# Nostrademous/dotaclient

Hardware: AMD Instinct MI355X
Metric: PPO optimizer samples/sec (whole node) + actor steps/sec, 1v1-mid LSTM policy (higher is better)
Workload: dtype fp32

## Files before the change

### dotaclient_amd/learner/engine.py

```python
from __future__ import annotations

import contextlib
import itertools
import os
import threading
from dataclasses import dataclass
from typing import Dict, List, Optional

import torch

from ..models.policy import Policy
from ..parallel.dp import DataParallel, FlatParams
from .losses import ppo_loss, split_heads, vpg_loss
from .optim import FlatAdam


CAPTURE_LOCK = threading.RLock()


_GRAPH_TOKENS = itertools.count(1)


def _capture_stream(device):
    return torch.cuda.Stream(device=device)
# ... 1 lines not shown

@dataclass

class LossConfig:
    algo: str = 'ppo'
    learning_rate: float = 1e-4
    entropy_coef: float = 0.01
    vf_coef: float = 0.5
    clip_eps: float = 0.1
    gamma: float = 0.98
    gae_lambda: float = 0.95
    max_grad_norm: float = 0.5
    compat_value_bug: bool = False
    offpolicy: str = 'clip'
    vtrace: bool = False
    vtrace_rho_bar: float = 1.0
    vtrace_c_bar: float = 1.0


class Learner:
    def __init__(self, policy: Policy, loss_cfg: LossConfig, device='cpu', backend: str = 'auto',
                 bucket_cap_mb: float = 8.0, overlap: bool = True, dp: bool = True, precision: str = 'fp32'):
        if precision not in ('fp32', 'bf16', 'fp32-exact'):
            raise ValueError(f'precision must be fp32, fp32-exact or bf16, got {precision!r}')
        self.device = torch.device(device)
        self.cfg = loss_cfg
        self.precision = precision
        self.policy = policy.to(self.device)
        auto = backend == 'auto'
        if auto:
            backend = 'fused' if self.device.type == 'cuda' else 'torch'
        self.backend = backend
        self.flat = FlatParams(self.policy, device=self.device)
        self.dp = DataParallel(self.policy, flat=self.flat, bucket_cap_mb=bucket_cap_mb, overlap=overlap,
                               broadcast=dp)
        self.opt = FlatAdam(self.flat, lr=loss_cfg.learning_rate, max_grad_norm=loss_cfg.max_grad_norm,
                            use_kernels=self.device.type == 'cuda')
        self.model = self.policy
        if backend == 'fused':
            from ..models.fused import FusedPolicy
            fused = FusedPolicy(self.policy, loss_cfg, precision=precision)
            if fused.use_pipeline():
                self.model = fused
                self.model.attach_flat(self.flat.flat)
            elif auto:
                self.backend = backend = 'torch'
            else:
                raise ValueError(f'backend fused: no kernel path for {self.policy.config} at {precision}')
        self.counts = self.policy.layout.action_counts()
        self.n_steps = 0
        self.graph = None
        self._static_idx: Dict[tuple, torch.Tensor] = {}
        self._graph_warmup = 0

    def enable_graph(self, warmup: int = 2):
        if self.backend != 'fused' or self.device.type != 'cuda':
            return False
        if not self.model.use_pipeline():
            return False
        self._graph_warmup = max(1, int(warmup))
        return True

    def _autocast(self):
        if self.backend == 'torch' and self.device.type == 'cuda' and self.precision == 'bf16':
            return torch.autocast('cuda', dtype=torch.bfloat16)
        return contextlib.nullcontext()

    def hidden_from_batch(self, batch):
        if not self.policy.is_recurrent:
            return None
        return (batch['h0'].unsqueeze(0).contiguous(), batch['c0'].unsqueeze(0).contiguous())

    def loss(self, batch: Dict[str, torch.Tensor]):
        cfg = self.cfg
        stable = not self.policy.config.compat_bugs
        if self.backend == 'fused':
            return self.model.loss(batch, cfg)
        with self._autocast():
            logits, values, _ = self.model.forward_packed(batch['env'], batch['units'], self.hidden_from_batch(batch),
                                                          reset=batch.get('reset'))
        logits = {k: v.float() for k, v in logits.items()}
        values = values.float()
        actions = split_heads(batch['actions'], self.counts)
        masks = split_heads(batch['masks'], self.counts)
        if cfg.algo == 'ppo':
            adv, ret, extra = batch['adv'], batch['ret'], {}
            if cfg.vtrace:
                adv, ret, extra = self._vtrace_torch(batch, logits, values, masks, actions)
            loss, metrics = ppo_loss(logits, values, actions, masks, adv, ret, batch['logp_old'],
                                     cfg.clip_eps, cfg.entropy_coef, cfg.vf_coef, stable=stable,
                                     offpolicy=cfg.offpolicy)
            metrics.update(extra)
            return loss, metrics
        return vpg_loss(logits, values, actions, masks, batch['norm_ret'], batch['ret'], cfg.entropy_coef,
                        cfg.vf_coef, compat_value_bug=cfg.compat_value_bug, stable=stable)

    def _vtrace_torch(self, batch, logits, values, masks, actions):
        from ..constants import EPS
        from ..ops.scan import vtrace_step
        from .losses import sampled_logp
        cfg = self.cfg
        B, S = batch['env'].shape[:2]
        tm = (lambda x: x.detach().float().reshape(B, S, *x.shape[2:]).transpose(0, 1).reshape(B * S, *x.shape[2:]))
        with torch.no_grad():
            lp = sampled_logp(logits, actions, masks, stable=not self.policy.config.compat_bugs)
            adv, ret, st = vtrace_step(tm(values.squeeze(-1)).cpu(), tm(lp).cpu(), tm(batch['logp_old']).cpu(),
                                       tm(batch['vt']).cpu(), B, S, cfg.gamma, cfg.gae_lambda, cfg.vtrace_rho_bar,
                                       cfg.vtrace_c_bar)
            dev = batch['env'].device
            back = (lambda x: x.reshape(S, B).t().contiguous().to(dev))
            adv, ret = back(adv), back(ret)
            v = batch['vt'][..., 2].float()
            n = v.sum().clamp_min(1.0)
            mu = (adv * v).sum() / n
            sd = (((adv - mu) ** 2 * v).sum() / n).sqrt()
            adv = ((adv - mu) / (sd + EPS)) * v
            s = st.sum(0)
            extra = {'offpolicy/rho_mean': (s[0] / s[3].clamp_min(1)).to(dev),
                     'offpolicy/rho_truncated': (s[1] / s[3].clamp_min(1)).to(dev),
                     'offpolicy/behaviour_kl': (s[2] / s[3].clamp_min(1)).to(dev)}
        return adv, ret, extra

    def _fwd_bwd(self, batch):
        self.dp.zero_grad()
        loss, metrics = self.loss(batch)
        loss.backward()
        if self.backend == 'fused' and getattr(self.model, 'direct_used', False):
            self.dp.has_grad.copy_(self.model.grad_mask)
        return {k: v.detach() for k, v in metrics.items()}

    def direct(self) -> bool:
        return self.backend == 'fused' and self.device.type == 'cuda' and self.model.use_pipeline()

    STEP_FIELDS = ('units', 'env', 'actions', 'masks', 'adv', 'ret', 'logp_old', 'norm_ret')

    @staticmethod
    def batch_to_time_major(batch):
        B, S = batch['env'].shape[:2]
        out = {}
        for k in Learner.STEP_FIELDS:
            v = batch.get(k)
            if v is None:
                v = torch.zeros(B, S, device=batch['env'].device)
            out[k] = v.transpose(0, 1).reshape(S * B, *v.shape[2:]).contiguous()
        if 'reset' in batch:
            out['reset'] = batch['reset'].transpose(0, 1).reshape(S * B).contiguous()
        if 'vt' in batch:
            out['vt'] = batch['vt'].transpose(0, 1).reshape(S * B, 4).contiguous()
        for k in ('h0', 'c0'):
            if k in batch:
                out[k] = batch[k].contiguous()
        return out, B, S

    def gather_time_major(self, replay, idx, S: int):
        B = idx.numel()
        fields = self.STEP_FIELDS + tuple(k for k in ('reset', 'vt') if k in replay.data)
        if idx.is_cuda:
            from .. import ops
            seq = [k for k in ('h0', 'c0') if k in replay.data]
            outs = ops.require().replay_gather([replay.data[k] for k in fields] +
                                               [replay.data[k] for k in seq], len(fields),
                                               idx.contiguous())
            return dict(zip(list(fields) + seq, outs))
        ar = getattr(self, '_arange', None)
        if ar is None or ar.numel() < S or ar.device != idx.device:
            ar = self._arange = torch.arange(max(S, 1), device=idx.device, dtype=torch.long)
        rows = (idx.view(1, B) * S + ar[:S].view(S, 1)).reshape(-1)
        out = {}
        for k in fields:
            pool = replay.data[k]
            out[k] = pool.view(-1, *pool.shape[2:]).index_select(0, rows)
        for k in ('h0', 'c0'):
            if k in replay.data:
                out[k] = replay.data[k].index_select(0, idx)
        return out

    def _split_mode(self) -> bool:
        import os
        if getattr(self, '_split', None) is None:
            force = os.environ.get('DCA_DP_SPLIT') == '1'
            ok = (self.direct() and (self.dp.enabled or force) and self.model.chunks == 1
                  and os.environ.get('DCA_DP_SPLIT', '') != '0')
            if ok:
                early = self.model.early_param_names()
                idx = [i for i, n in enumerate(self.model.param_names) if n in early]
                ok = self.dp.split_buckets(idx) if self.dp.enabled else bool(idx)
            self._split = bool(ok)
        return self._split

    def _direct_body(self, batch_tm, B, S, hook=None):
        self.flat.grad.zero_()
        if hook is None and self._split_mode():
            hook = self.dp.launch_early
        self.model.split_hook = hook
        try:
            vec = self.model.train_direct(batch_tm, B, S, self.cfg)
        finally:
            self.model.split_hook = None
        self.dp.has_grad.copy_(self.model.grad_mask)
        return vec

    def _metrics_from_vec(self, vec):
        from ..models.pipelined import METRIC_NAMES
        names = [n for n in METRIC_NAMES if (self.cfg.algo == 'ppo' or n not in ('approx_kl', 'clipfrac'))
                 and (self.cfg.vtrace or not n.startswith('offpolicy/'))]
        return {n: vec[METRIC_NAMES.index(n)] for n in names}

    def _graph_ready(self) -> bool:
        return bool(self._graph_warmup) and self.n_steps >= self._graph_warmup

    @staticmethod
    def _capture_mode() -> str:
        return 'thread_local'

    def _replay_split(self, key, body):
        graphs = self.__dict__.setdefault('_graphs', {})
        if key not in graphs:
            if getattr(self, '_graph_stream', None) is None:
                self._graph_stream = _capture_stream(self.device)
            s = self._graph_stream
            cur = torch.cuda.current_stream(self.device)
            s.wait_stream(cur)
            with torch.cuda.stream(s):
                body(lambda: None)
            cur.wait_stream(s)
            mode = self._capture_mode()
            g1, g2 = torch.cuda.CUDAGraph(), torch.cuda.CUDAGraph()
            switched = []

            def switch():
                g1.capture_end()
                g2.capture_begin(pool=g1.pool(), capture_error_mode=mode)
                switched.append(True)

            torch.cuda.synchronize(self.device)
            with CAPTURE_LOCK, torch.cuda.stream(s):
                g1.capture_begin(capture_error_mode=mode)
                out = body(switch)
                if not switched:
                    raise RuntimeError('direct step never reached its DP split point')
                g2.capture_end()
            cur.wait_stream(s)
            graphs[key] = ((g1, g2), out)
            self.graph = g1
        (g1, g2), out = graphs[key]
        g1.replay()
        self.dp.launch_early()
        g2.replay()
        return out

    def _replay_graph(self, key, body):
        graphs = self.__dict__.setdefault('_graphs', {})
        if key not in graphs:
            if getattr(self, '_graph_stream', None) is None:
                self._graph_stream = _capture_stream(self.device)
            s = self._graph_stream
            cur = torch.cuda.current_stream(self.device)
            s.wait_stream(cur)
            with torch.cuda.stream(s):
                body()
            cur.wait_stream(s)
            g = torch.cuda.CUDAGraph()
            with CAPTURE_LOCK, torch.cuda.graph(g, stream=s, capture_error_mode=self._capture_mode()):
                out = body()
            graphs[key] = (g, out)
            self.graph = g
        g, out = graphs[key]
        g.replay()
        return out

    def _step_direct_batch(self, batch):
        if not self._graph_ready():
            bt, B, S = self.batch_to_time_major(batch)
            return self._direct_body(bt, B, S)
        B, S = batch['env'].shape[:2]
        key = ('batch', B, S, tuple(sorted(batch)))
        if key not in self.__dict__.get('_graphs', {}):
            self._static_in = {k: v.clone() for k, v in batch.items()}
        else:
            for k, v in batch.items():
                self._static_in[k].copy_(v, non_blocking=True)

        if self._split_mode():
            def body_split(hook):
                bt, B_, S_ = self.batch_to_time_major(self._static_in)
                return self._direct_body(bt, B_, S_, hook=hook)
            return self._replay_split(key, body_split)

        def body():
            bt, B_, S_ = self.batch_to_time_major(self._static_in)
            return self._direct_body(bt, B_, S_)
        return self._replay_graph(key, body)

    @staticmethod
    def _replay_key(replay, B: int, S: int):
        tok = replay.__dict__.get('_dca_graph_token')
        if tok is None:
            tok = replay.__dict__['_dca_graph_token'] = next(_GRAPH_TOKENS)
        return ('replay', tok, B, S)

    def release_graphs(self, replay) -> int:
        tok = replay.__dict__.get('_dca_graph_token')
        if tok is None:
            return 0
        graphs = self.__dict__.get('_graphs', {})
        dead = [k for k in graphs if k[0] == 'replay' and k[1] == tok]
        for k in dead:
            g = graphs.pop(k)[0]
            if self.graph is g or (isinstance(g, tuple) and self.graph in g):
                self.graph = None
            self._static_idx.pop(k, None)
        return len(dead)

    def train_step_replay(self, replay, B: int, recent: Optional[int] = None) -> Dict[str, torch.Tensor]:
        if self.direct() and self._graph_ready() and getattr(replay, 'host_sampling', False):
            key = self._replay_key(replay, B, replay.S)
            if key in self.__dict__.get('_graphs', {}):
                replay.sample_into(self._static_idx[key], recent)
                return self._step_replay_key(replay, key, None)
        return self.train_step_indices(replay, replay.sample_indices(B, recent))

    def train_step_indices(self, replay, idx: torch.Tensor) -> Dict[str, torch.Tensor]:
        if not self.direct():
            return self.train_step(replay.gather(idx))
        if self._graph_ready():
            return self._step_replay_key(replay, self._replay_key(replay, idx.numel(), replay.S), idx)
        return self._finish(self._direct_body(self.gather_time_major(replay, idx, replay.S), idx.numel(), replay.S))

    def _step_replay_key(self, replay, key, idx: Optional[torch.Tensor]) -> Dict[str, torch.Tensor]:
        B, S = key[2], key[3]
        if key not in self.__dict__.get('_graphs', {}):
            self._static_idx[key] = idx.clone()
        elif idx is not None:
            self._static_idx[key].copy_(idx)
        sidx = self._static_idx[key]
        if self._split_mode():
            vec = self._replay_split(key, lambda hook: self._direct_body(
                self.gather_time_major(replay, sidx, S), B, S, hook=hook))
        else:
            vec = self._replay_graph(key, lambda: self._direct_body(self.gather_time_major(replay, sidx, S), B, S))
        return self._finish(vec)

    def _sync_and_step(self):
        if self.backend == 'fused':
            self.dp.err_flag.copy_(self.model.err)
        fold = self.dp.enabled and self.opt.use_kernels
        self.dp.sync(scale=not fold)
        if self.backend == 'fused' and self.dp.enabled:
            sticky = getattr(self, '_err_any', None)
            if sticky is None:
                sticky = self._err_any = torch.zeros_like(self.dp.err_flag)
            torch.maximum(sticky, self.dp.err_flag, out=sticky)
        return self.opt.step(self.dp.counts, divide=fold, skip=self.dp.err_flag)

    def check_error(self):
        self.opt.check_nonfinite()
        if self.backend != 'fused':
            return
        sticky = getattr(self, '_err_any', None)
        if sticky is not None and float(sticky.item()) != 0.0:
            own = int(self.model.err.item())
            sticky.zero_()
            raise RuntimeError(f'persistent kernel error on a data-parallel rank (own code {own}): the step was '
                               'skipped by every rank\'s Adam')
        self.model.check_error()

    def error_flags(self) -> List[torch.Tensor]:
        flags = [self.opt.nonfinite]
        if self.backend == 'fused':
            sticky = getattr(self, '_err_any', None)
            if sticky is not None:
                flags.append(sticky)
            flags.append(self.model.err)
        return flags

    def _finish(self, vec):
        metrics = self._metrics_from_vec(vec.clone())
        metrics['grad_norm'] = self._sync_and_step().clone()
        self.n_steps += 1
        return metrics

    def train_step(self, batch: Dict[str, torch.Tensor]) -> Dict[str, torch.Tensor]:
        if self.direct():
            return self._finish(self._step_direct_batch(batch))
        metrics = self._fwd_bwd(batch)
        metrics['grad_norm'] = self._sync_and_step().clone()
        self.n_steps += 1
        return metrics

    @torch.no_grad()
    def evaluate_sequences(self, data: Dict[str, torch.Tensor], n: int, chunk: int = 32):
        S = data['units'].shape[1]
        if self.direct():
            from .. import ops
            C = ops.require()
            fields = ('units', 'env', 'actions', 'masks') + (('reset',) if 'reset' in data else ())
            seq = [k for k in ('h0', 'c0') if k in data]
            lps, vals = [], []
            for i0 in range(0, n, chunk):
                i1 = min(n, i0 + chunk)
                idx = torch.arange(i0, i1, device=self.device, dtype=torch.int64)
                outs = C.replay_gather([data[k] for k in fields] + [data[k] for k in seq], len(fields), idx)
                bt = dict(zip(list(fields) + seq, outs))
                lp, v = self.model.forward_logp_value(bt, i1 - i0, S)
                lps.append(lp.view(S, i1 - i0).t())
                vals.append(v.view(S, i1 - i0).t())
            return torch.cat(lps, 0).contiguous(), torch.cat(vals, 0).contiguous()
        from .losses import sampled_logp
        hidden = None
        if self.policy.is_recurrent and 'h0' in data:
            hidden = (data['h0'][:n].unsqueeze(0).contiguous(), data['c0'][:n].unsqueeze(0).contiguous())
        with self._autocast():
            logits, values, _ = self.model.forward_packed(data['env'][:n], data['units'][:n], hidden,
                                                          reset=data['reset'][:n] if 'reset' in data else None)
        logits = {k: v.float() for k, v in logits.items()}
        lp = sampled_logp(logits, split_heads(data['actions'][:n], self.counts), split_heads(data['masks'][:n],
                                                                                             self.counts),
                          stable=not self.policy.config.compat_bugs)
        return lp.float(), values.float().reshape(n, S)

    def state_dict(self):
        return {'optimizer': self.opt.state_dict(), 'n_steps': self.n_steps}

    def broadcast_state(self, src: int = 0):
        import torch.distributed as dist
        for t in (self.opt.exp_avg, self.opt.exp_avg_sq, self.opt.steps):
            dist.broadcast(t, src)
        n = torch.tensor([self.n_steps], dtype=torch.int64, device=self.opt.steps.device)
        dist.broadcast(n, src)
        self.n_steps = int(n.item())

    def load_state_dict(self, d):
        self.opt.load_state_dict(d['optimizer'])
        self.n_steps = d.get('n_steps', 0)

    def after_load_weights(self):
        self.flat.rebind()
        if self.backend == 'fused':
            self.model.refresh()
```

### dotaclient_amd/models/fused.py

```python
from __future__ import annotations

from typing import Dict, List

import torch

from .policy import Policy

LDZ = 160


class FusedPolicy:
    def __init__(self, policy: Policy, loss_cfg=None, precision: str = 'fp32'):
        from .. import ops
        if precision not in ('fp32', 'bf16', 'fp32-exact'):
            raise ValueError(f'precision must be fp32, fp32-exact or bf16, got {precision!r}')
        self.C = ops.require()
        self.policy = policy
        self.cfg = policy.config
        self.loss_cfg = loss_cfg
        self.precision = precision
        self.fp32 = precision in ('fp32', 'fp32-exact')
        self.exact = precision == 'fp32-exact'
        dev = next(policy.parameters()).device
        self.err = torch.zeros(1, dtype=torch.int32, device=dev)
        self.param_names: List[str] = [n for n, _ in policy.named_parameters()]
        self.params = [p for _, p in policy.named_parameters()]
        self.fully_fused = not self.cfg.entity_attention and self.cfg.unit_dim == 128 and self.cfg.env_dim == 128
        self.attention_fused = (self.cfg.entity_attention and self.cfg.unit_dim == 128 and self.cfg.env_dim == 128
                                and self.cfg.attention_heads == 4 and self.cfg.layout.max_units == 64)

    def wcast(self, t: torch.Tensor) -> torch.Tensor:
        t = t.detach()
        return t if self.fp32 else t.to(torch.bfloat16)

    def apply_direct_grads(self, grads, g, written=(), set_mask: bool = True):
        gl, views, mask = [], [], []
        for name, p, t in zip(self.param_names, self.params, grads):
            mask.append(t is not None or name in written)
            if t is None:
                continue
            if p.grad is None:
                p.grad = torch.zeros_like(p)
            gl.append((t if t.dtype == torch.float32 else t.float()).contiguous())
            views.append(p.grad)
        self.C.multi_axpy(views, gl, None if g is None else g.reshape(1).float().contiguous())
        if set_mask and getattr(self, '_mask_list', None) != mask:
            self._mask_list = mask
            self.grad_mask = torch.tensor(mask, dtype=torch.float32, device=self.err.device)
        self.direct_used = True

    def attach_flat(self, flat: torch.Tensor):
        self.flat_buffer = flat
        self._wimg = None

    def weight_images(self):
        from .pipelined import WeightImages
        with_value = self.loss_cfg is None or self.loss_cfg.vf_coef > 0
        key = (with_value, self.flat_buffer.data_ptr() if getattr(self, 'flat_buffer', None) is not None else None,
               tuple(p.data_ptr() for p in self.params))
        if getattr(self, '_wimg', None) is None or self._wimg_key != key:
            if getattr(self, 'flat_buffer', None) is None:
                raise RuntimeError('FusedPolicy.attach_flat(flat) must be called before the fused LSTM step')
            self._wimg = WeightImages(self, self.flat_buffer, with_value)
            self._wimg_key = key
        return self._wimg

    def scratch(self, name, shape, dtype, device):
        d = self.__dict__.setdefault('_scratch', {})
        t = d.get(name)
        if t is None or tuple(t.shape) != tuple(shape) or t.dtype != dtype or t.device != torch.device(device):
            t = d[name] = torch.zeros(shape, dtype=dtype, device=device)
        return t

    def loss_prep_ws(self, device):
        return self.scratch('loss_prep_ws', (int(self.C.loss_prep_ws_elems()),), torch.int32, device)

    def train_direct(self, batch_tm, B: int, S: int, cfg=None) -> torch.Tensor:
        from .pipelined import train_direct
        if cfg is not None:
            self.loss_cfg = cfg
        self.refresh()
        self.direct_used = False
        return train_direct(self, batch_tm, B, S)

    def forward_logp_value(self, batch_tm, B: int, S: int):
        from .pipelined import forward_logp_value
        self.refresh()
        H = self.cfg.hidden
        dev = batch_tm['units'].device
        h0, c0 = batch_tm.get('h0'), batch_tm.get('c0')
        if h0 is None:
            h0 = c0 = torch.zeros(B, H, device=dev)
        return forward_logp_value(self, batch_tm['units'], batch_tm['env'], batch_tm['actions'], batch_tm['masks'],
                                  h0, c0, B, S, reset_t=batch_tm.get('reset'))

    def side_stream(self):
        if getattr(self, '_side', None) is None:
            self._side = torch.cuda.Stream(device=self.err.device)
        return self._side

    def use_pipeline(self) -> bool:
        if not (self.fully_fused or self.attention_fused) or not self.fp32:
            return False
        if self.cfg.rnn == 'lstm':
            return self.cfg.hidden % 128 == 0
        return self.cfg.hidden % 128 == 0 and self.cfg.pre_rnn_dim == 256

    split_hook = None
    early_applied = frozenset()

    def early_param_names(self) -> frozenset:
        pre = ('affine_pre_rnn.', 'rnn.', 'fake_rnn.', 'affine_head_enum.', 'affine_move_', 'affine_unit_attention.',
               'affine_value.')
        return frozenset(n for n in self.param_names if n.startswith(pre))

    @property
    def chunks(self) -> int:
        import os
        return int(os.environ.get('DCA_PIPELINE_CHUNKS', '1'))

    def gate_perm(self, H, device):
        key = (H, str(device))
        if getattr(self, '_perm_key', None) != key:
            from ..ops.lstm import gate_perm
            self._perm, self._perm_key = gate_perm(H, device), key
            self._inv = torch.empty_like(self._perm)
            self._inv[self._perm] = torch.arange(self._perm.numel(), device=self._perm.device)
        return self._perm

    def gate_perm_i32(self, H, device):
        key = (H, str(device))
        if getattr(self, '_perm32_key', None) != key:
            self._perm32, self._perm32_key = self.gate_perm(H, device).to(torch.int32).contiguous(), key
        return self._perm32

    def gate_inv(self, H, device):
        self.gate_perm(H, device)
        return self._inv

    def type_segments(self, device):
        key = str(device)
        if getattr(self, '_seg_key', None) != key:
            counts = list(self.cfg.layout.counts)
            seg = torch.zeros(sum(counts), 6, device=device)
            off = 0
            for t, cnt in enumerate(counts):
                seg[off:off + cnt, t] = 1.0
                off += cnt
            self._seg, self._seg_key = seg, key
        return self._seg

    def type_offset_list(self):
        import itertools
        return [0] + list(itertools.accumulate(self.cfg.layout.counts))

    def type_offsets(self, device):
        key = str(device)
        if getattr(self, '_toff_key', None) != key:
            import itertools
            offs = [0] + list(itertools.accumulate(self.cfg.layout.counts))
            self._toff, self._toff_key = torch.tensor(offs, dtype=torch.int32, device=device), key
        return self._toff

    def unit_types(self, device):
        key = str(device)
        if getattr(self, '_utype_key', None) != key:
            ty = sum([[t] * c for t, c in enumerate(self.cfg.layout.counts)], [])
            self._utype, self._utype_key = torch.tensor(ty, dtype=torch.uint8, device=device), key
        return self._utype

    def refresh(self):
        self.params = [p for _, p in self.policy.named_parameters()]

    def head_cat(self, P, differentiable: bool = False):
        H = self.cfg.hidden
        dev = P['affine_value.weight'].device
        d = (lambda t: t) if differentiable else (lambda t: t.detach())
        with_value = self.loss_cfg is None or self.loss_cfg.vf_coef > 0
        wv = d(P['affine_value.weight']) if with_value else torch.zeros(1, H, device=dev)
        bv = d(P['affine_value.bias']) if with_value else torch.zeros(1, device=dev)
        pad = LDZ - 150
        w = torch.cat([d(P['affine_unit_attention.weight']), d(P['affine_head_enum.weight']),
                       d(P['affine_move_x.weight']), d(P['affine_move_y.weight']), wv,
                       torch.zeros(pad, H, device=dev)], 0)
        b = torch.cat([d(P['affine_unit_attention.bias']), d(P['affine_head_enum.bias']),
                       d(P['affine_move_x.bias']), d(P['affine_move_y.bias']), bv,
                       torch.zeros(pad, device=dev)], 0)
        return w, b

    def split_head_grads(self, dW, db, grads):
        spans = [('affine_unit_attention', 0, 128), ('affine_head_enum', 128, 131), ('affine_move_x', 131, 140),
                 ('affine_move_y', 140, 149)]
        if self.loss_cfg is None or self.loss_cfg.vf_coef > 0:
            spans.append(('affine_value', 149, 150))
        for name, lo, hi in spans:
            grads[f'{name}.weight'] = dW[lo:hi]
            grads[f'{name}.bias'] = db[lo:hi]

    def loss(self, batch: Dict[str, torch.Tensor], cfg):
        from ..ops.heads import assemble_loss, batch_norms
        from .pipelined import PipelinedPolicyLoss
        if not self.use_pipeline():
            raise ValueError(f'FusedPolicy: no kernel path for {self.cfg} at {self.precision} (use the torch backend)')
        self.loss_cfg = cfg
        self.direct_used = False
        B, S = batch['env'].shape[:2]
        N = B * S
        dev = batch['env'].device
        actions = batch['actions'].reshape(N, -1).contiguous()
        masks = batch['masks'].reshape(N, -1).contiguous()
        ret = batch['ret'].reshape(N).float().contiguous()
        algo = 0 if cfg.algo == 'ppo' else 1
        norms = batch_norms(actions, ret, cfg.compat_value_bug and algo == 1, S)
        zeros = torch.zeros(N, device=dev)
        adv = batch['adv'].reshape(N).contiguous() if 'adv' in batch else zeros
        lpo = batch['logp_old'].reshape(N).contiguous() if 'logp_old' in batch else zeros
        nret = batch['norm_ret'].reshape(N).contiguous() if 'norm_ret' in batch else zeros
        rst = batch.get('reset')
        H = self.cfg.hidden
        h0 = batch.get('h0')
        c0 = batch.get('c0')
        if h0 is None:
            h0 = torch.zeros(B, H, device=dev)
            c0 = torch.zeros(B, H, device=dev)
        self.refresh()
        vt = batch.get('vt') if getattr(cfg, 'vtrace', False) else None
        part, logp = PipelinedPolicyLoss.apply(self, batch['units'].contiguous(), batch['env'].contiguous(), actions,
                                               masks, adv, ret, lpo, nret, norms, h0.contiguous(), c0.contiguous(),
                                               rst, vt, *self.params)
        loss, metrics = assemble_loss(part, norms, cfg, ret, N, S)
        if getattr(self, 'vtrace_stats', None) is not None:
            st = self.vtrace_stats.sum(0)
            for i, k in enumerate(('offpolicy/rho_mean', 'offpolicy/rho_truncated', 'offpolicy/behaviour_kl')):
                metrics[k] = st[i] / st[3].clamp_min(1.0)
        return loss, metrics

# ... 5 lines not shown
```

### dotaclient_amd/models/pipelined.py

```python
from __future__ import annotations

import os
from typing import Dict, List, Optional

import torch

from ..ops.lstm import team_bwd, team_fwd
from .policy import TYPE_SUFFIX

LDZ = 160

DIRECT_GEMM_GRADS = ('rnn.weight_hh_l0', 'rnn.weight_ih_l0', 'affine_pre_rnn.weight', 'affine_pre_rnn.bias')

METRIC_NAMES = ['loss', 'policy_loss', 'entropy_loss', 'advantage_loss', 'entropy', 'advantage', 'approx_kl',
                'clipfrac', 'entropy/enum', 'entropy/x', 'entropy/y', 'entropy/target_unit',
                'offpolicy/rho_mean', 'offpolicy/rho_truncated', 'offpolicy/behaviour_kl']


def _frag_order(w: torch.Tensor) -> torch.Tensor:
    R, K = w.shape
    return w.view(R // 16, 16, K // 32, 4, 8).permute(0, 2, 3, 1, 4).contiguous()


def _k16_order(w: torch.Tensor) -> torch.Tensor:
# ... 375 lines not shown
            if lin:
                pass
            elif rst is not None:
                hprev = torch.cat([h016.unsqueeze(0), hs16[:S - 1]], 0).masked_fill_(rst.bool().unsqueeze(2), 0.0)
                gemm_tn(dG16, hprev.view(n, H), out=dWhh, perm=gperm, accumulate=True)
            elif t0 > 0:
                gemm_tn(dG16, hs16[t0 - 1:t1 - 1].view(n, H), out=dWhh, perm=gperm, accumulate=True)
            else:
                gemm_tn(dG16, hs16[0:t1 - 1].view(n - B, H), out=dWhh, perm=gperm, accumulate=True, b0=h016)
            if lin:
                gemm_tn(dG16, x16[r0:r1], out=dWih, colsum=dbf)
            else:
                gemm_tn(dG16, x16[r0:r1], out=dWih, perm=gperm, accumulate=True)
        dpre16, dx896 = C.dpre_dx(dG16, dx_w[0], dx_w[1], x16[r0:r1], dx_w[2], dx_w[3])
        pre_main = wg_side and split is None and exact
        if pre_main:
            with torch.cuda.stream(sL):
                wg_done = torch.cuda.Event()
                wg_done.record(sL)
            after_enc.append(lambda d=dpre16, xr=x896[r0:r1]: gemm_tn(d, xr, out=dWpre, accumulate=True,
                                                                      colsum=dbpre))
        elif wg_side:
            sL.wait_stream(main)
            with torch.cuda.stream(sL):
                gemm_tn(dpre16, x896[r0:r1], out=dWpre, accumulate=True, colsum=dbpre)
                wg_done = torch.cuda.Event()
                wg_done.record(sL)
        else:
            gemm_tn(dpre16, x896[r0:r1], out=dWpre, accumulate=True, colsum=dbpre)
        if split is not None:
            if wg_done is not None:
                main.wait_event(wg_done)
                wg_done = None
            if not lin:
                grads['rnn.bias_ih_l0'] = db
                grads['rnn.bias_hh_l0'] = db
            early = [grads.pop(nm, None) if nm in early_names else None for nm in fp.param_names]
            fp.apply_direct_grads(early, None, set_mask=False)
            fp.early_applied = early_names
            split()
            split = None
        demb_in = None
        if attn:
            if exact:
                nil = E0p.new_empty(0)
                wot, wq4 = (W['wot_x'], nil), (W['wq4_x'], nil)
            else:
                wot = [_frag_order(t) for t in C.split_bf16x2(P['entity_attn.out.weight'].detach().t().contiguous())]
                wq4 = [_k16_order(t) for t in C.split_bf16x2(P['entity_attn.qkv.weight'].detach())]
            dE1, dQKV, demb_in, lnsum = C.attn_block_bwd(
                dtl, z, dx896, arg, toff, bool(cfg.compat_bugs), Oat, QKV, bqkv, lse, E0p, W['bout'], ln_mu, ln_rs,
                P['entity_attn.ln.weight'].detach(), wot[0], wot[1], wq4[0], wq4[1], None)
            dgam, dbet, dbt_attn = lnsum[:128], lnsum[128:256], lnsum[256:].view(6, 128)
            dbout = torch.empty(128, device=dev)
            dbqkv = torch.empty(384, device=dev)
            if wg_side and _WG_BALANCE == '1':
                sL.wait_stream(main)
                side_after.append(lambda: gemm_tn(dQKV, Xn, out=dWqkv, colsum=dbqkv))
                after_enc.append(lambda: gemm_tn(dE1, Oat, out=dWout, colsum=dbout))
            elif wg_side:
                sL.wait_stream(main)
                side_after.append(lambda: (gemm_tn(dE1, Oat, out=dWout, colsum=dbout),
                                           gemm_tn(dQKV, Xn, out=dWqkv, colsum=dbqkv)))
            else:
                dWout = gemm_tn(dE1, Oat, colsum=dbout)
                dWqkv = gemm_tn(dQKV, Xn, colsum=dbqkv)
        def small_grads():
            return C.enc_small_grads(z[r0:r1], dtl[r0:r1], fp.type_offsets(dev), dx896, env_t[r0:r1], we, be,
                                     bool(cfg.compat_bugs))
        small = None
        if wg_side and not side_after:
            sL.wait_stream(main)
            with torch.cuda.stream(sL):
                small = small_grads()
                wg_done = torch.cuda.Event()
                wg_done.record(sL)
        dwt_c, dw1_c, db1_c = C.encoder_bwd(units_t[r0:r1], w1, b1, wtT16, dtl[r0:r1], z[r0:r1],
                                            dx896, arg[r0:r1], counts, bool(cfg.compat_bugs), demb_in=demb_in,
                                            exact=exact)
        for fn in after_enc:
            fn()
        after_enc.clear()
        if side_after:
            with torch.cuda.stream(sL):
                for fn in side_after:
                    fn()
                small = small_grads()
                wg_done = torch.cuda.Event()
                wg_done.record(sL)
            side_after.clear()
        dw1 = _acc(dw1, dw1_c)
        db1 = _acc(db1, db1_c)
        dWt = _acc(dWt, dwt_c)
        dbt_c, dWe_c, dbe_c = small if small is not None else small_grads()
        dbt = _acc(dbt, dbt_attn if attn else dbt_c)
        dWe = _acc(dWe, dWe_c)
        dbe = _acc(dbe, dbe_c)
    if wg_done is not None:
        main.wait_event(wg_done)
    if not direct:
        if not lin:
            grads['rnn.weight_hh_l0'] = dWhh
            grads['rnn.weight_ih_l0'] = dWih
        grads['affine_pre_rnn.weight'] = dWpre
        grads['affine_pre_rnn.bias'] = dbpre
    if not lin and 'rnn.bias_ih_l0' not in fp.early_applied:
        grads['rnn.bias_ih_l0'] = db
        grads['rnn.bias_hh_l0'] = db
    grads['affine_unit_basic_stats.weight'] = dw1
    grads['affine_unit_basic_stats.bias'] = db1
    for t, s in enumerate(TYPE_SUFFIX):
        grads[f'affine_unit_{s}.weight'] = dWt[t]
        grads[f'affine_unit_{s}.bias'] = dbt[t]
    grads['affine_env.weight'] = dWe
    grads['affine_env.bias'] = dbe
    if attn:
        grads['entity_attn.ln.weight'] = dgam
        grads['entity_attn.ln.bias'] = dbet
        grads['entity_attn.qkv.weight'] = dWqkv
        grads['entity_attn.qkv.bias'] = dbqkv
        grads['entity_attn.out.weight'] = dWout
        grads['entity_attn.out.bias'] = dbout
    part = parts[0] if len(parts) == 1 else torch.cat(parts, 0)
    return part, logp, grads


class PipelinedPolicyLoss(torch.autograd.Function):
    @staticmethod
    def forward(ctx, fp, units, env, actions, masks, adv, ret, logp_old, nret, norms, h0, c0, reset, vt, *params):
        P = dict(zip(fp.param_names, params))
        B, S, U, _ = units.shape
        N = B * S
        tm = (lambda x: x.reshape(B, S, *x.shape[1:]).transpose(0, 1).reshape(N, *x.shape[1:]).contiguous())
        units_t = units.transpose(0, 1).reshape(N, U, 10).contiguous()
        env_t = env.transpose(0, 1).reshape(N, 3).contiguous()
        W = fp.weight_images().refresh(fp.C)
        rst_t = reset.reshape(B, S).transpose(0, 1).reshape(N).contiguous() if reset is not None else None
        part, logp, grads = fused_step_tm(fp, W, P, units_t, env_t, tm(actions), tm(masks), tm(adv), tm(ret),
                                          tm(logp_old), tm(nret), norms, h0, c0, B, S, reset_t=rst_t,
                                          vt_t=tm(vt.reshape(N, 4)) if vt is not None else None)
        ctx.grads = [grads.get(nm) for nm in fp.param_names]
        ctx.fp = fp
        logp_b = logp.view(S, B).t().reshape(N)
        ctx.mark_non_differentiable(logp_b)
        return part.sum(0), logp_b

    @staticmethod
    def backward(ctx, gpart, _glogp):
        ctx.fp.apply_direct_grads(ctx.grads, gpart[15])
        ctx.grads = None
        return (None,) * (14 + len(ctx.fp.param_names))


def train_direct(fp, batch_tm: Dict[str, torch.Tensor], B: int, S: int) -> torch.Tensor:
    C = fp.C
    lc = fp.loss_cfg
    N = B * S
    dev = batch_tm['units'].device
    norms = fp.scratch('norms', (8,), torch.float32, dev)
    main = torch.cuda.current_stream(dev)
    sL = fp.side_stream()
    sL.wait_stream(main)
    with torch.cuda.stream(sL):
        C.loss_prep(batch_tm['actions'], fp.loss_prep_ws(dev), norms)
        if lc.compat_value_bug and lc.vf_coef > 0:
            g_last = batch_tm['ret'].view(S, B)[:, B - 1]
            norms[6:8] = torch.stack([g_last.sum(), (g_last * g_last).sum()])
    W = fp.weight_images().refresh(C)
    P = dict(zip(fp.param_names, fp.params))
    H = fp.cfg.hidden
    h0 = batch_tm.get('h0')
    c0 = batch_tm.get('c0')
    if h0 is None:
        h0 = torch.zeros(B, H, device=dev)
        c0 = torch.zeros(B, H, device=dev)
    gout = {nm: P[nm].grad for nm in DIRECT_GEMM_GRADS if nm in P}
    vt = batch_tm.get('vt') if getattr(lc, 'vtrace', False) else None
    if getattr(lc, 'vtrace', False) and vt is None:
        raise ValueError('LossConfig.vtrace needs the per-row vt field (learner/optimizer.py advantages="vtrace-step")')
    part, _, grads = fused_step_tm(fp, W, P, batch_tm['units'], batch_tm['env'], batch_tm['actions'],
                                   batch_tm['masks'], batch_tm['adv'], batch_tm['ret'], batch_tm['logp_old'],
                                   batch_tm['norm_ret'], norms, h0, c0, B, S, gout=gout,
                                   reset_t=batch_tm.get('reset'), vt_t=vt)
    fp.apply_direct_grads([grads.get(nm) for nm in fp.param_names], None,
                          written=set(gout) | set(fp.early_applied))
    out = torch.empty(16, device=dev)
    C.loss_assemble(part, norms, N, 0 if lc.algo == 'ppo' else 1, float(lc.entropy_coef), float(lc.vf_coef), out,
                    S=S, compat_value_bug=bool(lc.compat_value_bug))
    if fp.vtrace_stats is not None:
        st = fp.vtrace_stats.sum(0)
        out[12:15] = st[:3] / st[3].clamp_min(1.0)
    return out


def forward_logp_value(fp, units_t, env_t, act_t, msk_t, h0, c0, B: int, S: int,
                       reset_t: Optional[torch.Tensor] = None):
    C = fp.C
    cfg = fp.cfg
    exact = bool(getattr(fp, 'exact', False))
    lin = cfg.rnn != 'lstm'
    N = B * S
    U = units_t.shape[1]
    H = cfg.hidden
    dev = units_t.device
    W = fp.weight_images().refresh(C)
    P = dict(zip(fp.param_names, fp.params))
    w1, b1 = P['affine_unit_basic_stats.weight'].detach(), P['affine_unit_basic_stats.bias'].detach()
    we, be = P['affine_env.weight'].detach(), P['affine_env.bias'].detach()
    x896, emb, arg = C.encoder_fwd(units_t, env_t, w1, b1, W['wt16'], W['bt'], we, be, list(cfg.layout.counts),
                                   bool(cfg.compat_bugs), exact=exact)
    if cfg.entity_attention:
        E0p = emb.view(N * U, 128)
        if exact:
            nil = E0p.new_empty(0)
            wq, wo = (W['wq_x'], nil), (W['wo_x'], nil)
        else:
            wq, wo = W['wq_f'], W['wo_f']
        arg = torch.empty(N, 6, 128, dtype=torch.uint8, device=dev)
        out = C.attn_block_fwd(E0p, W['bout'], P['entity_attn.ln.weight'].detach(), P['entity_attn.ln.bias'].detach(),
                               wq[0], wq[1], P['entity_attn.qkv.bias'].detach(), wo[0], wo[1],
                               fp.type_offset_list(), x896, arg, bool(cfg.compat_bugs), 1e-5)
        emb = out[6].view(N, U, 128)
    elif cfg.compat_bugs:
        x896[:, 768:896] = x896[:, 512:640]
    if exact:
        nil = W['wpre16'].new_empty(0)
        x16, xp = C.pre_rnn_chain(x896, W['wpre16'], nil, W['bpre16'], W['wih16'], nil)
        hw = ((W['wcat256'], nil), W['bcat256'])
    else:
        x16, xp = C.pre_rnn_chain(x896, W['pre_s'][0], W['pre_s'][1], W['bpre16'], W['ih_s'][0], W['ih_s'][1])
        hw = (W['wcat_s'], W['bcat256'])
    if lin:
        hs = xp.add_(W['bias4']).view(S, B, H)
    else:
        rst = reset_t.reshape(S, B) if reset_t is not None else None
        hs = torch.empty(S, B, H, device=dev)
        o = team_fwd(C, xp.view(S, B, H, 4), W['whh16'], h0.contiguous(), c0.contiguous(), fp.err, False,
                     time_major=True, hs_out=hs, cs_out=torch.empty(S, B, H, device=dev),
                     gates_out=torch.empty(S, B, H, 4, device=dev), bias4=W['bias4'], reset=rst)
        hs = o[0]
    z = C.rowmm_out256(hs.reshape(N, H), hw[0][0], hw[0][1], hw[1])
    zero = fp.scratch('fwd_zero', (N,), torch.float32, dev)
    norms = fp.scratch('fwd_norms', (8,), torch.float32, dev)
    _, _, _, lp = C.heads_loss(z, emb, act_t, msk_t, zero, zero, zero, zero, norms, 0, False, S, B, 0.1, 0.0, 0.0,
                               dz_bf16=False, precise=exact)
    return lp, z[:, 149].contiguous()
```

### dotaclient_amd/ops/csrc/bindings.cpp

```cpp
#include <torch/extension.h>
#include <ATen/hip/HIPContext.h>
#include <hip/hip_runtime.h>

#include <algorithm>
#include <cstring>

#include "launchers.h"

namespace {

inline hipStream_t cur_stream() { return at::hip::getCurrentHIPStream().stream(); }

inline void hip_check(hipError_t e, const char* what) {
  TORCH_CHECK(e == hipSuccess, what, " failed: ", hipGetErrorString(e));
}

#define CHECK_DEV(t) TORCH_CHECK((t).is_cuda(), #t " must be a GPU tensor")
#define CHECK_CONTIG(t) TORCH_CHECK((t).is_contiguous(), #t " must be contiguous")
#define CHECK_DT(t, dt) TORCH_CHECK((t).scalar_type() == (dt), #t " must be " #dt)
#define CHECK_F32(t) CHECK_DEV(t); CHECK_CONTIG(t); CHECK_DT(t, at::kFloat)
#define CHECK_BF16(t) CHECK_DEV(t); CHECK_CONTIG(t); CHECK_DT(t, at::kBFloat16)
#define CHECK_I32(t) CHECK_DEV(t); CHECK_CONTIG(t); CHECK_DT(t, at::kInt)
#define CHECK_U8(t) CHECK_DEV(t); CHECK_CONTIG(t); CHECK_DT(t, at::kByte)

// ... 75 lines not shown
    CHECK_DEV(dst[i]); CHECK_DEV(src[i]); CHECK_CONTIG(dst[i]); CHECK_CONTIG(src[i]);
    TORCH_CHECK(dst[i].nbytes() == src[i].nbytes(), "multi_copy: byte size mismatch at ", i);
    d.push_back(dst[i].data_ptr());
    s.push_back(src[i].data_ptr());
    n.push_back((long long)dst[i].nbytes());
  }
  hip_check(dca_multi_copy(d.data(), s.data(), n.data(), (int)d.size(), cur_stream()), "dca_multi_copy");
}

void multi_axpy(std::vector<torch::Tensor> dst, std::vector<torch::Tensor> src, c10::optional<torch::Tensor> scale) {
  TORCH_CHECK(dst.size() == src.size(), "multi_axpy: list length mismatch");
  TORCH_CHECK(dst.size() <= 64, "multi_axpy: at most 64 tensors");
  std::vector<float*> d;
  std::vector<const float*> s;
  std::vector<long long> n;
  for (size_t i = 0; i < dst.size(); ++i) {
    CHECK_F32(dst[i]); CHECK_F32(src[i]);
    TORCH_CHECK(dst[i].numel() == src[i].numel(), "multi_axpy: numel mismatch at ", i);
    d.push_back(ptr<float>(dst[i]));
    s.push_back(ptr<float>(src[i]));
    n.push_back(dst[i].numel());
  }
  const float* sp = nullptr;
  if (scale.has_value() && scale->defined()) { CHECK_F32((*scale)); sp = ptr<float>(*scale); }
  hip_check(dca_multi_axpy(d.data(), s.data(), n.data(), (int)d.size(), sp, cur_stream()), "dca_multi_axpy");
}

constexpr int64_t kTeamTraceElems = 32LL * 4 * 64 * 8;
inline unsigned long long* trace_ptr(const c10::optional<torch::Tensor>& t, int64_t need, const char* name) {
  if (!t.has_value() || !t->defined()) return nullptr;
  CHECK_DEV(*t); CHECK_CONTIG(*t);
  TORCH_CHECK(t->scalar_type() == at::kLong && t->numel() >= need, name,
              ": trace must be a contiguous int64 GPU tensor with >= ", need, " elements");
  return ptr<unsigned long long>(*t);
}


namespace {
inline torch::Tensor out_or_new(const c10::optional<torch::Tensor>& o, at::IntArrayRef shape,
                                const at::TensorOptions& opt, const char* name) {
  if (o.has_value() && o->defined()) {
    TORCH_CHECK(o->is_cuda() && o->is_contiguous() && o->sizes() == shape && o->scalar_type() == opt.dtype(),
                name, ": preallocated output has the wrong shape/dtype/layout");
    return *o;
  }
  return torch::empty(shape, opt);
}
}

inline const unsigned char* reset_ptr(const c10::optional<torch::Tensor>& r, int B, int S) {
  if (!r.has_value() || !r->defined()) return nullptr;
  CHECK_DEV(*r); CHECK_CONTIG(*r);
  TORCH_CHECK(r->scalar_type() == at::kByte && r->numel() == (int64_t)B * S, "reset must be B*S uint8 flags");
  return r->data_ptr<unsigned char>();
}

inline void check_ctl(const torch::Tensor& ctl) {
  CHECK_DEV(ctl); CHECK_CONTIG(ctl);
  TORCH_CHECK(ctl.numel() * ctl.element_size() >= (int64_t)dca_lstm_team_ctl_bytes(),
              "team control block too small (use ops.lstm.team_ctl())");
}

std::vector<torch::Tensor> lstm_team_fwd(torch::Tensor xp4, torch::Tensor whh, torch::Tensor h0, torch::Tensor c0,
                                         torch::Tensor err, torch::Tensor ctl, bool want_f32_h,
                                         c10::optional<torch::Tensor> trace,
                                         bool time_major, c10::optional<torch::Tensor> hs_out,
                                         c10::optional<torch::Tensor> cs_out, c10::optional<torch::Tensor> gates_out,
                                         c10::optional<torch::Tensor> bias4, bool precise,
                                         c10::optional<torch::Tensor> reset) {
  CHECK_F32(xp4); CHECK_DEV(whh); CHECK_CONTIG(whh); CHECK_F32(h0); CHECK_F32(c0); CHECK_I32(err); check_ctl(ctl);
  const bool f32w = whh.scalar_type() == at::kFloat;
  TORCH_CHECK(f32w || whh.scalar_type() == at::kBFloat16, "whh must be bf16 or f32");
  TORCH_CHECK(xp4.dim() == 4 && xp4.size(3) == 4, "xp4 must be (B,S,H,4) or (S,B,H,4)");
  const int B = time_major ? xp4.size(1) : xp4.size(0), S = time_major ? xp4.size(0) : xp4.size(1);
  const int H = xp4.size(2);
  TORCH_CHECK(whh.size(0) == 4 * H && whh.size(1) == H, "whh must be (4H,H)");
  TORCH_CHECK(h0.size(0) == B && h0.size(1) == H && c0.size(0) == B && c0.size(1) == H, "h0/c0 must be (B,H)");
  TORCH_CHECK(H == 128 || H == 256 || H == 512, "lstm_team_fwd: H in {128,256,512}");
  auto f32 = xp4.options();
  const int64_t d0 = time_major ? S : B, d1 = time_major ? B : S;
  auto hs = out_or_new(hs_out, {d0, d1, H}, f32w ? f32 : f32.dtype(at::kBFloat16), "hs_out");
  torch::Tensor hsf = (want_f32_h && !f32w) ? torch::empty({d0, d1, H}, f32) : torch::Tensor();
  auto cs = out_or_new(cs_out, {d0, d1, H}, f32, "cs_out");
  auto gates4 = out_or_new(gates_out, {d0, d1, H, 4}, f32, "gates_out");
  auto hn = torch::empty({B, H}, f32);
  auto cn = torch::empty({B, H}, f32);
  const float* bias_p = nullptr;
  if (bias4.has_value() && bias4->defined()) {
    CHECK_F32((*bias4));
    TORCH_CHECK(bias4->numel() == 4 * H, "bias4 must hold 4H floats (unit-major)");
    bias_p = ptr<float>(*bias4);
  }
  const size_t wsb = dca_lstm_team_workspace(B, H, 0, f32w ? 1 : 0);
  auto ws = torch::empty({(int64_t)wsb}, f32.dtype(at::kByte));
  hip_check(dca_lstm_team_fwd(ptr<float>(xp4), whh.data_ptr(), ptr<float>(h0), ptr<float>(c0),
                              f32w ? nullptr : ptr<short>(hs),
                              f32w ? ptr<float>(hs) : (want_f32_h ? ptr<float>(hsf) : nullptr), ptr<float>(cs),
                              ptr<float>(gates4), ptr<float>(hn), ptr<float>(cn), ctl.data_ptr(), ws.data_ptr(), wsb,
                              ptr<unsigned>(err), B, S, H, time_major ? 1 : 0, cur_stream(),
                              trace_ptr(trace, kTeamTraceElems, "lstm_team_fwd"),
                              bias_p, f32w ? 1 : 0, precise ? 1 : 0, reset_ptr(reset, B, S)),
            "dca_lstm_team_fwd");
  if (f32w) return {hs, hs, cs, gates4, hn, cn};
  return {hs, want_f32_h ? hsf : hs, cs, gates4, hn, cn};
}

std::vector<torch::Tensor> lstm_team_bwd(torch::Tensor dhs, torch::Tensor gates4, torch::Tensor cs,
                                         torch::Tensor c0, c10::optional<torch::Tensor> dhn,
                                         c10::optional<torch::Tensor> dcn, torch::Tensor whh, torch::Tensor err,
                                         torch::Tensor ctl, c10::optional<torch::Tensor> trace, bool time_major,
                                         c10::optional<torch::Tensor> dg_out, bool dg_bf16, bool want_dbias,
                                         bool precise, c10::optional<torch::Tensor> reset) {
  CHECK_F32(dhs); CHECK_F32(gates4); CHECK_F32(cs); CHECK_F32(c0); CHECK_DEV(whh); CHECK_CONTIG(whh); CHECK_I32(err);
  check_ctl(ctl);
  const bool f32w = whh.scalar_type() == at::kFloat;
  TORCH_CHECK(f32w || whh.scalar_type() == at::kBFloat16, "whh must be bf16 or f32");
  TORCH_CHECK(!(f32w && dg_bf16), "lstm_team_bwd: the fp32 variant writes fp32 gate gradients");
  const int B = time_major ? dhs.size(1) : dhs.size(0), S = time_major ? dhs.size(0) : dhs.size(1);
  const int H = dhs.size(2);
  TORCH_CHECK(gates4.dim() == 4 && gates4.size(0) == dhs.size(0) && gates4.size(1) == dhs.size(1) &&
                  gates4.size(2) == H && gates4.size(3) == 4, "gates4 must match dhs with a trailing 4");
  TORCH_CHECK(cs.sizes() == dhs.sizes(), "cs must match dhs");
  TORCH_CHECK(c0.size(0) == B && c0.size(1) == H, "c0 must be (B,H)");
  TORCH_CHECK(whh.size(0) == 4 * H && whh.size(1) == H, "whh must be (4H,H)");
  TORCH_CHECK(H == 128 || H == 256 || H == 512, "lstm_team_bwd: H in {128,256,512}");
  const float* dhn_p = nullptr;
  const float* dcn_p = nullptr;
  if (dhn.has_value() && dhn->defined()) { CHECK_F32((*dhn)); dhn_p = ptr<float>(*dhn); }
  if (dcn.has_value() && dcn->defined()) { CHECK_F32((*dcn)); dcn_p = ptr<float>(*dcn); }
  auto f32 = dhs.options();
  auto dgates4 = out_or_new(dg_out, {dhs.size(0), dhs.size(1), H, 4}, dg_bf16 ? f32.dtype(at::kBFloat16) : f32,
                            "dg_out");
  auto dh0 = torch::empty({B, H}, f32);
  auto dc0 = torch::empty({B, H}, f32);
  torch::Tensor dbp = want_dbias ? torch::empty({dca_lstm_team_chains(B, f32w ? 1 : 0), 4 * H}, f32) : torch::Tensor();
  const size_t wsb = dca_lstm_team_workspace(B, H, 1, f32w ? 1 : 0);
  auto ws = torch::empty({(int64_t)wsb}, f32.dtype(at::kByte));
  hip_check(dca_lstm_team_bwd(ptr<float>(dhs), ptr<float>(gates4), ptr<float>(cs), ptr<float>(c0), dhn_p, dcn_p,
                              whh.data_ptr(), dg_bf16 ? nullptr : ptr<float>(dgates4), ptr<float>(dh0),
                              ptr<float>(dc0), ctl.data_ptr(), ws.data_ptr(), wsb, ptr<unsigned>(err), B, S, H,
                              time_major ? 1 : 0, cur_stream(),
                              trace_ptr(trace, kTeamTraceElems, "lstm_team_bwd"),
                              dg_bf16 ? ptr<short>(dgates4) : nullptr, want_dbias ? ptr<float>(dbp) : nullptr,
                              f32w ? 1 : 0, precise ? 1 : 0, reset_ptr(reset, B, S)),
            "dca_lstm_team_bwd");
  if (want_dbias) return {dgates4, dh0, dc0, dbp.sum(0)};
  return {dgates4, dh0, dc0};
}

std::vector<torch::Tensor> heads_loss(torch::Tensor z, torch::Tensor emb, torch::Tensor act, torch::Tensor msk,
                                      torch::Tensor adv, torch::Tensor ret, torch::Tensor logp_old,
                                      torch::Tensor nret, torch::Tensor norms, int64_t algo, bool compat_value_bug,
                                      int64_t S_bug, int64_t B_bug, double clip_eps, double ent_coef,
                                      double vf_coef, bool dz_bf16, bool precise) {
  CHECK_F32(z); CHECK_DEV(emb); CHECK_CONTIG(emb); CHECK_U8(act); CHECK_U8(msk); CHECK_F32(adv); CHECK_F32(ret);
  CHECK_F32(logp_old); CHECK_F32(nret); CHECK_F32(norms);
  const bool ef32 = emb.scalar_type() == at::kFloat;
  TORCH_CHECK(ef32 || emb.scalar_type() == at::kBFloat16, "emb must be bf16 or f32");
  TORCH_CHECK(z.dim() == 2 && emb.dim() == 3 && emb.size(2) == 128, "z (N,ldz), emb (N,U,128)");
  const int N = z.size(0), ldz = z.size(1), U = emb.size(1);
  TORCH_CHECK(emb.size(0) == N && act.size(0) == N && msk.size(0) == N, "row count mismatch");
  TORCH_CHECK(act.size(1) == 21 + U && msk.size(1) == 21 + U, "actions/masks must be (N, 21+U)");
  TORCH_CHECK(adv.numel() == N && ret.numel() == N && logp_old.numel() == N && nret.numel() == N, "per-row inputs");
  TORCH_CHECK(norms.numel() >= 8, "norms must hold 8 floats");
  TORCH_CHECK(ldz % 4 == 0 && ldz >= 150 && U <= 64, "ldz must be a multiple of 4 and >= 150; U <= 64");
  auto dz = dz_bf16 ? torch::empty_like(z, z.options().dtype(at::kBFloat16)) : torch::empty_like(z);
  auto dtl = torch::empty({N, U}, z.options());
  const int nb = dca_heads_loss_nblocks(N);
  auto part = torch::empty({nb, 16}, z.options());
  auto logp = torch::empty({N}, z.options());
  hip_check(dca_heads_loss(ptr<float>(z), ldz, emb.data_ptr(), ptr<unsigned char>(act), ptr<unsigned char>(msk),
                           21 + U, ptr<float>(adv), ptr<float>(ret), ptr<float>(logp_old), ptr<float>(nret),
                           ptr<float>(norms), dz_bf16 ? nullptr : ptr<float>(dz), ptr<float>(dtl), ptr<float>(part),
                           ptr<float>(logp), N, U, (int)algo, compat_value_bug ? 1 : 0, (int)S_bug, (int)B_bug,
                           (float)clip_eps, (float)ent_coef, (float)vf_coef, cur_stream(),
                           dz_bf16 ? ptr<short>(dz) : nullptr, ef32 ? 1 : 0, precise && ef32 ? 1 : 0),
            "dca_heads_loss");
  return {dz, dtl, part, logp};
}

std::vector<torch::Tensor> encoder_fwd(torch::Tensor units, torch::Tensor env, torch::Tensor w1, torch::Tensor b1,
                                       torch::Tensor wt, torch::Tensor bt, torch::Tensor we, torch::Tensor be,
                                       std::vector<int64_t> counts, bool compat, bool exact,
                                       c10::optional<torch::Tensor> x896_out, c10::optional<torch::Tensor> emb_out,
                                       c10::optional<torch::Tensor> arg_out) {
  CHECK_F32(units); CHECK_F32(env); CHECK_F32(w1); CHECK_F32(b1); CHECK_DEV(wt); CHECK_CONTIG(wt); CHECK_F32(bt);
  CHECK_F32(we); CHECK_F32(be);
  const bool f32w = wt.scalar_type() == at::kFloat;
  TORCH_CHECK(f32w || wt.scalar_type() == at::kBFloat16, "wt must be bf16 or f32");
  TORCH_CHECK(!exact || f32w, "encoder_fwd: exact mode needs fp32 weights");
  TORCH_CHECK(units.dim() == 3 && units.size(2) == 10, "units must be (N,U,10)");
  const int N = units.size(0), U = units.size(1);
  TORCH_CHECK(env.size(0) == N && env.size(1) == 3, "env must be (N,3)");
  TORCH_CHECK(w1.size(0) == 128 && w1.size(1) == 10 && wt.size(0) == 6 && wt.size(1) == 128 && wt.size(2) == 128,
              "weight shapes");
  TORCH_CHECK(counts.size() == 6, "counts must have 6 entries");
  int c[6];
  int64_t tot = 0;
  for (int i = 0; i < 6; ++i) { c[i] = (int)counts[i]; tot += counts[i]; }
  TORCH_CHECK(tot == U && U <= 64, "counts must sum to U <= 64");
  auto o = units.options();
  const auto adt = f32w ? at::kFloat : at::kBFloat16;
  auto x896 = out_or_new(x896_out, {N, 896}, o.dtype(adt), "x896_out");
  auto emb = out_or_new(emb_out, {N, U, 128}, o.dtype(adt), "emb_out");
  auto arg = out_or_new(arg_out, {N, 6, 128}, o.dtype(at::kByte), "arg_out");
  hip_check(dca_encoder_fwd(ptr<float>(units), ptr<float>(env), ptr<float>(w1), ptr<float>(b1), wt.data_ptr(),
                            ptr<float>(bt), ptr<float>(we), ptr<float>(be), x896.data_ptr(), emb.data_ptr(),
                            ptr<unsigned char>(arg), N, U, c, compat ? 1 : 0, cur_stream(), exact ? 2 : (f32w ? 1 : 0)),
            "dca_encoder_fwd");
  return {x896, emb, arg};
}

std::vector<torch::Tensor> encoder_bwd(torch::Tensor units, torch::Tensor w1, torch::Tensor b1, torch::Tensor wtT,
                                       torch::Tensor dtl, torch::Tensor q, torch::Tensor dx, torch::Tensor arg,
                                       std::vector<int64_t> counts, bool compat,
                                       c10::optional<torch::Tensor> demb_in, bool exact) {
  CHECK_F32(units); CHECK_F32(w1); CHECK_F32(b1); CHECK_DEV(wtT); CHECK_CONTIG(wtT); CHECK_F32(dtl); CHECK_F32(dx);
  CHECK_U8(arg); CHECK_DEV(q); CHECK_DT(q, at::kFloat);
  const bool f32w = wtT.scalar_type() == at::kFloat;
  TORCH_CHECK(f32w || wtT.scalar_type() == at::kBFloat16, "wtT must be bf16 or f32");
  TORCH_CHECK(!exact || f32w, "encoder_bwd: exact mode needs fp32 weights");
  const int N = units.size(0), U = units.size(1);
  TORCH_CHECK(q.dim() == 2 && q.size(0) == N && q.size(1) >= 128 && q.stride(1) == 1 && q.stride(0) % 4 == 0,
              "q must be (N, >=128) with unit column stride and 16-B aligned rows");
  TORCH_CHECK(dtl.size(0) == N && dtl.size(1) == U && dx.size(0) == N && dx.size(1) == 896, "dtl/dx shapes");
  TORCH_CHECK(arg.size(0) == N && arg.size(1) == 6 && arg.size(2) == 128, "arg shape");
  int c[6];
  int64_t tot = 0;
  for (int i = 0; i < 6; ++i) { c[i] = (int)counts[i]; tot += counts[i]; }
  TORCH_CHECK(tot == U && U <= 64, "counts must sum to U <= 64");
  auto o = units.options();
  auto dwt = torch::empty({6, 128, 128}, o);
  auto dw1 = torch::empty({128, 10}, o);
  auto db1 = torch::empty({128}, o);
  const size_t wsb = dca_encoder_bwd_workspace(N, U, c, f32w ? 1 : 0);
  auto ws = torch::empty({(int64_t)((wsb + 3) / 4)}, o);
  const void* dein = nullptr;
  if (demb_in && demb_in->defined()) {
    CHECK_DEV(*demb_in); CHECK_CONTIG(*demb_in);
    TORCH_CHECK(demb_in->scalar_type() == (f32w ? at::kFloat : at::kBFloat16), "encoder_bwd: demb_in dtype");
    TORCH_CHECK(demb_in->numel() == (int64_t)N * U * 128, "demb_in must be (N, U, 128)");
    dein = demb_in->data_ptr();
  }
  hip_check(dca_encoder_bwd(ptr<float>(units), ptr<float>(w1), ptr<float>(b1), wtT.data_ptr(), ptr<float>(dtl),
                            ptr<float>(q), (int)q.stride(0), ptr<float>(dx), ptr<unsigned char>(arg), ptr<float>(dwt),
                            ptr<float>(dw1), ptr<float>(db1), ws.data_ptr(), wsb, N, U, c, compat ? 1 : 0,
                            cur_stream(), dein, exact ? 2 : (f32w ? 1 : 0)),
            "dca_encoder_bwd");
  return {dwt, dw1, db1};
}

void sample_actions(torch::Tensor z, torch::Tensor emb, torch::Tensor handles, int64_t seed, torch::Tensor ctr,
                    torch::Tensor idx, torch::Tensor act, torch::Tensor msk, torch::Tensor logp, torch::Tensor value) {
  CHECK_F32(z); CHECK_DEV(emb); CHECK_CONTIG(emb); CHECK_DEV(handles); CHECK_CONTIG(handles);
  const bool e32 = emb.scalar_type() == at::kFloat;
  TORCH_CHECK(e32 || emb.scalar_type() == at::kBFloat16, "sample_actions: emb bf16 or fp32");
  const bool h32 = handles.scalar_type() == at::kInt;
  TORCH_CHECK(h32 || handles.scalar_type() == at::kLong, "sample_actions: handles int64 or int32");
  CHECK_DEV(ctr); CHECK_DT(ctr, at::kLong); CHECK_I32(idx); CHECK_U8(act); CHECK_U8(msk); CHECK_F32(logp);
  CHECK_F32(value);
  TORCH_CHECK(z.dim() == 2 && emb.dim() == 3 && emb.size(2) == 128, "z (N,ldz), emb (N,U,128)");
  const int N = z.size(0), ldz = z.size(1), U = emb.size(1);
  TORCH_CHECK(emb.size(0) == N && handles.size(0) == N && handles.size(1) == U, "row/unit count mismatch");
  TORCH_CHECK(idx.size(0) == N && idx.size(1) == 4 && logp.numel() == N && value.numel() == N, "output shapes");
  TORCH_CHECK(act.size(0) == N && act.size(1) == 21 + U && msk.sizes() == act.sizes(), "act/msk (N,21+U)");
  TORCH_CHECK(U <= 64 && ldz >= 150, "U <= 64, ldz >= 150");
  hip_check(dca_sample_actions(ptr<float>(z), ldz, emb.data_ptr(), e32 ? 1 : 0, handles.data_ptr(), h32 ? 1 : 0, N,
                               U, (unsigned long long)seed, ptr<long long>(ctr), ptr<int>(idx),
                               ptr<unsigned char>(act), ptr<unsigned char>(msk), ptr<float>(logp), ptr<float>(value),
                               cur_stream()),
            "dca_sample_actions");
}

static long long* bump_ptr(const c10::optional<torch::Tensor>& bump) {
  if (!bump || !bump->defined()) return nullptr;
  CHECK_DEV(*bump); CHECK_DT(*bump, at::kLong);
  TORCH_CHECK(bump->numel() >= 1, "bump: (1) int64 counter");
  return ptr<long long>(*bump);
}

void actor_state_prep(torch::Tensor pre, torch::Tensor h, torch::Tensor c, torch::Tensor keep, torch::Tensor xh,
                      c10::optional<torch::Tensor> bump) {
  CHECK_BF16(pre); CHECK_F32(h); CHECK_F32(c); CHECK_F32(keep); CHECK_BF16(xh);
  const int N = h.size(0), H = h.size(1), P = pre.size(1);
  TORCH_CHECK(pre.dim() == 2 && pre.size(0) == N && c.sizes() == h.sizes() && keep.numel() == N && xh.dim() == 2 &&
              xh.size(0) == N && xh.size(1) == P + H && H % 4 == 0 && P % 4 == 0, "actor_state_prep shapes");
  hip_check(dca_actor_state_prep(ptr<short>(pre), ptr<float>(h), ptr<float>(c), ptr<float>(keep), ptr<short>(xh), N, P,
                                 H, bump_ptr(bump), cur_stream()), "dca_actor_state_prep");
}

void lstm_cell(torch::Tensor gates, torch::Tensor h, torch::Tensor c, torch::Tensor h16,
               c10::optional<torch::Tensor> active) {
  CHECK_F32(gates); CHECK_F32(h); CHECK_F32(c); CHECK_BF16(h16);
  const int N = h.size(0), H = h.size(1);
  TORCH_CHECK(gates.size(0) == N && gates.size(1) == 4 * H && c.sizes() == h.sizes() && h16.sizes() == h.sizes(),
              "lstm_cell shapes");
  const float* act = nullptr;
  if (active && active->defined()) {
    CHECK_F32(*active);
    TORCH_CHECK(active->numel() == N, "lstm_cell: active must have one entry per row");
    act = ptr<float>(*active);
  }
  hip_check(dca_lstm_cell(ptr<float>(gates), ptr<float>(h), ptr<float>(c), ptr<short>(h16), act, N, H, cur_stream()),
            "dca_lstm_cell");
}

void actor_fp8(torch::Tensor x896, torch::Tensor wpre, torch::Tensor spre, torch::Tensor bpre, torch::Tensor wg,
               torch::Tensor sg, torch::Tensor bg, torch::Tensor wh, torch::Tensor sh, torch::Tensor bh,
               torch::Tensor h, torch::Tensor c, torch::Tensor keep, torch::Tensor z,
               c10::optional<torch::Tensor> active, c10::optional<torch::Tensor> bump) {
  CHECK_BF16(x896); CHECK_U8(wpre); CHECK_U8(wg); CHECK_U8(wh);
  CHECK_F32(spre); CHECK_F32(bpre); CHECK_F32(sg); CHECK_F32(bg); CHECK_F32(sh); CHECK_F32(bh);
  CHECK_F32(h); CHECK_F32(c); CHECK_F32(keep); CHECK_F32(z);
  const int n = x896.size(0);
  TORCH_CHECK(x896.dim() == 2 && x896.size(1) == 896, "actor_fp8: x896 (n, 896)");
  TORCH_CHECK(wpre.numel() == 256 * 896 && spre.numel() == 256 && bpre.numel() == 256, "actor_fp8: pre-RNN 256x896");
  TORCH_CHECK(wg.numel() == 2048 * 768 && sg.numel() == 2048 && bg.numel() == 2048, "actor_fp8: gates 2048x768");
  TORCH_CHECK(wh.numel() == 160 * 512 && sh.numel() == 160 && bh.numel() == 160, "actor_fp8: heads 160x512");
  TORCH_CHECK(h.dim() == 2 && h.size(0) == n && h.size(1) == 512 && c.sizes() == h.sizes() && keep.numel() == n,
              "actor_fp8: h, c (n, 512), keep (n)");
  TORCH_CHECK(z.dim() == 2 && z.size(0) == n && z.size(1) == 160, "actor_fp8: z (n, 160)");
  const float* act = nullptr;
  if (active && active->defined()) {
    CHECK_F32(*active);
    TORCH_CHECK(active->numel() == n, "actor_fp8: active (n)");
    act = ptr<float>(*active);
  }
  hip_check(dca_actor_fp8(ptr<short>(x896), wpre.data_ptr(), ptr<float>(spre), ptr<float>(bpre), wg.data_ptr(),
                          ptr<float>(sg), ptr<float>(bg), wh.data_ptr(), ptr<float>(sh), ptr<float>(bh), ptr<float>(h),
// ... 78 lines not shown
  } else {
    CHECK_BF16(wqh); CHECK_BF16(wql); CHECK_BF16(woh); CHECK_BF16(wol);
  }
  TORCH_CHECK(e0.numel() % (64 * 128) == 0 && e0.size(-1) == 128, "attn_block_fwd: e0 (N·64, 128)");
  const int64_t N = e0.numel() / (64 * 128);
  TORCH_CHECK(wqh.numel() == 384 * 128 && (exact || wql.numel() == 384 * 128) && woh.numel() == 128 * 128 &&
              (exact || wol.numel() == 128 * 128) && bq.numel() == 384 && bout.numel() == 128 && gamma.numel() == 128 &&
              beta.numel() == 128, "attn_block_fwd: weight shapes");
  TORCH_CHECK(x896.dim() == 2 && x896.size(0) == N && x896.size(1) == 896, "attn_block_fwd: x896 (N, 896)");
  TORCH_CHECK(arg.numel() == N * 6 * 128, "attn_block_fwd: arg (N, 6, 128)");
  TORCH_CHECK(type_off.size() == 7 && type_off[0] == 0 && type_off[6] == 64, "attn_block_fwd: 7 type offsets 0 … 64");
  int off[7];
  for (int i = 0; i < 7; ++i) off[i] = (int)type_off[i];
  auto o32 = e0.options();
  auto xn = torch::empty({N * 64, 128}, o32);
  auto mu = torch::empty({N * 64}, o32);
  auto rs = torch::empty({N * 64}, o32);
  auto qkv = torch::empty({N * 64, 384}, o32);
  auto o = torch::empty({N * 64, 128}, o32);
  auto lse = torch::empty({N, 4, 64}, o32);
  auto e1 = torch::empty({N * 64, 128}, o32);
  hip_check(dca_attn_block_fwd_f32(ptr<float>(e0), ptr<float>(bout), ptr<float>(gamma), ptr<float>(beta),
                                   wqh.data_ptr(), exact ? nullptr : wql.data_ptr(), ptr<float>(bq), woh.data_ptr(),
                                   exact ? nullptr : wol.data_ptr(), ptr<float>(xn), ptr<float>(mu), ptr<float>(rs),
                                   ptr<float>(qkv), ptr<float>(o), ptr<float>(lse), ptr<float>(e1), ptr<float>(x896),
                                   ptr<unsigned char>(arg), off, compat ? 1 : 0, (int)N, (float)eps, cur_stream(),
                                   exact ? 1 : 0),
            "dca_attn_block_fwd_f32");
  return {xn, mu, rs, qkv, o, lse, e1};
}

static void check_type_off(const std::vector<int64_t>& t) {
  TORCH_CHECK(t.size() == 7 && t[0] == 0 && t[6] == 64, "type offsets must be 7 values from 0 to 64");
  for (int i = 0; i < 6; ++i) TORCH_CHECK(t[i + 1] >= t[i], "type offsets must be non-decreasing");
}

std::vector<torch::Tensor> attn_block_bwd(torch::Tensor dtl, torch::Tensor q, torch::Tensor dx, torch::Tensor arg,
                                          std::vector<int64_t> type_off, bool compat, torch::Tensor o,
                                          torch::Tensor qkv, torch::Tensor bq, torch::Tensor lse, torch::Tensor e0,
                                          torch::Tensor bout, torch::Tensor mu, torch::Tensor rs, torch::Tensor gamma,
                                          torch::Tensor woth, torch::Tensor wotl, torch::Tensor wq4h,
                                          torch::Tensor wq4l, c10::optional<torch::Tensor> trace) {
  CHECK_F32(dtl); CHECK_DEV(q); CHECK_DT(q, at::kFloat); CHECK_F32(dx); CHECK_U8(arg); CHECK_F32(o); CHECK_F32(qkv);
  CHECK_F32(bq); CHECK_F32(lse); CHECK_F32(e0); CHECK_F32(bout); CHECK_F32(mu); CHECK_F32(rs); CHECK_F32(gamma);
  const bool exact = woth.scalar_type() == at::kFloat;
  CHECK_DEV(woth); CHECK_CONTIG(woth); CHECK_DEV(wq4h); CHECK_CONTIG(wq4h);
  if (exact) {
    CHECK_F32(wq4h);
  } else {
    CHECK_BF16(woth); CHECK_BF16(wotl); CHECK_BF16(wq4h); CHECK_BF16(wq4l);
  }
  check_type_off(type_off);
  const int64_t N = dtl.size(0);
  TORCH_CHECK(dtl.dim() == 2 && dtl.size(1) == 64, "attn_block_bwd: dtl (N, 64)");
  TORCH_CHECK(q.dim() == 2 && q.size(0) == N && q.size(1) >= 128 && q.stride(1) == 1, "attn_block_bwd: q (N, >=128)");
  TORCH_CHECK(dx.dim() == 2 && dx.size(0) == N && dx.size(1) == 896, "attn_block_bwd: dx (N, 896)");
  TORCH_CHECK(arg.numel() == N * 6 * 128, "attn_block_bwd: arg (N, 6, 128)");
  TORCH_CHECK(o.numel() == N * 64 * 128 && e0.numel() == N * 64 * 128 && qkv.numel() == N * 64 * 384 &&
              lse.numel() == N * 4 * 64 && mu.numel() == N * 64 && rs.numel() == N * 64, "attn_block_bwd: saved shapes");
  TORCH_CHECK(bq.numel() == 384 && bout.numel() == 128 && gamma.numel() == 128 && woth.numel() == 128 * 128 &&
              (exact || wotl.numel() == 128 * 128) && wq4h.numel() == 384 * 128 &&
              (exact || wq4l.numel() == 384 * 128), "attn_block_bwd: weight shapes");
  int off[7];
  for (int i = 0; i < 7; ++i) off[i] = (int)type_off[i];
  auto o32 = e0.options();
  auto de1 = torch::empty({N * 64, 128}, o32);
  auto dqkv = torch::empty({N * 64, 384}, o32);
  auto de0 = torch::empty({N * 64, 128}, o32);
  auto part = torch::empty({N, 1024}, o32);
  auto tmp = torch::empty({(int64_t)dca_attn_block_bwd_groups((int)N), 1024}, o32);
  auto sums = torch::empty({1024}, o32);
  if (trace.has_value() && trace->defined()) {
    CHECK_DEV(*trace); CHECK_CONTIG(*trace);
    TORCH_CHECK(trace->scalar_type() == at::kLong && trace->numel() >= 64 * 4 * 8,
                "attn_block_bwd: trace must be a contiguous int64 GPU tensor with >= 2048 elements");
  }
  hip_check(dca_attn_block_bwd_f32(ptr<float>(dtl), ptr<float>(q), (int)q.stride(0), ptr<float>(dx),
                                   ptr<unsigned char>(arg), off, compat ? 1 : 0, ptr<float>(o), ptr<float>(qkv),
                                   ptr<float>(bq), ptr<float>(lse), ptr<float>(e0), ptr<float>(bout), ptr<float>(mu),
                                   ptr<float>(rs), ptr<float>(gamma), woth.data_ptr(),
                                   exact ? nullptr : wotl.data_ptr(), wq4h.data_ptr(),
                                   exact ? nullptr : wq4l.data_ptr(), ptr<float>(de1), ptr<float>(dqkv),
                                   ptr<float>(de0), ptr<float>(part), ptr<float>(tmp), ptr<float>(sums), (int)N,
                                   cur_stream(),
                                   (trace.has_value() && trace->defined()) ? ptr<unsigned long long>(*trace) : nullptr,
                                   exact ? 1 : 0),
            "dca_attn_block_bwd_f32");
  return {de1, dqkv, de0, sums};
}


void returns_scan(torch::Tensor rew, torch::Tensor val, torch::Tensor off, torch::Tensor seglen, torch::Tensor boot,
                  torch::Tensor done, torch::Tensor keys, torch::Tensor ema, torch::Tensor ret, torch::Tensor adv,
                  torch::Tensor norm, torch::Tensor stats, int64_t mode, bool normalize, double gamma, double lam,
                  double factor, double eps, c10::optional<torch::Tensor> lr, double rho_bar, double c_bar) {
  CHECK_F32(rew); CHECK_F32(ema); CHECK_F32(ret); CHECK_F32(adv); CHECK_F32(norm); CHECK_F32(stats);
  TORCH_CHECK(rew.dim() == 2, "rew must be (L, K)");
  const int64_t L = rew.size(0);
  const int nseg = seglen.numel();
  for (auto* t : {&off, &seglen, &keys, &boot, &done})
    TORCH_CHECK(!t->is_cuda() && t->is_contiguous(), "returns_scan: segment metadata must be contiguous host tensors");
  TORCH_CHECK(off.scalar_type() == at::kInt && seglen.scalar_type() == at::kInt && keys.scalar_type() == at::kInt &&
              boot.scalar_type() == at::kFloat && done.scalar_type() == at::kByte, "returns_scan: metadata dtypes");
  TORCH_CHECK(off.numel() == nseg + 1 && boot.numel() == nseg && done.numel() == nseg && keys.numel() == nseg,
              "returns_scan: per-segment tensor lengths");
  TORCH_CHECK(ret.numel() == L && adv.numel() == L && norm.numel() == L && stats.numel() == 2 * nseg,
              "returns_scan: output lengths");
  TORCH_CHECK(ema.dim() == 2 && ema.size(1) == 3, "ema must be (n_keys, 3)");
  TORCH_CHECK(mode == 0 || mode == 1 || mode == 2, "mode must be 0 (discount), 1 (gae) or 2 (v-trace gae)");
  TORCH_CHECK(rew.size(1) <= 64, "returns_scan: at most 64 sub-rewards");
  const float* vp = nullptr;
  const float* lp = nullptr;
  if (mode >= 1) {
    CHECK_F32(val);
    TORCH_CHECK(val.numel() == L, "returns_scan: values must have one entry per row");
    vp = ptr<float>(val);
  }
  if (mode == 2) {
    TORCH_CHECK(lr.has_value() && lr->defined(), "returns_scan: v-trace needs the per-row log ratios");
    CHECK_F32((*lr));
    TORCH_CHECK(lr->numel() == L, "returns_scan: log ratios must have one entry per row");
    lp = ptr<float>(*lr);
  }
  if (nseg == 0) return;
  const int* o = off.data_ptr<int>();
  const int* k = keys.data_ptr<int>();
  TORCH_CHECK(o[0] == 0 && o[nseg] == L, "returns_scan: offsets must span [0, L]");
  int max_len = 0;
  for (int i = 0; i < nseg; ++i) {
    TORCH_CHECK(o[i + 1] >= o[i], "returns_scan: decreasing offsets at segment ", i);
    TORCH_CHECK(k[i] >= 0 && k[i] < ema.size(0), "returns_scan: key out of range at segment ", i);
    max_len = std::max(max_len, o[i + 1] - o[i]);
  }
  auto meta = torch::empty({(int64_t)(4 * nseg + 1 + (nseg + 3) / 4)}, torch::dtype(at::kInt).pinned_memory(true));
  int* mp = meta.data_ptr<int>();
  std::memcpy(mp, o, sizeof(int) * (nseg + 1));
  std::memcpy(mp + nseg + 1, seglen.data_ptr<int>(), sizeof(int) * nseg);
  std::memcpy(mp + 2 * nseg + 1, k, sizeof(int) * nseg);
  std::memcpy(mp + 3 * nseg + 1, boot.data_ptr<float>(), sizeof(float) * nseg);
  std::memcpy(mp + 4 * nseg + 1, done.data_ptr<uint8_t>(), nseg);
  auto md = meta.to(rew.device(), true);
  int* d = md.data_ptr<int>();
  auto ema_out = ema.clone();
  hip_check(dca_returns(ptr<float>(rew), (int)rew.size(1), vp, lp, d, d + nseg + 1,
                        reinterpret_cast<float*>(d + 3 * nseg + 1), reinterpret_cast<unsigned char*>(d + 4 * nseg + 1),
                        d + 2 * nseg + 1, nseg, max_len, ptr<float>(ret), ptr<float>(adv), ptr<float>(norm),
                        ptr<float>(stats), ptr<float>(ema), ptr<float>(ema_out), (int)mode, normalize ? 1 : 0,
                        (float)gamma, (float)lam, (float)rho_bar, (float)c_bar, (float)factor, (float)eps,
                        cur_stream()),
            "dca_returns");
  ema.copy_(ema_out);
}

void loss_prep(torch::Tensor act, torch::Tensor ws, torch::Tensor norms) {
  CHECK_U8(act); CHECK_I32(ws); CHECK_F32(norms);
  TORCH_CHECK(act.dim() == 2 && act.size(1) >= 22 && act.size(1) <= 128, "act must be (N, 21+U), U <= 107");
  const int nb = dca_loss_prep_blocks();
  TORCH_CHECK(ws.numel() >= 5 * nb + 1 && norms.numel() >= 8, "loss_prep: workspace / norms too small");
  int* w = ptr<int>(ws);
  hip_check(dca_loss_prep(ptr<unsigned char>(act), (int)act.size(0), (int)act.size(1), w,
                          reinterpret_cast<unsigned*>(w + 5 * nb), ptr<float>(norms), cur_stream()),
            "dca_loss_prep");
}

int64_t loss_prep_ws_elems() { return 5 * dca_loss_prep_blocks() + 1; }

std::vector<torch::Tensor> vtrace_step(torch::Tensor z, int64_t vcol, torch::Tensor lp, torch::Tensor mu,
                                       torch::Tensor vt, int64_t B, int64_t S, double gamma, double lam,
                                       double rho_bar, double c_bar) {
  CHECK_DEV(z); CHECK_DT(z, at::kFloat); CHECK_F32(lp); CHECK_F32(mu); CHECK_F32(vt);
  const int64_t N = B * S;
  TORCH_CHECK(z.dim() == 2 && z.size(0) == N && z.stride(1) == 1 && vcol >= 0 && vcol < z.size(1),
              "vtrace_step: z (B·S, ldz) with the value column inside");
  TORCH_CHECK(lp.numel() == N && mu.numel() == N && vt.numel() == 4 * N, "vtrace_step: per-row inputs");
  auto adv = torch::empty({N}, z.options());
  auto ret = torch::empty({N}, z.options());
  auto stats = torch::empty({B, 4}, z.options());
  hip_check(dca_vtrace_step(ptr<float>(z), (int)z.stride(0), (int)vcol, ptr<float>(lp), ptr<float>(mu),
                            ptr<float>(vt), ptr<float>(adv), ptr<float>(ret), ptr<float>(stats), (int)B, (int)S,
                            (float)gamma, (float)lam, (float)rho_bar, (float)c_bar, cur_stream()),
            "dca_vtrace_step");
  return {adv, ret, stats};
}

void featurize_raw(torch::Tensor raw, torch::Tensor hero, torch::Tensor units, c10::optional<torch::Tensor> handles) {
  CHECK_DEV(raw); CHECK_CONTIG(raw); CHECK_DT(raw, at::kInt);
  CHECK_F32(hero);
  CHECK_DEV(units); CHECK_CONTIG(units);
  TORCH_CHECK(raw.dim() == 3 && (raw.size(2) == 8 || raw.size(2) == 4),
              "featurize_raw: raw must be (rows, U, 8) int32, or (rows, U, 4) — the 16-byte records (fp16 out)");
  const int64_t rows = raw.size(0), U = raw.size(1);
  TORCH_CHECK(hero.numel() == rows * 4, "featurize_raw: hero must be (rows, 4)");
  TORCH_CHECK(units.numel() == rows * U * 10, "featurize_raw: units must be (rows, U, 10)");
  const bool half = units.scalar_type() == at::kHalf;
  TORCH_CHECK(half || units.scalar_type() == at::kFloat, "featurize_raw: units fp32 or fp16");
  void* hp = nullptr;
  if (handles.has_value() && handles->defined()) {
    CHECK_DEV(*handles); CHECK_CONTIG(*handles);
    TORCH_CHECK(handles->numel() == rows * U, "featurize_raw: handles must be (rows, U)");
    TORCH_CHECK(handles->scalar_type() == (half ? at::kInt : at::kLong),
                "featurize_raw: handles int64 with fp32 features, int32 with fp16");
    hp = handles->data_ptr();
  }
  TORCH_CHECK(rows * U < (int64_t)1 << 31, "featurize_raw: too many unit slots");
  if (raw.size(2) == 4) {
    TORCH_CHECK(half, "featurize_raw: 16-byte records featurize to fp16 (+ int32 handles)");
    hip_check(dca_featurize_raw16(raw.data_ptr(), ptr<float>(hero), units.data_ptr(), hp, (int)rows, (int)U,
                                  cur_stream()),
              "dca_featurize_raw16");
    return;
  }
  hip_check(dca_featurize_raw(raw.data_ptr(), ptr<float>(hero), units.data_ptr(), hp, (int)rows, (int)U, half ? 1 : 0,
                              cur_stream()),
            "dca_featurize_raw");
}

torch::Tensor occupy_xcd(int64_t xcd, int64_t blocks, double seconds, torch::Tensor like) {
  TORCH_CHECK(xcd >= 0 && xcd < 8 && blocks >= 1 && blocks <= 4096 && seconds > 0.0 && seconds <= 10.0,
              "occupy_xcd: xcd in [0, 8), 1..4096 blocks, 0 < seconds <= 10");
  auto seen = torch::zeros({blocks}, like.options().dtype(at::kInt));
  hip_check(dca_occupy_xcd((int)xcd, (int)blocks, seconds, ptr<int>(seen), cur_stream()), "dca_occupy_xcd");
  return seen;
}

void loss_assemble(torch::Tensor part, torch::Tensor norms, int64_t N, int64_t algo, double ent_coef, double vf_coef,
                   torch::Tensor out, int64_t S, bool compat_value_bug) {
  CHECK_F32(part); CHECK_F32(norms); CHECK_F32(out);
  TORCH_CHECK(part.dim() == 2 && part.size(1) == 16 && out.numel() >= 16 && norms.numel() >= 8,
              "loss_assemble shapes");
  hip_check(dca_loss_assemble(ptr<float>(part), (int)part.size(0), ptr<float>(norms), (int)N, (int)algo,
                              (float)ent_coef, (float)vf_coef, ptr<float>(out), (int)S, compat_value_bug ? 1 : 0,
                              cur_stream()),
            "dca_loss_assemble");
}

void weight_prep(torch::Tensor src, torch::Tensor map16, torch::Tensor dst16, torch::Tensor map32,
                 torch::Tensor dst32, c10::optional<torch::Tensor> maps, c10::optional<torch::Tensor> dsth,
                 c10::optional<torch::Tensor> dstl) {
  CHECK_F32(src); CHECK_I32(map16); CHECK_BF16(dst16); CHECK_I32(map32); CHECK_F32(dst32);
  TORCH_CHECK(map16.numel() == dst16.numel() && map32.numel() == 2 * dst32.numel(), "weight_prep: map sizes");
  const int* ms = nullptr;
  short *dh = nullptr, *dl = nullptr;
  int ns = 0;
  if (maps && maps->defined()) {
    TORCH_CHECK(dsth && dsth->defined() && dstl && dstl->defined(), "weight_prep: split map needs both hi / lo outputs");
    CHECK_I32(*maps); CHECK_BF16(*dsth); CHECK_BF16(*dstl);
    TORCH_CHECK(maps->numel() == dsth->numel() && dstl->numel() == dsth->numel(), "weight_prep: split map sizes");
    ms = ptr<int>(*maps); dh = ptr<short>(*dsth); dl = ptr<short>(*dstl); ns = (int)maps->numel();
  }
  hip_check(dca_weight_prep(ptr<float>(src), ptr<int>(map16), ptr<short>(dst16), (int)dst16.numel(), ptr<int>(map32),
                            ptr<float>(dst32), (int)dst32.numel(), ms, dh, dl, ns, cur_stream()),
            "dca_weight_prep");
}

void gemm_tn(torch::Tensor A, torch::Tensor B, torch::Tensor C, c10::optional<torch::Tensor> perm, bool accumulate,
             c10::optional<torch::Tensor> B0, c10::optional<torch::Tensor> colsum, bool exact) {
  CHECK_DEV(A); CHECK_DEV(B); CHECK_DEV(C);
  const bool f32 = A.scalar_type() == at::kFloat;
  TORCH_CHECK((A.scalar_type() == at::kBFloat16 || f32) && B.scalar_type() == A.scalar_type() &&
                  C.scalar_type() == at::kFloat, "gemm_tn: A, B both bf16 or both f32; C f32");
  TORCH_CHECK(A.dim() == 2 && B.dim() == 2 && C.dim() == 2 && A.stride(1) == 1 && B.stride(1) == 1 &&
              C.stride(1) == 1, "gemm_tn: 2-D operands with unit column stride");
  const int K = A.size(0), M = A.size(1), N = B.size(1);
  int split_rows = 0;
  const void* b0 = nullptr;
  if (B0 && B0->defined()) {
    CHECK_DEV(*B0);
    TORCH_CHECK(B0->scalar_type() == A.scalar_type() && B0->dim() == 2 && B0->size(1) == N && B0->stride(1) == 1 &&
                B0->stride(0) == B.stride(0), "gemm_tn: B0 must match B's dtype, columns and row stride");
    split_rows = B0->size(0);
    b0 = B0->data_ptr();
  }
  TORCH_CHECK(B.size(0) + split_rows == K, "gemm_tn: K mismatch between A and [B0; B]");
  const int al = f32 ? 4 : 8;
  TORCH_CHECK(M % 8 == 0 && N % 8 == 0 && A.stride(0) % al == 0 && B.stride(0) % al == 0,
              "gemm_tn: M, N multiples of 8 and row strides 16-B aligned");
  TORCH_CHECK((reinterpret_cast<uintptr_t>(A.data_ptr()) & 15) == 0 && (reinterpret_cast<uintptr_t>(B.data_ptr()) & 15) == 0 &&
              (b0 == nullptr || (reinterpret_cast<uintptr_t>(b0) & 15) == 0), "gemm_tn: operands must be 16-B aligned");
  const int* pp = nullptr;
  int64_t crow = M;
  if (perm && perm->defined()) {
    CHECK_I32(*perm);
    TORCH_CHECK(perm->numel() == M, "gemm_tn: perm must have M entries");
    pp = ptr<int>(*perm);
    crow = C.size(0);
  }
  TORCH_CHECK(C.size(0) >= crow && C.size(1) == N, "gemm_tn: C shape");
  float* csp = nullptr;
  if (colsum && colsum->defined()) {
    CHECK_F32(*colsum);
    TORCH_CHECK(colsum->numel() >= crow, "gemm_tn: colsum must have one entry per C row");
    csp = ptr<float>(*colsum);
  }
  if (K == 0) {
    if (!accumulate) {
      C.zero_();
      if (csp) colsum->zero_();
    }
    return;
  }
  int splits, kc, tiles;
  TORCH_CHECK(!exact || f32, "gemm_tn: exact mode needs fp32 operands");
  const int mode = exact ? 2 : (f32 ? 1 : 0);
  dca_gemm_tn_plan(M, N, K, &splits, &kc, &tiles, mode);
  torch::Tensor slab;
  if (splits > 1) slab = torch::empty({(int64_t)splits * M * N + (csp ? (int64_t)splits * M : 0)}, C.options());
  hip_check(dca_gemm_tn(A.data_ptr(), (int)A.stride(0), B.data_ptr(), (int)B.stride(0), b0, split_rows,
                        ptr<float>(C), (int)C.stride(0), pp, accumulate ? 1 : 0, M, N, K,
                        splits > 1 ? ptr<float>(slab) : nullptr, csp, cur_stream(), mode),
            "dca_gemm_tn");
}

std::vector<torch::Tensor> enc_small_grads(torch::Tensor z, torch::Tensor dtl, torch::Tensor type_off, torch::Tensor dx,
                                           torch::Tensor env, torch::Tensor we, torch::Tensor be, bool compat) {
// ... 2 lines not shown
  const int N = z.size(0), U = dtl.size(1);
  TORCH_CHECK(dtl.size(0) == N && dx.size(0) == N && dx.size(1) == 896 && env.size(0) == N && env.size(1) == 3 &&
              we.size(0) == 128 && we.size(1) == 3 && be.numel() == 128 && type_off.numel() == 7,
              "enc_small_grads shapes");
  auto o = z.options();
  auto part = torch::empty({(int64_t)dca_enc_small_blocks() * dca_enc_small_out()}, o);
  auto out = torch::empty({(int64_t)dca_enc_small_out()}, o);
  hip_check(dca_enc_small_grads(ptr<float>(z), (int)z.stride(0), ptr<float>(dtl), U, ptr<int>(type_off),
                                ptr<float>(dx), ptr<float>(env), ptr<float>(we), ptr<float>(be), N, compat ? 1 : 0,
                                ptr<float>(part), ptr<float>(out), cur_stream()),
            "dca_enc_small_grads");
  return {out.narrow(0, 0, 768).view({6, 128}), out.narrow(0, 768, 384).view({128, 3}), out.narrow(0, 1152, 128)};
}

std::vector<torch::Tensor> split_bf16x2(torch::Tensor src, bool slab_major) {
  CHECK_F32(src);
  TORCH_CHECK(src.numel() % 4 == 0, "split_bf16x2: numel % 4 == 0");
  if (slab_major) {
    TORCH_CHECK(src.dim() == 2 && src.size(1) % 32 == 0, "split_bf16x2: slab-major images need (R, K), K % 32 == 0");
    const int R = src.size(0), K = src.size(1);
    auto hi = torch::empty({K / 32, R, 32}, src.options().dtype(at::kBFloat16));
    auto lo = torch::empty({K / 32, R, 32}, src.options().dtype(at::kBFloat16));
    hip_check(dca_split_bf16x2_blk(ptr<float>(src), ptr<short>(hi), ptr<short>(lo), R, K, cur_stream()),
              "dca_split_bf16x2_blk");
    return {hi, lo};
  }
  auto hi = torch::empty(src.sizes(), src.options().dtype(at::kBFloat16));
  auto lo = torch::empty(src.sizes(), src.options().dtype(at::kBFloat16));
  hip_check(dca_split_bf16x2(ptr<float>(src), ptr<short>(hi), ptr<short>(lo), src.numel(), cur_stream()),
            "dca_split_bf16x2");
  return {hi, lo};
}

std::vector<torch::Tensor> dpre_dx(torch::Tensor dG, torch::Tensor w1h, torch::Tensor w1l, torch::Tensor x,
                                   torch::Tensor w2h, torch::Tensor w2l) {
  CHECK_F32(dG); CHECK_F32(x); CHECK_DEV(w1h); CHECK_CONTIG(w1h); CHECK_DEV(w2h); CHECK_CONTIG(w2h);
  const bool exact = w1h.scalar_type() == at::kFloat;
  if (exact) {
    TORCH_CHECK(w2h.scalar_type() == at::kFloat, "dpre_dx: both weights fp32 (exact) or bf16 hi/lo pairs");
  } else {
    CHECK_DT(w1h, at::kBFloat16); CHECK_DT(w2h, at::kBFloat16); CHECK_DEV(w1l); CHECK_CONTIG(w1l);
    CHECK_DEV(w2l); CHECK_CONTIG(w2l); CHECK_DT(w1l, at::kBFloat16); CHECK_DT(w2l, at::kBFloat16);
    TORCH_CHECK(w1l.sizes() == w1h.sizes() && w2l.sizes() == w2h.sizes(), "dpre_dx: hi / lo image shapes");
  }
  const int N = dG.size(0), K1 = dG.size(1);
  TORCH_CHECK(dG.dim() == 2 && x.dim() == 2, "dpre_dx: 2-D dG and x");
  int X;
  if (exact) {
    TORCH_CHECK(w1h.dim() == 2 && w2h.dim() == 2, "dpre_dx: exact weights (256,K1) (X,256)");
    X = w2h.size(0);
    TORCH_CHECK(w1h.size(0) == 256 && w1h.size(1) == K1 && w2h.size(1) == 256, "dpre_dx: shapes (256,K1) (X,256)");
  } else {
    TORCH_CHECK(w1h.dim() == 3 && w2h.dim() == 3 && w1h.size(0) * 32 == K1 && w1h.size(1) == 256 &&
                w1h.size(2) == 32 && w2h.size(0) == 8 && w2h.size(2) == 32,
                "dpre_dx: bf16x3 weights are slab-major images (K1/32,256,32) and (8,X,32)");
    X = w2h.size(1);
  }
  TORCH_CHECK(x.size(0) == N && x.size(1) == 256, "dpre_dx: x (N,256)");
  TORCH_CHECK(K1 % 128 == 0 && X % 128 == 0, "dpre_dx: K1 % 128 == 0 and X % 128 == 0");
  TORCH_CHECK((long long)N * K1 * 4 <= 0x7fff0000LL, "dpre_dx: dG too large for one launch");
  auto o = dG.options();
  auto dpre = torch::empty({N, 256}, o);
  auto dx = torch::empty({N, X}, o);
  hip_check(dca_dpre_dx(ptr<float>(dG), w1h.data_ptr(), exact ? nullptr : w1l.data_ptr(), ptr<float>(x),
                        w2h.data_ptr(), exact ? nullptr : w2l.data_ptr(), ptr<float>(dpre), ptr<float>(dx), N, K1, X,
                        exact ? 1 : 0, 0, cur_stream()),
            "dca_dpre_dx");
  return {dpre, dx};
}

static bool chain_exact(const torch::Tensor& wh, const torch::Tensor& wl, const char* what) {
  CHECK_DEV(wh); CHECK_CONTIG(wh);
  if (wh.scalar_type() == at::kFloat) {
    TORCH_CHECK(wh.dim() == 2 && wl.numel() == 0, what, ": exact weights are 2-D fp32 with an empty lo image");
    return true;
  }
  CHECK_BF16(wh); CHECK_BF16(wl);
  TORCH_CHECK(wl.sizes() == wh.sizes(), what, ": hi / lo image shapes");
  return false;
}

torch::Tensor rowmm_out256(torch::Tensor A, torch::Tensor wh, torch::Tensor wl, torch::Tensor bias) {
  CHECK_F32(A); CHECK_F32(bias);
  const bool exact = chain_exact(wh, wl, "rowmm_out256");
  const int N = A.size(0), K = A.size(1);
  TORCH_CHECK(A.dim() == 2 && K % 128 == 0 && bias.numel() == 256, "rowmm_out256: A (N, K % 128 == 0), bias (256)");
  if (exact) {
    TORCH_CHECK(wh.size(0) == 256 && wh.size(1) == K, "rowmm_out256: exact W (256, K)");
  } else {
    TORCH_CHECK(wh.dim() == 3 && wh.size(0) * 32 == K && wh.size(1) == 256 && wh.size(2) == 32,
                "rowmm_out256: slab-major images (K/32, 256, 32)");
  }
  TORCH_CHECK((long long)N * K * 4 <= 0x7fff0000LL, "rowmm_out256: A too large for one launch");
  auto out = torch::empty({N, 256}, A.options());
  hip_check(dca_dpre_dx(ptr<float>(A), wh.data_ptr(), exact ? nullptr : wl.data_ptr(), ptr<float>(bias), nullptr,
                        nullptr, ptr<float>(out), nullptr, N, K, 0, exact ? 1 : 0, 2, cur_stream()),
            "dca_dpre_dx(stage 1)");
  return out;
}

torch::Tensor rowmm_in256(torch::Tensor A, torch::Tensor wh, torch::Tensor wl) {
  CHECK_F32(A);
  const bool exact = chain_exact(wh, wl, "rowmm_in256");
  const int N = A.size(0);
  TORCH_CHECK(A.dim() == 2 && A.size(1) == 256, "rowmm_in256: A (N, 256)");
  int X;
  if (exact) {
    TORCH_CHECK(wh.size(1) == 256 && wh.size(0) % 128 == 0, "rowmm_in256: exact W (X, 256), X % 128 == 0");
    X = wh.size(0);
  } else {
    TORCH_CHECK(wh.dim() == 3 && wh.size(0) == 8 && wh.size(2) == 32 && wh.size(1) % 128 == 0,
                "rowmm_in256: slab-major images (8, X, 32), X % 128 == 0");
    X = wh.size(1);
  }
  auto out = torch::empty({N, X}, A.options());
  hip_check(dca_dpre_dx(ptr<float>(A), nullptr, nullptr, nullptr, wh.data_ptr(), exact ? nullptr : wl.data_ptr(),
                        nullptr, ptr<float>(out), N, 0, X, exact ? 1 : 0, 0, cur_stream()),
            "dca_dpre_dx(stage 2)");
  return out;
}

std::vector<torch::Tensor> pre_rnn_chain(torch::Tensor x896, torch::Tensor w1h, torch::Tensor w1l, torch::Tensor bias,
                                         torch::Tensor w2h, torch::Tensor w2l, c10::optional<torch::Tensor> x_out,
                                         c10::optional<torch::Tensor> xp_out) {
  CHECK_F32(x896); CHECK_F32(bias);
  const bool exact = chain_exact(w1h, w1l, "pre_rnn_chain");
  TORCH_CHECK(chain_exact(w2h, w2l, "pre_rnn_chain") == exact, "pre_rnn_chain: both weights exact or both bf16x3");
  const int N = x896.size(0), K1 = x896.size(1);
  TORCH_CHECK(x896.dim() == 2 && bias.numel() == 256, "pre_rnn_chain: x896 (N, K1), bias (256)");
  int X;
  if (exact) {
    TORCH_CHECK(w1h.size(0) == 256 && w1h.size(1) == K1 && w2h.size(1) == 256, "pre_rnn_chain: exact W_pre (256, K1), "
                "W_ih (X, 256)");
    X = w2h.size(0);
  } else {
    TORCH_CHECK(w1h.dim() == 3 && w1h.size(0) * 32 == K1 && w1h.size(1) == 256 && w1h.size(2) == 32 &&
                w2h.dim() == 3 && w2h.size(0) == 8 && w2h.size(2) == 32,
                "pre_rnn_chain: slab-major images (K1/32,256,32) and (8,X,32)");
    X = w2h.size(1);
  }
  TORCH_CHECK(K1 % 128 == 0 && X % 128 == 0, "pre_rnn_chain: K1 % 128 == 0 and X % 128 == 0");
  TORCH_CHECK((long long)N * K1 * 4 <= 0x7fff0000LL, "pre_rnn_chain: x896 too large for one launch");
  auto o = x896.options();
  auto x = out_or_new(x_out, {N, 256}, o, "x_out");
  auto xp = out_or_new(xp_out, {N, X}, o, "xp_out");
  hip_check(dca_dpre_dx(ptr<float>(x896), w1h.data_ptr(), exact ? nullptr : w1l.data_ptr(), ptr<float>(bias),
                        w2h.data_ptr(), exact ? nullptr : w2l.data_ptr(), ptr<float>(x), ptr<float>(xp), N, K1, X,
                        exact ? 1 : 0, 1, cur_stream()),
            "dca_dpre_dx(forward)");
  return {x, xp};
}


std::vector<torch::Tensor> replay_gather(std::vector<torch::Tensor> pools, int64_t n_step, torch::Tensor idx) {
  CHECK_DEV(idx); CHECK_CONTIG(idx); CHECK_DT(idx, at::kLong);
  TORCH_CHECK(!pools.empty() && pools.size() <= 12, "replay_gather: 1..12 fields");
  const int B = idx.numel();
  const int S = n_step > 0 ? pools[0].size(1) : 1;
  std::vector<torch::Tensor> out;
  std::vector<const void*> src;
  std::vector<void*> dst;
  std::vector<long long> rb;
  std::vector<int> ps;
  for (size_t i = 0; i < pools.size(); ++i) {
    const torch::Tensor& p = pools[i];
    CHECK_DEV(p); CHECK_CONTIG(p);
    const bool step = (int64_t)i < n_step;
    TORCH_CHECK(!step || (p.dim() >= 2 && p.size(1) == S), "replay_gather: per-step pools must be (capacity, S, ...)");
    std::vector<int64_t> shape;
    if (step) {
      shape.push_back((int64_t)S * B);
      for (int d = 2; d < p.dim(); ++d) shape.push_back(p.size(d));
    } else {
      shape.push_back(B);
      for (int d = 1; d < p.dim(); ++d) shape.push_back(p.size(d));
    }
    auto o = torch::empty(shape, p.options());
    const int64_t per = step ? p.numel() / (p.size(0) * S) : p.numel() / p.size(0);
    src.push_back(p.data_ptr());
    dst.push_back(o.data_ptr());
    rb.push_back((long long)(per * p.element_size()));
    ps.push_back(step ? 1 : 0);
    out.push_back(o);
  }
  hip_check(dca_replay_gather(src.data(), dst.data(), rb.data(), ps.data(), (int)pools.size(), ptr<long long>(idx), S,
                              B, cur_stream()),
            "dca_replay_gather");
  return out;
}

}

PYBIND11_MODULE(TORCH_EXTENSION_NAME, m) {
  m.doc() = "dotaclient_amd gfx950 HIP kernels";
  m.def("adam_step", &adam_step, "fused global-norm clip + Adam over a flat fp32 buffer (divide: grad holds DP sums, "
        "averaged by the has-grad counts in-kernel)", py::arg("param"), py::arg("grad"), py::arg("m"), py::arg("v"),
        py::arg("seg"), py::arg("counts"), py::arg("steps"), py::arg("norm_out"), py::arg("lr"), py::arg("b1"),
        py::arg("b2"), py::arg("eps"), py::arg("max_norm"), py::arg("divide") = false, py::arg("header") = 0,
        py::arg("skip") = py::none(), py::arg("nonfinite") = py::none());
  m.def("ingest_scatter", &ingest_scatter, "packed valid rows -> zero-padded rows of every field + validity mask");
  m.def("adv_normalize", &adv_normalize, "PPO advantage normalisation over the valid rows (one workgroup)");
  m.def("multi_copy", &multi_copy, "dst_i <- src_i (same byte sizes, contiguous, 16-B aligned) in one launch");
  m.def("multi_axpy", &multi_axpy, "dst_i += scale * src_i for a list of fp32 tensors (one graph-safe launch)",
        py::arg("dst"), py::arg("src"), py::arg("scale") = py::none());
  m.def("lstm_team_ctl_bytes", &dca_lstm_team_ctl_bytes, "bytes of a persistent team-LSTM control block");
  m.def("heads_loss", &heads_loss, "fused heads + pointer + masked log-softmax + PPO/VPG loss + gradients",
        py::arg("z"), py::arg("emb"), py::arg("act"), py::arg("msk"), py::arg("adv"), py::arg("ret"),
        py::arg("logp_old"), py::arg("nret"), py::arg("norms"), py::arg("algo"), py::arg("compat_value_bug"),
        py::arg("S_bug"), py::arg("B_bug"), py::arg("clip_eps"), py::arg("ent_coef"), py::arg("vf_coef"),
        py::arg("dz_bf16") = false, py::arg("precise") = false);
  m.def("encoder_fwd", &encoder_fwd, "fused entity encoder forward (unit MLP, per-type GEMM, max-pool+argmax)",
        py::arg("units"), py::arg("env"), py::arg("w1"), py::arg("b1"), py::arg("wt"), py::arg("bt"), py::arg("we"),
        py::arg("be"), py::arg("counts"), py::arg("compat"), py::arg("exact") = false,
        py::arg("x896_out") = py::none(), py::arg("emb_out") = py::none(), py::arg("arg_out") = py::none());
  m.def("encoder_bwd", &encoder_bwd, "fused entity encoder backward: dW_type (K-blocked split-K MFMA GEMM), dW1, db1",
        py::arg("units"), py::arg("w1"), py::arg("b1"), py::arg("wtT"), py::arg("dtl"), py::arg("q"), py::arg("dx"),
        py::arg("arg"), py::arg("counts"), py::arg("compat"), py::arg("demb_in") = py::none(),
        py::arg("exact") = false);
  m.def("lstm_team_fwd", &lstm_team_fwd, "XCD-team persistent LSTM forward (L2-local hand-off), unit-major gates",
        py::arg("xp4"), py::arg("whh"), py::arg("h0"), py::arg("c0"), py::arg("err"), py::arg("ctl"),
        py::arg("want_f32_h"), py::arg("trace") = py::none(), py::arg("time_major") = false, py::arg("hs_out") = py::none(),
        py::arg("cs_out") = py::none(), py::arg("gates_out") = py::none(), py::arg("bias4") = py::none(),
        py::arg("precise") = false, py::arg("reset") = py::none());
  m.def("lstm_team_bwd", &lstm_team_bwd, "XCD-team persistent LSTM backward (L2-local reduce-scatter)",
        py::arg("dhs"), py::arg("gates4"), py::arg("cs"), py::arg("c0"), py::arg("dhn"), py::arg("dcn"),
        py::arg("whh"), py::arg("err"), py::arg("ctl"), py::arg("trace") = py::none(),
        py::arg("time_major") = false, py::arg("dg_out") = py::none(), py::arg("dg_bf16") = false,
        py::arg("want_dbias") = false, py::arg("precise") = false, py::arg("reset") = py::none());
  m.def("lstm_team_chains", [](int64_t B, bool f32) { return dca_lstm_team_chains((int)B, f32 ? 1 : 0); },
        "sequence chains of a team-recurrence launch of B sequences", py::arg("B"), py::arg("f32"));
  m.def("sample_actions", &sample_actions, "fused masked hierarchical Gumbel-max action sampling (actor)");
  m.def("actor_state_prep", &actor_state_prep, "actor step: state resets + [x | bf16(h)] gate-GEMM operand",
        py::arg("pre"), py::arg("h"), py::arg("c"), py::arg("keep"), py::arg("xh"), py::arg("bump") = py::none());
  m.def("lstm_cell", &lstm_cell, "LSTM cell nonlinearity from fp32 gates (actor single step)", py::arg("gates"),
        py::arg("h"), py::arg("c"), py::arg("h16"), py::arg("active") = py::none());
  m.def("encoder_fp8", &encoder_fp8, "fp8 (e4m3) entity encoder of the actor step: unit MLP, per-type GEMMs, pools "
        "(per_unit: the one-unit-at-a-time workgroup form instead of the wave-parallel one)", py::arg("units"),
        py::arg("env"), py::arg("w1"), py::arg("b1"), py::arg("wt"), py::arg("st"), py::arg("bt"), py::arg("we"),
        py::arg("be"), py::arg("counts"), py::arg("per_unit") = false);
  m.def("actor_core", &actor_core, "fp32 / bf16 actor policy core: pre-RNN + LSTM step (or linear layer) + heads",
        py::arg("x896"), py::arg("wpre"), py::arg("bpre"), py::arg("wg"), py::arg("bg"), py::arg("wh"), py::arg("bh"),
        py::arg("h"), py::arg("c"), py::arg("keep"), py::arg("z"), py::arg("mode"), py::arg("linear") = false,
        py::arg("active") = py::none(), py::arg("bump") = py::none());
  m.def("actor_fp8", &actor_fp8, "fp8 (e4m3) actor policy core: pre-RNN + LSTM step + heads from x896",
        py::arg("x896"), py::arg("wpre"), py::arg("spre"), py::arg("bpre"), py::arg("wg"), py::arg("sg"), py::arg("bg"),
        py::arg("wh"), py::arg("sh"), py::arg("bh"), py::arg("h"), py::arg("c"), py::arg("keep"), py::arg("z"),
        py::arg("active") = py::none(), py::arg("bump") = py::none());
  m.def("attn_block_fwd", &attn_block_fwd, "fused fp32 entity-attention block forward: LN + QKV + attention + "
        "out-projection + residual + pools (-> xn, mean, rstd, qkv, o, lse, e1)");
  m.def("attn_block_bwd", &attn_block_bwd, "fused fp32 entity-attention block backward: demb + dO + attention "
        "backward + dXn + LayerNorm backward (-> de1, dqkv, de0, [dgamma | dbeta | dbt])");
    m.def("loss_prep", &loss_prep, "loss normalisers from one-hot action rows (graph-replayable)");
  m.def("loss_prep_ws_elems", &loss_prep_ws_elems, "int32 workspace elements of loss_prep");
  m.def("loss_assemble", &loss_assemble, "loss scalar + metrics from heads/loss partials", py::arg("part"),
        py::arg("norms"), py::arg("N"), py::arg("algo"), py::arg("ent_coef"), py::arg("vf_coef"), py::arg("out"),
        py::arg("S") = 0, py::arg("compat_value_bug") = false);
  m.def("weight_prep", &weight_prep, "gather the flat fp32 params into bf16 / fp32 working weight images (+ bf16 "
        "hi / lo split images)", py::arg("src"), py::arg("map16"), py::arg("dst16"), py::arg("map32"), py::arg("dst32"),
        py::arg("maps") = py::none(), py::arg("dsth") = py::none(), py::arg("dstl") = py::none());
  m.def("gemm_tn", &gemm_tn, "C (+)= A^T B for K-outer bf16 or fp32 (bf16x3) operands (split-K MFMA, LDS transposed reads)",
        py::arg("A"), py::arg("B"), py::arg("C"), py::arg("perm") = py::none(), py::arg("accumulate") = false,
        py::arg("B0") = py::none(), py::arg("colsum") = py::none(), py::arg("exact") = false);
  m.def("dpre_dx", &dpre_dx, "fused pre-RNN dX chain: (dG·W_ih)*[x>0] -> dpre, dpre·W_pre -> dx (bf16x3 with pre-split "
        "bf16 hi/lo weights, or exact-f32 MFMA with fp32 weights)", py::arg("dG"), py::arg("w1h"), py::arg("w1l"),
        py::arg("x"), py::arg("w2h"), py::arg("w2l"));
  m.def("pre_rnn_chain", &pre_rnn_chain, "fused forward chain x = relu(x896·W_pre^T + b), xp = x·W_ih^T (bf16x3)",
        py::arg("x896"), py::arg("w1h"), py::arg("w1l"), py::arg("bias"), py::arg("w2h"), py::arg("w2l"),
        py::arg("x_out") = py::none(), py::arg("xp_out") = py::none());
  m.def("rowmm_out256", &rowmm_out256, "C (N,256) = A (N,K)·W^T + b on the chain kernel's stage 1 (bf16x3)",
        py::arg("A"), py::arg("wh"), py::arg("wl"), py::arg("bias"));
  m.def("rowmm_in256", &rowmm_in256, "C (N,X) = A (N,256)·W^T on the chain kernel's stage 2 (bf16x3)", py::arg("A"),
        py::arg("wh"), py::arg("wl"));
  m.def("split_bf16x2", &split_bf16x2, "fp32 -> (hi, lo) bf16 images with x = hi + lo (slab_major: (R,K) -> "
        "[K/32][R][32] images, the dpre_dx operand layout)", py::arg("src"), py::arg("slab_major") = false);
  m.def("enc_small_grads", &enc_small_grads, "entity-encoder type-bias and env-layer gradients in one pass");
  m.def("replay_gather", &replay_gather, "minibatch gather from an HBM replay pool into time-major rows (one launch)");
  m.def("vtrace_step", &vtrace_step, "V-trace advantages / value targets of a minibatch from the step's own values",
        py::arg("z"), py::arg("vcol"), py::arg("lp"), py::arg("mu"), py::arg("vt"), py::arg("B"), py::arg("S"),
        py::arg("gamma"), py::arg("lam"), py::arg("rho_bar") = 1.0, py::arg("c_bar") = 1.0);
  m.def("featurize_raw", &featurize_raw, "GPU unit featurization from raw unit records (featurize.hip)",
        py::arg("raw"), py::arg("hero"), py::arg("units"), py::arg("handles") = py::none());
  m.def("occupy_xcd", &occupy_xcd, "test utility: hold CUs of one XCD for a while (160 KB LDS per workgroup)",
        py::arg("xcd"), py::arg("blocks"), py::arg("seconds"), py::arg("like"));
  m.def("returns_scan", &returns_scan, "segmented reverse scan: discounted returns / GAE / V-trace GAE + per-team EMA "
        "normalisation (positional: ..., factor, eps, lr or None, rho_bar, c_bar)");
}
```

### dotaclient_amd/ops/csrc/glue.hip

```cpp
#include "common.h"

namespace {

constexpr int kPrepThreads = 256;
constexpr int kPrepBlocks = 256;

__global__ __launch_bounds__(kPrepThreads) void loss_prep_kernel(const unsigned char* __restrict__ act, int N, int A,
                                                                 int* __restrict__ partial,
                                                                 unsigned* __restrict__ counter,
                                                                 float* __restrict__ norms) {
  const int lane = threadIdx.x & 63, w = threadIdx.x >> 6;
  const int nw = gridDim.x * (kPrepThreads / dca::kWave);
  const unsigned long long m_enum = 0x7ull, m_x = 0x1ffull << 3, m_y = 0x1ffull << 12;
  const unsigned long long m_t = ~(m_enum | m_x | m_y);
  int c[5] = {0, 0, 0, 0, 0};
  for (int r = blockIdx.x * (kPrepThreads / dca::kWave) + w; r < N; r += nw) {
    const unsigned char* row = act + (size_t)r * A;
    const bool v0 = lane < A && row[lane] != 0;
    const bool v1 = lane + 64 < A && row[lane + 64] != 0;
    const unsigned long long b0 = __ballot(v0), b1 = __ballot(v1);
    c[0] += (b0 | b1) != 0ull;
    c[1] += __popcll(b0 & m_enum);
    c[2] += __popcll(b0 & m_x);
    c[3] += __popcll(b0 & m_y);
    c[4] += __popcll(b0 & m_t) + __popcll(b1);
  }
  __shared__ int red[kPrepThreads / dca::kWave][5];
  __shared__ bool last;
  if (lane == 0)
    for (int i = 0; i < 5; ++i) red[w][i] = c[i];
  __syncthreads();
  if (threadIdx.x < 5) {
    int v = 0;
#pragma unroll
    for (int k = 0; k < kPrepThreads / dca::kWave; ++k) v += red[k][threadIdx.x];
    partial[blockIdx.x * 5 + threadIdx.x] = v;
  }
  __syncthreads();
  if (threadIdx.x == 0) {
    __threadfence();
    const unsigned t = __hip_atomic_fetch_add(counter, 1u, __ATOMIC_ACQ_REL, __HIP_MEMORY_SCOPE_AGENT);
    last = (t == gridDim.x - 1);
  }
  __syncthreads();
  if (!last) return;
  __threadfence();
  __shared__ int fold[kPrepBlocks][5];
  for (int b = threadIdx.x; b < kPrepBlocks; b += kPrepThreads)
    for (int i = 0; i < 5; ++i)
      fold[b][i] = b < (int)gridDim.x
                       ? __hip_atomic_load(partial + b * 5 + i, __ATOMIC_RELAXED, __HIP_MEMORY_SCOPE_AGENT) : 0;
  __syncthreads();
  for (int o = kPrepBlocks / 2; o > 0; o >>= 1) {
    for (int b = threadIdx.x; b < o; b += kPrepThreads)
      for (int i = 0; i < 5; ++i) fold[b][i] += fold[b + o][i];
    __syncthreads();
  }
  if (threadIdx.x < 5) red[0][threadIdx.x] = fold[0][threadIdx.x];
  __syncthreads();
  if (threadIdx.x == 0) {
    auto inv = [](long long x) { return x > 0 ? 1.f / (float)x : 0.f; };
    const long long n_valid = red[0][0];
    long long tot = 0;
    for (int h = 0; h < 4; ++h) tot += red[0][1 + h];
    norms[0] = inv(n_valid);
    norms[1] = inv(tot);
    for (int h = 0; h < 4; ++h) norms[2 + h] = inv(red[0][1 + h]);
    norms[6] = 0.f;
    norms[7] = 0.f;
    __hip_atomic_store(counter, 0u, __ATOMIC_RELAXED, __HIP_MEMORY_SCOPE_AGENT);
  }
}

constexpr int kAsmThreads = 1024;

__global__ __launch_bounds__(kAsmThreads) void loss_assemble_kernel(const float* __restrict__ part, int nrows,
                                                                    const float* __restrict__ norms, int N, int algo,
                                                                    float ent_coef, float vf_coef,
                                                                    float* __restrict__ out, int S, int vbug) {
  const int t = threadIdx.x, col = t & 15, rg = t >> 4;
  float s = 0.f;
  int r = rg;
  for (; r + 7 * 64 < nrows; r += 8 * 64) {
    float v[8];
#pragma unroll
    for (int k = 0; k < 8; ++k) v[k] = part[(size_t)(r + k * 64) * 16 + col];
#pragma unroll
    for (int k = 0; k < 8; ++k) s += v[k];
  }
  for (; r < nrows; r += 64) s += part[(size_t)r * 16 + col];
  __shared__ float red[64][17];
  red[rg][col] = s;
  __syncthreads();
  for (int o = 32; o > 0; o >>= 1) {
    if (rg < o) red[rg][col] += red[rg + o][col];
    __syncthreads();
  }
  if (t != 0) return;
  float p[16];
  for (int i = 0; i < 16; ++i) p[i] = red[0][i];
  float eh[4], ent = 0.f;
  for (int h = 0; h < 4; ++h) {
    eh[h] = p[2 + h] * norms[2 + h];
    ent += eh[h];
  }
  float pol, val, entl, adv, kl = 0.f, cf = 0.f;
  const float invN = 1.f / (float)(N > 0 ? N : 1);
  if (algo != 1) {
    pol = -p[0] * norms[0];
    val = vf_coef * p[1] * norms[0];
    entl = -ent_coef * ent;
    adv = p[8] * norms[0];
    kl = p[6] * norms[0];
    cf = p[7] * norms[0];
  } else {
    pol = p[0] * norms[1];
    entl = ent_coef > 0.f ? -ent_coef * ent : 0.f;
    val = vf_coef > 0.f ? vf_coef * p[1] * invN : 0.f;
    adv = p[8] * invN;
    if (vbug && vf_coef > 0.f && S > 0) {
      const float Sf = (float)S, Bf = (float)(N / S);
      val = vf_coef * (Sf * p[10] - 2.f * p[9] * norms[6] + (float)N * norms[7]) / (Bf * Sf * Sf);
      adv = p[9] * invN - norms[6] / Sf;
    }
  }
  out[0] = pol + val + entl;
  out[1] = pol;
  out[2] = entl;
  out[3] = val;
  out[4] = ent;
  out[5] = adv;
  out[6] = kl;
  out[7] = cf;
  for (int h = 0; h < 4; ++h) out[8 + h] = eh[h];
  for (int i = 12; i < 16; ++i) out[i] = 0.f;
}

__global__ __launch_bounds__(256) void weight_prep_kernel(const float* __restrict__ src, const int* __restrict__ map16,
                                                          short* __restrict__ dst16, int n16,
                                                          const int2* __restrict__ map32, float* __restrict__ dst32,
                                                          int n32, const int* __restrict__ maps,
                                                          short* __restrict__ dsth, short* __restrict__ dstl, int ns) {
  const int stride = gridDim.x * blockDim.x;
  for (int i = blockIdx.x * blockDim.x + threadIdx.x; i < ns; i += stride) {
    const int m = maps[i];
    const float v = m >= 0 ? src[m] : 0.f;
    const short h = dca::f2bf(v);
    dsth[i] = h;
    dstl[i] = dca::f2bf(v - dca::bf2f(h));
  }
  for (int i = blockIdx.x * blockDim.x + threadIdx.x; i < n16; i += stride) {
    const int m = map16[i];
    dst16[i] = dca::f2bf(m >= 0 ? src[m] : 0.f);
  }
  for (int i = blockIdx.x * blockDim.x + threadIdx.x; i < n32; i += stride) {
    const int2 m = map32[i];
    dst32[i] = (m.x >= 0 ? src[m.x] : 0.f) + (m.y >= 0 ? src[m.y] : 0.f);
  }
}

constexpr int kSgBlocks = 256;
constexpr int kSgPhases = 4;
constexpr int kSgRows = 32;
constexpr int kSgOut = 6 * 128 + 128 * 3 + 128;

__global__ __launch_bounds__(128 * kSgPhases) void enc_small_grads_kernel(const float* __restrict__ z, int ldz,
                                                              const float* __restrict__ dtl, int U,
                                                              const int* __restrict__ type_off,
                                                              const float* __restrict__ dx, const float* __restrict__ env,
                                                              const float* __restrict__ we, const float* __restrict__ be,
                                                              int N, int compat, float* __restrict__ part) {
  const int d = threadIdx.x & 127, ph = threadIdx.x >> 7;
  __shared__ float s_seg[kSgRows][6];
  __shared__ float s_env[kSgRows][3];
  __shared__ float red[kSgPhases - 1][kSgOut];
  float adbt[6] = {0.f, 0.f, 0.f, 0.f, 0.f, 0.f}, adwe[3] = {0.f, 0.f, 0.f}, adbe = 0.f;
  const float w0 = we[d * 3 + 0], w1 = we[d * 3 + 1], w2 = we[d * 3 + 2], bd = be[d];
  const int rows_per = (N + gridDim.x - 1) / gridDim.x;
  const int r_lo = blockIdx.x * rows_per, r_hi = min(N, r_lo + rows_per);
  for (int t0 = r_lo; t0 < r_hi; t0 += kSgRows) {
    const int nt = min(kSgRows, r_hi - t0);
    __syncthreads();
    for (int i = threadIdx.x; i < nt * 6; i += 128 * kSgPhases) {
      const int r = i / 6, ty = i % 6;
      const float* dr = dtl + (size_t)(t0 + r) * U;
      float sacc = 0.f;
      for (int u = type_off[ty]; u < type_off[ty + 1]; ++u) sacc += dr[u];
      s_seg[r][ty] = sacc;
    }
    for (int i = threadIdx.x; i < nt * 3; i += 128 * kSgPhases)
      s_env[i / 3][i % 3] = env[(size_t)(t0 + i / 3) * 3 + i % 3];
    __syncthreads();
    for (int r = ph; r < nt; r += kSgPhases) {
      const size_t n = t0 + r;
      const float q = z[n * ldz + d];
      const float* dxr = dx + n * 896;
      float pool[6];
#pragma unroll
      for (int ty = 0; ty < 6; ++ty) pool[ty] = dxr[128 + 128 * ty + d];
      if (compat) {
        pool[3] += pool[5];
        pool[5] = 0.f;
      }
#pragma unroll
      for (int ty = 0; ty < 6; ++ty) adbt[ty] += q * s_seg[r][ty] + pool[ty];
      const float e0 = s_env[r][0], e1 = s_env[r][1], e2 = s_env[r][2];
      const float pre = e0 * w0 + e1 * w1 + e2 * w2 + bd;
      const float de = pre > 0.f ? dxr[d] : 0.f;
      adwe[0] += de * e0;
      adwe[1] += de * e1;
      adwe[2] += de * e2;
      adbe += de;
    }
  }
  __syncthreads();
  if (ph > 0) {
    float* rr = red[ph - 1];
    for (int ty = 0; ty < 6; ++ty) rr[ty * 128 + d] = adbt[ty];
    for (int c = 0; c < 3; ++c) rr[768 + d * 3 + c] = adwe[c];
    rr[1152 + d] = adbe;
  }
  __syncthreads();
  if (ph == 0) {
    float* o = part + (size_t)blockIdx.x * kSgOut;
    for (int ty = 0; ty < 6; ++ty) {
      float v = adbt[ty];
      for (int k = 0; k < kSgPhases - 1; ++k) v += red[k][ty * 128 + d];
      o[ty * 128 + d] = v;
    }
    for (int c = 0; c < 3; ++c) {
      float v = adwe[c];
      for (int k = 0; k < kSgPhases - 1; ++k) v += red[k][768 + d * 3 + c];
      o[768 + d * 3 + c] = v;
    }
    float v = adbe;
    for (int k = 0; k < kSgPhases - 1; ++k) v += red[k][1152 + d];
    o[1152 + d] = v;
  }
}

__global__ __launch_bounds__(256) void enc_small_reduce(const float* __restrict__ part, int nblk,
                                                        float* __restrict__ out) {
  const int c = blockIdx.x * 64 + (threadIdx.x & 63), ph = threadIdx.x >> 6;
  float s = 0.f;
  if (c < kSgOut) {
    int b = ph;
    for (; b + 12 < nblk; b += 16) {
      const float v0 = part[(size_t)b * kSgOut + c], v1 = part[(size_t)(b + 4) * kSgOut + c];
      const float v2 = part[(size_t)(b + 8) * kSgOut + c], v3 = part[(size_t)(b + 12) * kSgOut + c];
      s += v0;
      s += v1;
      s += v2;
      s += v3;
    }
    for (; b < nblk; b += 4) s += part[(size_t)b * kSgOut + c];
  }
  __shared__ float red[4][64];
  red[ph][threadIdx.x & 63] = s;
  __syncthreads();
  if (ph == 0 && c < kSgOut) out[c] = ((red[0][threadIdx.x] + red[1][threadIdx.x]) + red[2][threadIdx.x]) +
                                       red[3][threadIdx.x];
}

constexpr int kMaxGather = 12;
struct GatherField {
  const char* src;
  char* dst;
  long long row_bytes;
  int per_step;
  int unit;
};
struct GatherArgs {
  GatherField f[kMaxGather];
  const long long* idx;
  int S, B;
};

template <typename T>
__device__ __forceinline__ void gather_rows(const GatherField& F, const long long* __restrict__ idx, int S, int B) {
  const long long wpr = F.row_bytes / (long long)sizeof(T);
  const long long rows = F.per_step ? (long long)S * B : B;
  const long long total = rows * wpr;
  const T* src = reinterpret_cast<const T*>(F.src);
  T* dst = reinterpret_cast<T*>(F.dst);
  for (long long i = (long long)blockIdx.x * blockDim.x + threadIdx.x; i < total; i += (long long)gridDim.x * blockDim.x) {
    const long long r = i / wpr, w = i - r * wpr;
    long long srow;
    if (F.per_step) {
      const long long t = r / B, b = r - t * B;
      srow = idx[b] * S + t;
    } else {
      srow = idx[r];
    }
    dst[r * wpr + w] = src[srow * wpr + w];
  }
}

__global__ __launch_bounds__(256) void replay_gather_kernel(GatherArgs a) {
  const GatherField& F = a.f[blockIdx.y];
  if (F.unit == 16) gather_rows<uint4>(F, a.idx, a.S, a.B);
  else if (F.unit == 4) gather_rows<unsigned>(F, a.idx, a.S, a.B);
  else gather_rows<unsigned char>(F, a.idx, a.S, a.B);
}

}

extern "C" hipError_t dca_replay_gather(const void* const* src, void* const* dst, const long long* row_bytes,
                                        const int* per_step, int nf, const long long* idx, int S, int B,
                                        hipStream_t st) {
  if (nf < 1 || nf > kMaxGather) return hipErrorInvalidValue;
  GatherArgs a{};
  for (int i = 0; i < nf; ++i) {
    const unsigned long long align = (unsigned long long)src[i] | (unsigned long long)dst[i];
    int unit = 1;
    if (row_bytes[i] % 16 == 0 && align % 16 == 0) unit = 16;
    else if (row_bytes[i] % 4 == 0 && align % 4 == 0) unit = 4;
    a.f[i] = GatherField{static_cast<const char*>(src[i]), static_cast<char*>(dst[i]), row_bytes[i], per_step[i], unit};
  }
  a.idx = idx;
  a.S = S;
  a.B = B;
  hipLaunchKernelGGL(replay_gather_kernel, dim3(256, nf), dim3(256), 0, st, a);
  DCA_CHECK_LAUNCH();
  return hipSuccess;
}

extern "C" int dca_enc_small_out() { return kSgOut; }
extern "C" int dca_enc_small_blocks() { return kSgBlocks; }

extern "C" hipError_t dca_enc_small_grads(const float* z, int ldz, const float* dtl, int U, const int* type_off,
                                          const float* dx, const float* env, const float* we, const float* be, int N,
                                          int compat, float* part, float* out, hipStream_t st) {
  hipLaunchKernelGGL(enc_small_grads_kernel, dim3(kSgBlocks), dim3(128 * kSgPhases), 0, st, z, ldz, dtl, U, type_off, dx, env, we,
                     be, N, compat, part);
  DCA_CHECK_LAUNCH();
  hipLaunchKernelGGL(enc_small_reduce, dim3((kSgOut + 63) / 64), dim3(256), 0, st, part, kSgBlocks, out);
  DCA_CHECK_LAUNCH();
  return hipSuccess;
}

extern "C" int dca_loss_prep_blocks() { return kPrepBlocks; }

extern "C" hipError_t dca_loss_prep(const unsigned char* act, int N, int A, int* partial, unsigned* counter,
                                    float* norms, hipStream_t st) {
  hipLaunchKernelGGL(loss_prep_kernel, dim3(kPrepBlocks), dim3(kPrepThreads), 0, st, act, N, A, partial, counter,
                     norms);
  DCA_CHECK_LAUNCH();
  return hipSuccess;
}

extern "C" hipError_t dca_loss_assemble(const float* part, int nrows, const float* norms, int N, int algo,
                                        float ent_coef, float vf_coef, float* out, int S, int vbug, hipStream_t st) {
  hipLaunchKernelGGL(loss_assemble_kernel, dim3(1), dim3(kAsmThreads), 0, st, part, nrows, norms, N, algo, ent_coef, vf_coef,
                     out, S, vbug);
  DCA_CHECK_LAUNCH();
  return hipSuccess;
}

extern "C" hipError_t dca_weight_prep(const float* src, const int* map16, short* dst16, int n16, const int* map32,
                                      float* dst32, int n32, const int* maps, short* dsth, short* dstl, int ns,
                                      hipStream_t st) {
  int n = n16 > n32 ? n16 : n32;
  if (ns > n) n = ns;
  int blocks = (n + 255) / 256;
  if (blocks > 2048) blocks = 2048;
  if (blocks < 1) blocks = 1;
  hipLaunchKernelGGL(weight_prep_kernel, dim3(blocks), dim3(256), 0, st, src, map16, dst16, n16,
                     reinterpret_cast<const int2*>(map32), dst32, n32, maps, dsth, dstl, ns);
  DCA_CHECK_LAUNCH();
  return hipSuccess;
}

namespace {
constexpr int kOccupyLds = 160 * 1024;
__global__ __launch_bounds__(64) void occupy_xcd_kernel(int xcd, unsigned long long ticks, int* seen) {
  extern __shared__ __attribute__((aligned(16))) float occ_lds[];
  const unsigned x = __builtin_amdgcn_s_getreg((3 << 11) | 20) & 0xf;
  if ((int)x != xcd) {
    if (threadIdx.x == 0) seen[blockIdx.x] = 0;
    return;
  }
  const unsigned long long t0 = __builtin_amdgcn_s_memrealtime();
  occ_lds[threadIdx.x] = 0.f;
  while (__builtin_amdgcn_s_memrealtime() - t0 < ticks) __builtin_amdgcn_s_sleep(127);
  if (threadIdx.x == 0) seen[blockIdx.x] = (int)x + 1 + (int)occ_lds[threadIdx.x];
}
}

extern "C" hipError_t dca_occupy_xcd(int xcd, int blocks, double seconds, int* seen, hipStream_t st) {
  if (blocks < 1 || blocks > 4096 || seconds <= 0.0 || seconds > 10.0) return hipErrorInvalidValue;
  static bool attr = false;
  if (!attr) {
    hipError_t e = hipFuncSetAttribute(reinterpret_cast<const void*>(occupy_xcd_kernel),
                                       hipFuncAttributeMaxDynamicSharedMemorySize, kOccupyLds);
    if (e != hipSuccess) return e;
    attr = true;
  }
  const unsigned long long ticks = (unsigned long long)(seconds * 1e8);
  hipLaunchKernelGGL(occupy_xcd_kernel, dim3(blocks), dim3(64), kOccupyLds, st, xcd, ticks, seen);
  DCA_CHECK_LAUNCH();
  return hipSuccess;
}
```

### dotaclient_amd/ops/csrc/heads_loss.hip

```cpp
#include "common.h"

namespace {

constexpr int kRowsPerBlock = 4;
constexpr int kQ = 128;
constexpr int kNPart = 16;

struct Params {
  const float* z; int ldz;
  const void* emb;
  const unsigned char* act; const unsigned char* msk; int A;
  const float* adv; const float* ret; const float* logp_old; const float* nret;
  const float* norms;
  float* dz; float* dtl; float* part; float* logp_out;
  short* dz16;
  int N, U, algo, compat_value_bug, S_bug, B_bug;
  float clip_eps, ent_coef, vf_coef;
};

__device__ __forceinline__ void put_dz(const Params& P, size_t i, float v) {
  if (P.dz16) P.dz16[i] = dca::f2bf(v);
  else P.dz[i] = v;
}

template <bool PRECISE>
__device__ __forceinline__ float xexp(float x) { return PRECISE ? expf(x) : __expf(x); }
template <bool PRECISE>
__device__ __forceinline__ float xlog(float x) { return PRECISE ? logf(x) : __logf(x); }

template <bool PRECISE>
__device__ __forceinline__ void head_lsm(float logit, bool m, int lane, int W, float& logp, float& p) {
  const bool in = lane < W;
  const float v = (in && m) ? logit : -INFINITY;
  float mx = dca::wave_max(v);
  const bool any = mx > -INFINITY;
  if (!any) mx = 0.f;
  const float e = (in && m) ? xexp<PRECISE>(logit - mx) : 0.f;
  float s = dca::wave_sum(e);
  if (!(s > 0.f)) s = 1.f;
  logp = logit - mx - xlog<PRECISE>(s);
  p = (in && m) ? (PRECISE ? e / s : xexp<PRECISE>(logp)) : 0.f;
}

template <bool F32, bool PRECISE>
__global__ __launch_bounds__(256) void heads_loss_kernel(Params P) {
  const int tid = threadIdx.x, wv = tid >> 6, lane = tid & 63;
  const int n = blockIdx.x * kRowsPerBlock + wv;
  __shared__ float s_tl[kRowsPerBlock][64];
  __shared__ float s_dtl[kRowsPerBlock][64];
  __shared__ float s_part[kRowsPerBlock][kNPart];
  __shared__ float s_zl[kRowsPerBlock][32];
  __shared__ unsigned char s_act[kRowsPerBlock][128];
  __shared__ unsigned char s_msk[kRowsPerBlock][128];
  float acc[kNPart];
#pragma unroll
  for (int i = 0; i < kNPart; ++i) acc[i] = 0.f;

  if (n < P.N) {
    const int U = P.U;
    const float* zr = P.z + (size_t)n * P.ldz;
    const int ks = lane & 15, ug = lane >> 4;
    float q8[8];
    {
      const float4 a = *reinterpret_cast<const float4*>(zr + 8 * ks);
      const float4 b = *reinterpret_cast<const float4*>(zr + 8 * ks + 4);
      q8[0] = a.x; q8[1] = a.y; q8[2] = a.z; q8[3] = a.w; q8[4] = b.x; q8[5] = b.y; q8[6] = b.z; q8[7] = b.w;
    }
    const float zl = zr[kQ + min(lane, 21)];
    const float A_n = P.adv[n], R_n = P.ret[n], lpo_n = P.logp_old[n], nret_n = P.nret[n];
    float nm[8];
#pragma unroll
    for (int i = 0; i < 8; ++i) nm[i] = P.norms[i];
    const unsigned char* ar = P.act + (size_t)n * P.A;
    const unsigned char* mr = P.msk + (size_t)n * P.A;
    const unsigned char a0 = ar[min(lane, P.A - 1)], a1 = ar[min(lane + 64, P.A - 1)];
    const unsigned char m0 = mr[min(lane, P.A - 1)], m1 = mr[min(lane + 64, P.A - 1)];
    constexpr int kMaxIt = 16;
    float e8[kMaxIt][8];
    const int nit = (U + 3) >> 2;
#pragma unroll
    for (int it = 0; it < kMaxIt; ++it)
      if (it < nit) {
        const size_t o = ((size_t)n * U + min(it * 4 + ug, U - 1)) * kQ + 8 * ks;
        if constexpr (F32) {
          const float4 a = *reinterpret_cast<const float4*>(static_cast<const float*>(P.emb) + o);
          const float4 b = *reinterpret_cast<const float4*>(static_cast<const float*>(P.emb) + o + 4);
          e8[it][0] = a.x; e8[it][1] = a.y; e8[it][2] = a.z; e8[it][3] = a.w;
          e8[it][4] = b.x; e8[it][5] = b.y; e8[it][6] = b.z; e8[it][7] = b.w;
        } else {
          const dca::bf16x8 h = *reinterpret_cast<const dca::bf16x8*>(static_cast<const short*>(P.emb) + o);
#pragma unroll
          for (int j = 0; j < 8; ++j) e8[it][j] = dca::bf2f(h[j]);
        }
      }
    if (lane < 32) s_zl[wv][lane] = zl;
    s_act[wv][lane] = a0; s_act[wv][lane + 64] = a1;
    s_msk[wv][lane] = m0; s_msk[wv][lane + 64] = m1;
#pragma unroll
    for (int it = 0; it < kMaxIt; ++it) {
      if (it < nit) {
        const int u = it * 4 + ug;
        float d = 0.f;
#pragma unroll
        for (int j = 0; j < 8; ++j) d += q8[j] * e8[it][j];
        d = dca::group_sum<16>(d);
        if (ks == 0 && u < U) s_tl[wv][u] = d;
      }
    }
    __builtin_amdgcn_wave_barrier();
    __builtin_amdgcn_fence(__ATOMIC_RELEASE, "wavefront");
    const int hoff[4] = {0, 3, 12, 21};
    const int hw[4] = {3, 9, 9, U};
    float logp[4], pr[4], a[4];
    bool mk[4];
    float sel = 0.f;
    int nsel = 0;
#pragma unroll
    for (int h = 0; h < 4; ++h) {
      const bool in = lane < hw[h];
      float lg = 0.f;
      if (in) lg = (h == 3) ? s_tl[wv][lane] : s_zl[wv][hoff[h] + lane];
      mk[h] = in && s_msk[wv][hoff[h] + lane];
      a[h] = (in && s_act[wv][hoff[h] + lane]) ? 1.f : 0.f;
      head_lsm<PRECISE>(lg, mk[h], lane, hw[h], logp[h], pr[h]);
      if (!in) logp[h] = 0.f;
      const float sh = dca::wave_sum(a[h] * logp[h]);
      sel += sh;
      const int ns = __popcll(__ballot(a[h] > 0.f));
      nsel += ns;
      acc[2 + h] += -dca::wave_sum(mk[h] ? pr[h] * logp[h] : 0.f);
    }
    const float valid = nsel > 0 ? 1.f : 0.f;
    const float V = s_zl[wv][21];
    const float R = R_n;
    float g_sel = 0.f, dV = 0.f;
    if (P.algo == 0) {
      const float A = A_n;
      const float lr = sel - lpo_n;
      const float r = xexp<PRECISE>(lr);
      const float s1 = r * A;
      const float rc = fminf(fmaxf(r, 1.f - P.clip_eps), 1.f + P.clip_eps);
      const float s2 = rc * A;
      acc[0] += valid * fminf(s1, s2);
      const bool clipped = (A > 0.f && r > 1.f + P.clip_eps) || (A < 0.f && r < 1.f - P.clip_eps);
      g_sel = clipped ? 0.f : -valid * A * r * nm[0];
      acc[1] += valid * (V - R) * (V - R);
      dV = P.vf_coef * 2.f * (V - R) * valid * nm[0];
      acc[6] += valid * (-lr);
      acc[7] += valid * (fabsf(r - 1.f) > P.clip_eps ? 1.f : 0.f);
      acc[8] += valid * A;
    } else if (P.algo == 2) {
      const float A = A_n;
      const float lr = sel - lpo_n;
      const float r = xexp<PRECISE>(lr);
      const float w = fminf(r, 1.f);
      acc[0] += valid * w * A;
      g_sel = -valid * A * w * nm[0];
      acc[1] += valid * (V - R) * (V - R);
      dV = P.vf_coef * 2.f * (V - R) * valid * nm[0];
      acc[6] += valid * (-lr);
      acc[7] += valid * (r > 1.f ? 1.f : 0.f);
      acc[8] += valid * A;
    } else {
      const float nr = nret_n;
      acc[0] += -sel * nr;
      g_sel = -nr * nm[1];
      acc[1] += (V - R) * (V - R);
      acc[9] += V;
      acc[10] += V * V;
      acc[8] += V - R;
      if (P.vf_coef > 0.f) {
        if (P.compat_value_bug) {
          const float S = (float)P.S_bug, Bq = (float)P.B_bug;
          dV = P.vf_coef * 2.f * (S * V - nm[6]) / (Bq * S * S);
        } else {
          dV = P.vf_coef * 2.f * (V - R) / ((float)P.S_bug * (float)P.B_bug);
        }
      }
    }
    acc[11] += valid;
    if (P.logp_out) if (lane == 0) P.logp_out[n] = sel;
#pragma unroll
    for (int h = 0; h < 4; ++h) {
      const bool in = lane < hw[h];
      float dlp = g_sel * a[h];
      if (P.ent_coef > 0.f) dlp += P.ent_coef * nm[2 + h] * (mk[h] ? pr[h] * (1.f + logp[h]) : 0.f);
      if (!in) dlp = 0.f;
      const float sd = dca::wave_sum(dlp);
      const float dl = dlp - (mk[h] ? pr[h] : 0.f) * sd;
      if (in) {
        if (h == 3) {
          s_dtl[wv][lane] = dl;
          P.dtl[(size_t)n * U + lane] = dl;
        } else {
          put_dz(P, (size_t)n * P.ldz + kQ + hoff[h] + lane, dl);
        }
      }
    }
    if (lane == 0) put_dz(P, (size_t)n * P.ldz + kQ + 21, dV);
    for (int c = kQ + 22 + lane; c < P.ldz; c += 64) put_dz(P, (size_t)n * P.ldz + c, 0.f);
    __builtin_amdgcn_wave_barrier();
    __builtin_amdgcn_fence(__ATOMIC_RELEASE, "wavefront");
    float dq[8] = {0.f, 0.f, 0.f, 0.f, 0.f, 0.f, 0.f, 0.f};
#pragma unroll
    for (int it = 0; it < kMaxIt; ++it) {
      if (it < nit) {
        const int u = it * 4 + ug;
        const float g = (u < U) ? s_dtl[wv][u] : 0.f;
#pragma unroll
        for (int j = 0; j < 8; ++j) dq[j] += g * e8[it][j];
      }
    }
#pragma unroll
    for (int j = 0; j < 8; ++j) {
      dq[j] += __shfl_xor(dq[j], 16, 64);
      dq[j] += __shfl_xor(dq[j], 32, 64);
    }
    if (ug == 0) {
      if (P.dz16) {
        dca::bf16x8 h;
#pragma unroll
        for (int j = 0; j < 8; ++j) h[j] = dca::f2bf(dq[j]);
        *reinterpret_cast<dca::bf16x8*>(P.dz16 + (size_t)n * P.ldz + 8 * ks) = h;
      } else {
        float4* o = reinterpret_cast<float4*>(P.dz + (size_t)n * P.ldz + 8 * ks);
        o[0] = make_float4(dq[0], dq[1], dq[2], dq[3]);
        o[1] = make_float4(dq[4], dq[5], dq[6], dq[7]);
      }
    }
  }
  if (lane == 0) {
#pragma unroll
    for (int i = 0; i < kNPart; ++i) s_part[wv][i] = acc[i];
  }
  __syncthreads();
  if (tid < kNPart) {
    float s = 0.f;
#pragma unroll
    for (int w = 0; w < kRowsPerBlock; ++w) s += s_part[w][tid];
    P.part[(size_t)blockIdx.x * kNPart + tid] = s;
  }
}

}

extern "C" int dca_heads_loss_nblocks(int N) { return (N + kRowsPerBlock - 1) / kRowsPerBlock; }

extern "C" hipError_t dca_heads_loss(const float* z, int ldz, const void* emb, const unsigned char* act,
                                     const unsigned char* msk, int A, const float* adv, const float* ret,
                                     const float* logp_old, const float* nret, const float* norms, float* dz,
                                     float* dtl, float* part, float* logp_out, int N, int U, int algo,
                                     int compat_value_bug, int S_bug, int B_bug, float clip_eps, float ent_coef,
                                     float vf_coef, hipStream_t st, short* dz16, int emb_f32, int precise) {
  if (U > 64 || U < 1 || ldz < kQ + 22 || A != 21 + U) return hipErrorInvalidValue;
  Params P{z, ldz, emb, act, msk, A, adv, ret, logp_old, nret, norms, dz, dtl, part, logp_out, dz16, N, U, algo,
           compat_value_bug, S_bug, B_bug, clip_eps, ent_coef, vf_coef};
  if (emb_f32 && precise) heads_loss_kernel<true, true><<<dca_heads_loss_nblocks(N), 256, 0, st>>>(P);
  else if (emb_f32) heads_loss_kernel<true, false><<<dca_heads_loss_nblocks(N), 256, 0, st>>>(P);
  else heads_loss_kernel<false, false><<<dca_heads_loss_nblocks(N), 256, 0, st>>>(P);
  return hipGetLastError();
}
```

### dotaclient_amd/ops/csrc/launchers.h

```cpp
#pragma once
#include <hip/hip_runtime.h>
#include <stdint.h>

extern "C" {

hipError_t dca_split_bf16x2(const float* src, short* hi, short* lo, long long n, hipStream_t stream);
hipError_t dca_split_bf16x2_blk(const float* src, short* hi, short* lo, int R, int K, hipStream_t stream);
hipError_t dca_attn_block_fwd_f32(const float* e0, const float* bout, const float* gamma, const float* beta,
                                  const void* wqh, const void* wql, const float* bq, const void* woh,
                                  const void* wol, float* xn, float* mu, float* rs, float* qkv, float* o, float* lse,
                                  float* e1, float* x896, unsigned char* arg, const int* off, int compat, int N,
                                  float eps, hipStream_t stream, int exact);
int dca_attn_block_bwd_groups(int N);
hipError_t dca_attn_block_bwd_f32(const float* dtl, const float* q, int ldq, const float* dx, const unsigned char* arg,
                                  const int* off, int compat, const float* o, const float* qkv, const float* bq,
                                  const float* lse, const float* e0, const float* bout, const float* mu,
                                  const float* rs, const float* gamma, const void* woth, const void* wotl,
                                  const void* wq4h, const void* wq4l, float* de1, float* dqkv, float* de0,
                                  float* part, float* tmp, float* sums, int N, hipStream_t stream,
                                  unsigned long long* trace, int exact);
hipError_t dca_actor_fp8(const short* x896, const void* wpre, const float* spre, const float* bpre, const void* wg,
                         const float* sg, const float* bg, const void* wh, const float* sh, const float* bh, float* h,
                         float* c, const float* keep, const float* active, float* z, int n, long long* bump,
                         hipStream_t stream);
hipError_t dca_encoder_fp8(const void* units, int f16, const float* env, const float* w1, const float* b1,
                           const void* wt, const float* st, const float* bt, const float* we, const float* be,
                           short* x896, short* emb, int N, int U, const int* counts, int per_unit,
                           hipStream_t stream);

hipError_t dca_dpre_dx(const float* dG, const void* w1h, const void* w1l, const float* x, const void* w2h,
                       const void* w2l, float* dpre, float* dx, int N, int K1, int X, int exact, int epi, hipStream_t stream);

hipError_t dca_adam_step(float* param, const float* grad, float* m, float* v, const int* seg, int64_t n,
                         const float* counts, float* steps, int n_params, float* partials, float* norm_out, float lr,
                         float b1, float b2, float eps, float max_norm, hipStream_t st, int divide, int64_t header,
                         const float* skip, float* nonfinite);
int dca_adam_partials_len(int n_params);

hipError_t dca_ingest_scatter(void* const* dst, const void* const* src, const int* row_bytes, int n, const int* inv,
                              int L, int nsrc, float* valid, hipStream_t st);
hipError_t dca_adv_normalize(const float* adv, const float* valid, float* out, int L, float eps, hipStream_t st);
hipError_t dca_multi_copy(void* const* dst, const void* const* src, const long long* bytes, int n, hipStream_t st);
hipError_t dca_multi_axpy(float* const* dst, const float* const* src, const long long* numel, int n,
                          const float* scale, hipStream_t st);

int dca_heads_loss_nblocks(int N);
hipError_t dca_heads_loss(const float* z, int ldz, const void* emb, const unsigned char* act, const unsigned char* msk,
                          int A, const float* adv, const float* ret, const float* logp_old, const float* nret,
                          const float* norms, float* dz, float* dtl, float* part, float* logp_out, int N, int U,
                          int algo, int compat_value_bug, int S_bug, int B_bug, float clip_eps, float ent_coef,
                          float vf_coef, hipStream_t st, short* dz16, int emb_f32, int precise = 0);

hipError_t dca_encoder_fwd(const float* units, const float* env, const float* w1, const float* b1, const void* wt,
                           const float* bt, const float* we, const float* be, void* x896, void* emb,
                           unsigned char* arg, int N, int U, const int* counts, int compat, hipStream_t st, int f32);
size_t dca_encoder_bwd_workspace(int N, int U, const int* counts, int f32);
hipError_t dca_encoder_bwd(const float* units, const float* w1, const float* b1, const void* wtT, const float* dtl,
                           const float* q, int ldq, const float* dx, const unsigned char* arg, float* dwt, float* dw1,
                           float* db1, void* ws, size_t ws_bytes, int N, int U, const int* counts, int compat,
                           hipStream_t st, const void* demb_in, int f32);

size_t dca_lstm_team_ctl_bytes();
size_t dca_lstm_team_workspace(int B, int H, int backward, int f32);
hipError_t dca_lstm_team_fwd(const float* xp4, const void* whh, const float* h0, const float* c0, short* hs,
                             float* hsf, float* cs, float* gates4, float* hn, float* cn, void* ctl, void* ws,
                             size_t ws_bytes, unsigned* err, int B, int S, int H, int time_major, hipStream_t st,
                             unsigned long long* trace, const float* bias4, int f32, int precise = 0,
                             const unsigned char* rst = nullptr);
int dca_lstm_team_chains(int B, int f32);
hipError_t dca_lstm_team_bwd(const float* dhs, const float* gates4, const float* cs, const float* c0,
                             const float* dhn, const float* dcn, const void* whh, float* dgates4, float* dh0,
                             float* dc0, void* ctl, void* ws, size_t ws_bytes, unsigned* err, int B, int S, int H,
                             int time_major, hipStream_t st, unsigned long long* trace, short* dg16, float* dbpart,
                             int f32, int precise = 0, const unsigned char* rst = nullptr);

hipError_t dca_sample_actions(const float* z, int ldz, const void* emb, int emb_f32, const void* handles, int h32,
                              int N, int U, unsigned long long seed, const long long* ctr, int* idx,
                              unsigned char* act, unsigned char* msk, float* logp, float* value, hipStream_t st);
hipError_t dca_actor_core(const void* x896, int x_f32, const void* wpre, const float* bpre, const void* wg,
                          const float* bg, const void* wh, const float* bh, float* h, float* c, const float* keep,
                          const float* active, float* z, int n, int hidden, int linear, int mode, long long* bump,
                          hipStream_t st);
hipError_t dca_actor_state_prep(const short* pre, float* h, float* c, const float* keep, short* xh, int N, int P,
                                int H, long long* bump, hipStream_t st);
hipError_t dca_lstm_cell(const float* gates, float* h, float* c, short* h16, const float* active, int N, int H,
                         hipStream_t st);

hipError_t dca_vtrace_step(const float* z, int ldz, int vcol, const float* lp, const float* mu, const float* vt,
                           float* adv, float* ret, float* stats, int B, int S, float gamma, float lam, float rho_bar,
                           float c_bar, hipStream_t st);
hipError_t dca_returns(const float* rew, int K, const float* val, const float* lr, const int* off, const int* seglen,
                       const float* boot, const unsigned char* done, const int* keys, int nseg, int max_len,
                       float* ret, float* adv, float* norm, float* stats, const float* ema_in, float* ema_out,
                       int mode, int normalize, float gamma, float lam, float rho_bar, float c_bar, float factor,
                       float eps, hipStream_t st);

int dca_loss_prep_blocks();
hipError_t dca_loss_prep(const unsigned char* act, int N, int A, int* partial, unsigned* counter, float* norms,
                         hipStream_t st);
hipError_t dca_occupy_xcd(int xcd, int blocks, double seconds, int* seen, hipStream_t st);
hipError_t dca_featurize_raw(const void* raw, const float* hero, void* units, void* handles, int rows, int U,
                             int half_out, hipStream_t st);
hipError_t dca_featurize_raw16(const void* raw16, const float* hero, void* units, void* handles, int rows, int U,
                               hipStream_t st);
hipError_t dca_loss_assemble(const float* part, int nrows, const float* norms, int N, int algo, float ent_coef,
                             float vf_coef, float* out, int S, int vbug, hipStream_t st);
hipError_t dca_weight_prep(const float* src, const int* map16, short* dst16, int n16, const int* map32, float* dst32,
                           int n32, const int* maps, short* dsth, short* dstl, int ns, hipStream_t st);

void dca_gemm_tn_plan(int M, int N, int K, int* splits, int* kc, int* tiles, int f32);
hipError_t dca_gemm_tn(const void* A, int lda, const void* B, int ldb, const void* B0, int split_rows, float* C,
                       int ldc, const int* perm, int accumulate, int M, int N, int K, float* slab, float* colsum,
                       hipStream_t st, int f32);

int dca_enc_small_out();
int dca_enc_small_blocks();
hipError_t dca_enc_small_grads(const float* z, int ldz, const float* dtl, int U, const int* type_off, const float* dx,
                               const float* env, const float* we, const float* be, int N, int compat, float* part,
                               float* out, hipStream_t st);

hipError_t dca_replay_gather(const void* const* src, void* const* dst, const long long* row_bytes, const int* per_step,
                             int nf, const long long* idx, int S, int B, hipStream_t st);

}
```

Measured before the change: 2.006 million.

## Fuse replay gather, grad zeroing and weight prep into one step prologue kernel

Adds a step_prologue launch that performs the replay minibatch gather, zero-fills the flat gradient buffer and builds the bf16/fp32 weight images in a single kernel. It also lets loss_prep read action rows directly from the replay pool through the index vector on a side stream, so train_direct skips its own loss_prep and weight refresh. Separately, the heads/loss kernel gains a template specialisation with fewer unit iterations for U<=40. The aim is to cut per-step launch count and small-kernel overhead inside the captured graph, at the cost of a more complex combined kernel and a dependency on the side-stream ordering.

```diff
diff --git a/dotaclient_amd/learner/engine.py b/dotaclient_amd/learner/engine.py
--- a/dotaclient_amd/learner/engine.py
+++ b/dotaclient_amd/learner/engine.py
@@ -177,16 +177,20 @@
                 out[k] = batch[k].contiguous()
         return out, B, S
 
-    def gather_time_major(self, replay, idx, S: int):
+    def gather_time_major(self, replay, idx, S: int, prologue: bool = False):
         B = idx.numel()
         fields = self.STEP_FIELDS + tuple(k for k in ('reset', 'vt') if k in replay.data)
         if idx.is_cuda:
             from .. import ops
             seq = [k for k in ('h0', 'c0') if k in replay.data]
-            outs = ops.require().replay_gather([replay.data[k] for k in fields] +
-                                               [replay.data[k] for k in seq], len(fields),
-                                               idx.contiguous())
+            pools = [replay.data[k] for k in fields] + [replay.data[k] for k in seq]
+            if prologue:
+                outs = self.model.step_prologue(pools, len(fields), idx.contiguous(), replay.data['actions'],
+                                                self.flat.grad, self.cfg)
+            else:
+                outs = ops.require().replay_gather(pools, len(fields), idx.contiguous())
             return dict(zip(list(fields) + seq, outs))
+        assert not prologue
         ar = getattr(self, '_arange', None)
         if ar is None or ar.numel() < S or ar.device != idx.device:
             ar = self._arange = torch.arange(max(S, 1), device=idx.device, dtype=torch.long)
@@ -213,13 +217,18 @@
             self._split = bool(ok)
         return self._split
 
-    def _direct_body(self, batch_tm, B, S, hook=None):
-        self.flat.grad.zero_()
+    def _fused_prologue(self) -> bool:
+        import os
+        return os.environ.get('DCA_STEP_PROLOGUE', '1') != '0' and not self._split_mode()
+
+    def _direct_body(self, batch_tm, B, S, hook=None, prologue_done: bool = False):
+        if not prologue_done:
+            self.flat.grad.zero_()
         if hook is None and self._split_mode():
             hook = self.dp.launch_early
         self.model.split_hook = hook
         try:
-            vec = self.model.train_direct(batch_tm, B, S, self.cfg)
+            vec = self.model.train_direct(batch_tm, B, S, self.cfg, prologue_done=prologue_done)
         finally:
             self.model.split_hook = None
         self.dp.has_grad.copy_(self.model.grad_mask)
@@ -363,7 +372,9 @@
             vec = self._replay_split(key, lambda hook: self._direct_body(
                 self.gather_time_major(replay, sidx, S), B, S, hook=hook))
         else:
-            vec = self._replay_graph(key, lambda: self._direct_body(self.gather_time_major(replay, sidx, S), B, S))
+            fused = self._fused_prologue()
+            vec = self._replay_graph(key, lambda: self._direct_body(
+                self.gather_time_major(replay, sidx, S, prologue=fused), B, S, prologue_done=fused))
         return self._finish(vec)
 
     def _sync_and_step(self):
diff --git a/dotaclient_amd/models/fused.py b/dotaclient_amd/models/fused.py
--- a/dotaclient_amd/models/fused.py
+++ b/dotaclient_amd/models/fused.py
@@ -75,13 +75,30 @@
     def loss_prep_ws(self, device):
         return self.scratch('loss_prep_ws', (int(self.C.loss_prep_ws_elems()),), torch.int32, device)
 
-    def train_direct(self, batch_tm, B: int, S: int, cfg=None) -> torch.Tensor:
+    def train_direct(self, batch_tm, B: int, S: int, cfg=None, prologue_done: bool = False) -> torch.Tensor:
         from .pipelined import train_direct
         if cfg is not None:
             self.loss_cfg = cfg
         self.refresh()
         self.direct_used = False
-        return train_direct(self, batch_tm, B, S)
+        return train_direct(self, batch_tm, B, S, prologue_done=prologue_done)
+
+    def step_prologue(self, pools, n_step: int, idx, pool_actions, grad, cfg=None):
+        if cfg is not None:
+            self.loss_cfg = cfg
+        self.refresh()
+        wi = self.weight_images()
+        dev = grad.device
+        main = torch.cuda.current_stream(dev)
+        sL = self.side_stream()
+        ev = torch.cuda.Event()
+        ev.record(main)
+        outs = self.C.step_prologue(pools, n_step, idx, grad, wi.flat, wi.map16, wi.buf16, wi.map32, wi.buf32,
+                                    wi.mapS, wi.bufH, wi.bufL)
+        sL.wait_event(ev)
+        with torch.cuda.stream(sL):
+            self.C.loss_prep(pool_actions, self.loss_prep_ws(dev), self.scratch('norms', (8,), torch.float32, dev), idx)
+        return outs
 
     def forward_logp_value(self, batch_tm, B: int, S: int):
         from .pipelined import forward_logp_value
diff --git a/dotaclient_amd/models/pipelined.py b/dotaclient_amd/models/pipelined.py
--- a/dotaclient_amd/models/pipelined.py
+++ b/dotaclient_amd/models/pipelined.py
@@ -551,7 +551,7 @@
         return (None,) * (14 + len(ctx.fp.param_names))
 
 
-def train_direct(fp, batch_tm: Dict[str, torch.Tensor], B: int, S: int) -> torch.Tensor:
+def train_direct(fp, batch_tm: Dict[str, torch.Tensor], B: int, S: int, prologue_done: bool = False) -> torch.Tensor:
     C = fp.C
     lc = fp.loss_cfg
     N = B * S
@@ -561,11 +561,12 @@
     sL = fp.side_stream()
     sL.wait_stream(main)
     with torch.cuda.stream(sL):
-        C.loss_prep(batch_tm['actions'], fp.loss_prep_ws(dev), norms)
+        if not prologue_done:
+            C.loss_prep(batch_tm['actions'], fp.loss_prep_ws(dev), norms)
         if lc.compat_value_bug and lc.vf_coef > 0:
             g_last = batch_tm['ret'].view(S, B)[:, B - 1]
             norms[6:8] = torch.stack([g_last.sum(), (g_last * g_last).sum()])
-    W = fp.weight_images().refresh(C)
+    W = fp.weight_images().views if prologue_done else fp.weight_images().refresh(C)
     P = dict(zip(fp.param_names, fp.params))
     H = fp.cfg.hidden
     h0 = batch_tm.get('h0')
diff --git a/dotaclient_amd/ops/csrc/bindings.cpp b/dotaclient_amd/ops/csrc/bindings.cpp
--- a/dotaclient_amd/ops/csrc/bindings.cpp
+++ b/dotaclient_amd/ops/csrc/bindings.cpp
@@ -251,7 +251,7 @@
                                       torch::Tensor adv, torch::Tensor ret, torch::Tensor logp_old,
                                       torch::Tensor nret, torch::Tensor norms, int64_t algo, bool compat_value_bug,
                                       int64_t S_bug, int64_t B_bug, double clip_eps, double ent_coef,
-                                      double vf_coef, bool dz_bf16, bool precise) {
+                                      double vf_coef, bool dz_bf16, bool precise, int64_t wide) {
   CHECK_F32(z); CHECK_DEV(emb); CHECK_CONTIG(emb); CHECK_U8(act); CHECK_U8(msk); CHECK_F32(adv); CHECK_F32(ret);
   CHECK_F32(logp_old); CHECK_F32(nret); CHECK_F32(norms);
   const bool ef32 = emb.scalar_type() == at::kFloat;
@@ -273,7 +273,7 @@
                            ptr<float>(norms), dz_bf16 ? nullptr : ptr<float>(dz), ptr<float>(dtl), ptr<float>(part),
                            ptr<float>(logp), N, U, (int)algo, compat_value_bug ? 1 : 0, (int)S_bug, (int)B_bug,
                            (float)clip_eps, (float)ent_coef, (float)vf_coef, cur_stream(),
-                           dz_bf16 ? ptr<short>(dz) : nullptr, ef32 ? 1 : 0, precise && ef32 ? 1 : 0),
+                           dz_bf16 ? ptr<short>(dz) : nullptr, ef32 ? 1 : 0, precise && ef32 ? 1 : 0, (int)wide),
             "dca_heads_loss");
   return {dz, dtl, part, logp};
 }
@@ -658,14 +658,25 @@
   ema.copy_(ema_out);
 }
 
-void loss_prep(torch::Tensor act, torch::Tensor ws, torch::Tensor norms) {
+void loss_prep(torch::Tensor act, torch::Tensor ws, torch::Tensor norms, c10::optional<torch::Tensor> idx) {
   CHECK_U8(act); CHECK_I32(ws); CHECK_F32(norms);
-  TORCH_CHECK(act.dim() == 2 && act.size(1) >= 22 && act.size(1) <= 128, "act must be (N, 21+U), U <= 107");
+  const bool pool = idx && idx->defined();
+  TORCH_CHECK(act.dim() == (pool ? 3 : 2), "act must be (N, 21+U), or the pool's (capacity, S, 21+U) with idx");
+  const int A = act.size(-1);
+  TORCH_CHECK(A >= 22 && A <= 128, "act rows must be 21+U wide, U <= 107");
   const int nb = dca_loss_prep_blocks();
   TORCH_CHECK(ws.numel() >= 5 * nb + 1 && norms.numel() >= 8, "loss_prep: workspace / norms too small");
   int* w = ptr<int>(ws);
-  hip_check(dca_loss_prep(ptr<unsigned char>(act), (int)act.size(0), (int)act.size(1), w,
-                          reinterpret_cast<unsigned*>(w + 5 * nb), ptr<float>(norms), cur_stream()),
+  int N = act.size(0), S = 0, B = 0;
+  const long long* ip = nullptr;
+  if (pool) {
+    CHECK_DEV(*idx); CHECK_CONTIG(*idx); CHECK_DT(*idx, at::kLong);
+    S = act.size(1); B = idx->numel(); N = S * B;
+    TORCH_CHECK(B >= 1 && S >= 1, "loss_prep: empty minibatch");
+    ip = ptr<long long>(*idx);
+  }
+  hip_check(dca_loss_prep(ptr<unsigned char>(act), N, A, w, reinterpret_cast<unsigned*>(w + 5 * nb), ptr<float>(norms),
+                          cur_stream(), ip, S, B),
             "dca_loss_prep");
 }
 
@@ -974,16 +985,21 @@
 }
 
 
-std::vector<torch::Tensor> replay_gather(std::vector<torch::Tensor> pools, int64_t n_step, torch::Tensor idx) {
-  CHECK_DEV(idx); CHECK_CONTIG(idx); CHECK_DT(idx, at::kLong);
-  TORCH_CHECK(!pools.empty() && pools.size() <= 12, "replay_gather: 1..12 fields");
-  const int B = idx.numel();
-  const int S = n_step > 0 ? pools[0].size(1) : 1;
+struct GatherPlan {
   std::vector<torch::Tensor> out;
   std::vector<const void*> src;
   std::vector<void*> dst;
   std::vector<long long> rb;
   std::vector<int> ps;
+  int B, S;
+};
+
+GatherPlan gather_plan(const std::vector<torch::Tensor>& pools, int64_t n_step, const torch::Tensor& idx) {
+  CHECK_DEV(idx); CHECK_CONTIG(idx); CHECK_DT(idx, at::kLong);
+  TORCH_CHECK(!pools.empty() && pools.size() <= 12, "replay_gather: 1..12 fields");
+  GatherPlan g;
+  const int B = g.B = idx.numel();
+  const int S = g.S = n_step > 0 ? pools[0].size(1) : 1;
   for (size_t i = 0; i < pools.size(); ++i) {
     const torch::Tensor& p = pools[i];
     CHECK_DEV(p); CHECK_CONTIG(p);
@@ -999,16 +1015,46 @@
     }
     auto o = torch::empty(shape, p.options());
     const int64_t per = step ? p.numel() / (p.size(0) * S) : p.numel() / p.size(0);
-    src.push_back(p.data_ptr());
-    dst.push_back(o.data_ptr());
-    rb.push_back((long long)(per * p.element_size()));
-    ps.push_back(step ? 1 : 0);
-    out.push_back(o);
-  }
-  hip_check(dca_replay_gather(src.data(), dst.data(), rb.data(), ps.data(), (int)pools.size(), ptr<long long>(idx), S,
-                              B, cur_stream()),
+    g.src.push_back(p.data_ptr());
+    g.dst.push_back(o.data_ptr());
+    g.rb.push_back((long long)(per * p.element_size()));
+    g.ps.push_back(step ? 1 : 0);
+    g.out.push_back(o);
+  }
+  return g;
+}
+
+std::vector<torch::Tensor> replay_gather(std::vector<torch::Tensor> pools, int64_t n_step, torch::Tensor idx) {
+  GatherPlan g = gather_plan(pools, n_step, idx);
+  hip_check(dca_replay_gather(g.src.data(), g.dst.data(), g.rb.data(), g.ps.data(), (int)pools.size(),
+                              ptr<long long>(idx), g.S, g.B, cur_stream()),
             "dca_replay_gather");
-  return out;
+  return g.out;
+}
+
+std::vector<torch::Tensor> step_prologue(std::vector<torch::Tensor> pools, int64_t n_step, torch::Tensor idx,
+                                         torch::Tensor zero, torch::Tensor src, torch::Tensor map16,
+                                         torch::Tensor dst16, torch::Tensor map32, torch::Tensor dst32,
+                                         c10::optional<torch::Tensor> maps, c10::optional<torch::Tensor> dsth,
+                                         c10::optional<torch::Tensor> dstl) {
+  GatherPlan g = gather_plan(pools, n_step, idx);
+  CHECK_F32(zero); CHECK_F32(src); CHECK_I32(map16); CHECK_BF16(dst16); CHECK_I32(map32); CHECK_F32(dst32);
+  TORCH_CHECK(map16.numel() == dst16.numel() && map32.numel() == 2 * dst32.numel(), "step_prologue: map sizes");
+  const int* ms = nullptr;
+  short *dh = nullptr, *dl = nullptr;
+  int ns = 0;
+  if (maps && maps->defined()) {
+    TORCH_CHECK(dsth && dsth->defined() && dstl && dstl->defined(), "step_prologue: split map needs both hi / lo outputs");
+    CHECK_I32(*maps); CHECK_BF16(*dsth); CHECK_BF16(*dstl);
+    TORCH_CHECK(maps->numel() == dsth->numel() && dstl->numel() == dsth->numel(), "step_prologue: split map sizes");
+    ms = ptr<int>(*maps); dh = ptr<short>(*dsth); dl = ptr<short>(*dstl); ns = (int)maps->numel();
+  }
+  hip_check(dca_step_prologue(g.src.data(), g.dst.data(), g.rb.data(), g.ps.data(), (int)pools.size(),
+                              ptr<long long>(idx), g.S, g.B, ptr<float>(zero), (long long)zero.numel(), ptr<float>(src),
+                              ptr<int>(map16), ptr<short>(dst16), (int)dst16.numel(), ptr<int>(map32),
+                              ptr<float>(dst32), (int)dst32.numel(), ms, dh, dl, ns, cur_stream()),
+            "dca_step_prologue");
+  return g.out;
 }
 
 }
@@ -1030,7 +1076,9 @@
         py::arg("z"), py::arg("emb"), py::arg("act"), py::arg("msk"), py::arg("adv"), py::arg("ret"),
         py::arg("logp_old"), py::arg("nret"), py::arg("norms"), py::arg("algo"), py::arg("compat_value_bug"),
         py::arg("S_bug"), py::arg("B_bug"), py::arg("clip_eps"), py::arg("ent_coef"), py::arg("vf_coef"),
-        py::arg("dz_bf16") = false, py::arg("precise") = false);
+        py::arg("dz_bf16") = false, py::arg("precise") = false, py::arg("wide") = -1);
+  m.def("heads_loss_resident_blocks", &dca_heads_loss_resident_blocks,
+        "workgroups of the heads + loss kernel (U <= 40) resident on the device at once (4 rows each)");
   m.def("encoder_fwd", &encoder_fwd, "fused entity encoder forward (unit MLP, per-type GEMM, max-pool+argmax)",
         py::arg("units"), py::arg("env"), py::arg("w1"), py::arg("b1"), py::arg("wt"), py::arg("bt"), py::arg("we"),
         py::arg("be"), py::arg("counts"), py::arg("compat"), py::arg("exact") = false,
@@ -1072,7 +1120,8 @@
         "out-projection + residual + pools (-> xn, mean, rstd, qkv, o, lse, e1)");
   m.def("attn_block_bwd", &attn_block_bwd, "fused fp32 entity-attention block backward: demb + dO + attention "
         "backward + dXn + LayerNorm backward (-> de1, dqkv, de0, [dgamma | dbeta | dbt])");
-    m.def("loss_prep", &loss_prep, "loss normalisers from one-hot action rows (graph-replayable)");
+    m.def("loss_prep", &loss_prep, "loss normalisers from one-hot action rows (graph-replayable)", py::arg("act"),
+          py::arg("ws"), py::arg("norms"), py::arg("idx") = py::none());
   m.def("loss_prep_ws_elems", &loss_prep_ws_elems, "int32 workspace elements of loss_prep");
   m.def("loss_assemble", &loss_assemble, "loss scalar + metrics from heads/loss partials", py::arg("part"),
         py::arg("norms"), py::arg("N"), py::arg("algo"), py::arg("ent_coef"), py::arg("vf_coef"), py::arg("out"),
@@ -1097,6 +1146,10 @@
         "[K/32][R][32] images, the dpre_dx operand layout)", py::arg("src"), py::arg("slab_major") = false);
   m.def("enc_small_grads", &enc_small_grads, "entity-encoder type-bias and env-layer gradients in one pass");
   m.def("replay_gather", &replay_gather, "minibatch gather from an HBM replay pool into time-major rows (one launch)");
+  m.def("step_prologue", &step_prologue, "replay_gather + zero fill + weight_prep in one launch; returns the gathered "
+        "tensors", py::arg("pools"), py::arg("n_step"), py::arg("idx"), py::arg("zero"), py::arg("src"),
+        py::arg("map16"), py::arg("dst16"), py::arg("map32"), py::arg("dst32"), py::arg("maps") = py::none(),
+        py::arg("dsth") = py::none(), py::arg("dstl") = py::none());
   m.def("vtrace_step", &vtrace_step, "V-trace advantages / value targets of a minibatch from the step's own values",
         py::arg("z"), py::arg("vcol"), py::arg("lp"), py::arg("mu"), py::arg("vt"), py::arg("B"), py::arg("S"),
         py::arg("gamma"), py::arg("lam"), py::arg("rho_bar") = 1.0, py::arg("c_bar") = 1.0);
diff --git a/dotaclient_amd/ops/csrc/glue.hip b/dotaclient_amd/ops/csrc/glue.hip
--- a/dotaclient_amd/ops/csrc/glue.hip
+++ b/dotaclient_amd/ops/csrc/glue.hip
@@ -8,14 +8,16 @@
 __global__ __launch_bounds__(kPrepThreads) void loss_prep_kernel(const unsigned char* __restrict__ act, int N, int A,
                                                                  int* __restrict__ partial,
                                                                  unsigned* __restrict__ counter,
-                                                                 float* __restrict__ norms) {
+                                                                 float* __restrict__ norms,
+                                                                 const long long* __restrict__ idx, int S, int B) {
   const int lane = threadIdx.x & 63, w = threadIdx.x >> 6;
   const int nw = gridDim.x * (kPrepThreads / dca::kWave);
   const unsigned long long m_enum = 0x7ull, m_x = 0x1ffull << 3, m_y = 0x1ffull << 12;
   const unsigned long long m_t = ~(m_enum | m_x | m_y);
   int c[5] = {0, 0, 0, 0, 0};
   for (int r = blockIdx.x * (kPrepThreads / dca::kWave) + w; r < N; r += nw) {
-    const unsigned char* row = act + (size_t)r * A;
+    const size_t pr = idx ? (size_t)idx[r % B] * S + r / B : (size_t)r;
+    const unsigned char* row = act + pr * A;
     const bool v0 = lane < A && row[lane] != 0;
     const bool v1 = lane + 64 < A && row[lane + 64] != 0;
     const unsigned long long b0 = __ballot(v0), b1 = __ballot(v1);
@@ -136,28 +138,42 @@
   for (int i = 12; i < 16; ++i) out[i] = 0.f;
 }
 
-__global__ __launch_bounds__(256) void weight_prep_kernel(const float* __restrict__ src, const int* __restrict__ map16,
-                                                          short* __restrict__ dst16, int n16,
-                                                          const int2* __restrict__ map32, float* __restrict__ dst32,
-                                                          int n32, const int* __restrict__ maps,
-                                                          short* __restrict__ dsth, short* __restrict__ dstl, int ns) {
-  const int stride = gridDim.x * blockDim.x;
-  for (int i = blockIdx.x * blockDim.x + threadIdx.x; i < ns; i += stride) {
+struct WeightPrepArgs {
+  const float* src;
+  const int* map16; short* dst16; int n16;
+  const int2* map32; float* dst32; int n32;
+  const int* maps; short* dsth; short* dstl; int ns;
+};
+
+__device__ __forceinline__ void weight_prep_body(const WeightPrepArgs& a, int bx, int nbx) {
+  const float* __restrict__ src = a.src;
+  const int* __restrict__ map16 = a.map16;
+  short* __restrict__ dst16 = a.dst16;
+  const int2* __restrict__ map32 = a.map32;
+  float* __restrict__ dst32 = a.dst32;
+  const int* __restrict__ maps = a.maps;
+  short* __restrict__ dsth = a.dsth;
+  short* __restrict__ dstl = a.dstl;
+  const int n16 = a.n16, n32 = a.n32, ns = a.ns;
+  const int stride = nbx * 256, first = bx * 256 + threadIdx.x;
+  for (int i = first; i < ns; i += stride) {
     const int m = maps[i];
     const float v = m >= 0 ? src[m] : 0.f;
     const short h = dca::f2bf(v);
     dsth[i] = h;
     dstl[i] = dca::f2bf(v - dca::bf2f(h));
   }
-  for (int i = blockIdx.x * blockDim.x + threadIdx.x; i < n16; i += stride) {
+  for (int i = first; i < n16; i += stride) {
     const int m = map16[i];
     dst16[i] = dca::f2bf(m >= 0 ? src[m] : 0.f);
   }
-  for (int i = blockIdx.x * blockDim.x + threadIdx.x; i < n32; i += stride) {
+  for (int i = first; i < n32; i += stride) {
     const int2 m = map32[i];
     dst32[i] = (m.x >= 0 ? src[m.x] : 0.f) + (m.y >= 0 ? src[m.y] : 0.f);
   }
 }
+
+__global__ __launch_bounds__(256) void weight_prep_kernel(WeightPrepArgs a) { weight_prep_body(a, blockIdx.x, gridDim.x); }
 
 constexpr int kSgBlocks = 256;
 constexpr int kSgPhases = 4;
@@ -277,13 +293,14 @@
 };
 
 template <typename T>
-__device__ __forceinline__ void gather_rows(const GatherField& F, const long long* __restrict__ idx, int S, int B) {
+__device__ __forceinline__ void gather_rows(const GatherField& F, const long long* __restrict__ idx, int S, int B,
+                                            int bx, int nbx) {
   const long long wpr = F.row_bytes / (long long)sizeof(T);
   const long long rows = F.per_step ? (long long)S * B : B;
   const long long total = rows * wpr;
   const T* src = reinterpret_cast<const T*>(F.src);
   T* dst = reinterpret_cast<T*>(F.dst);
-  for (long long i = (long long)blockIdx.x * blockDim.x + threadIdx.x; i < total; i += (long long)gridDim.x * blockDim.x) {
+  for (long long i = (long long)bx * blockDim.x + threadIdx.x; i < total; i += (long long)nbx * blockDim.x) {
     const long long r = i / wpr, w = i - r * wpr;
     long long srow;
     if (F.per_step) {
@@ -296,20 +313,55 @@
   }
 }
 
-__global__ __launch_bounds__(256) void replay_gather_kernel(GatherArgs a) {
-  const GatherField& F = a.f[blockIdx.y];
-  if (F.unit == 16) gather_rows<uint4>(F, a.idx, a.S, a.B);
-  else if (F.unit == 4) gather_rows<unsigned>(F, a.idx, a.S, a.B);
-  else gather_rows<unsigned char>(F, a.idx, a.S, a.B);
-}
-
-}
-
-extern "C" hipError_t dca_replay_gather(const void* const* src, void* const* dst, const long long* row_bytes,
-                                        const int* per_step, int nf, const long long* idx, int S, int B,
-                                        hipStream_t st) {
-  if (nf < 1 || nf > kMaxGather) return hipErrorInvalidValue;
-  GatherArgs a{};
+constexpr int kGatherBlocks = 256;
+
+__device__ __forceinline__ void gather_field(const GatherArgs& a, int field, int bx) {
+  const GatherField& F = a.f[field];
+  if (F.unit == 16) gather_rows<uint4>(F, a.idx, a.S, a.B, bx, kGatherBlocks);
+  else if (F.unit == 4) gather_rows<unsigned>(F, a.idx, a.S, a.B, bx, kGatherBlocks);
+  else gather_rows<unsigned char>(F, a.idx, a.S, a.B, bx, kGatherBlocks);
+}
+
+__global__ __launch_bounds__(256) void replay_gather_kernel(GatherArgs a) { gather_field(a, blockIdx.y, blockIdx.x); }
+
+constexpr int kZeroSpan = 256 * 4 * 4;
+struct PrologueArgs {
+  GatherArgs g;
+  WeightPrepArgs w;
+  float* zero; long long nzero;
+  int gblocks, wblocks;
+  int zero_vec;
+};
+
+__global__ __launch_bounds__(256) void step_prologue_kernel(PrologueArgs a) {
+  int b = blockIdx.x;
+  if (b < a.gblocks) {
+    gather_field(a.g, b / kGatherBlocks, b % kGatherBlocks);
+    return;
+  }
+  b -= a.gblocks;
+  if (b < a.wblocks) {
+    weight_prep_body(a.w, b, a.wblocks);
+    return;
+  }
+  b -= a.wblocks;
+  const long long base = (long long)b * kZeroSpan;
+  if (a.zero_vec && base + kZeroSpan <= a.nzero) {
+    uint4* p = reinterpret_cast<uint4*>(a.zero + base);
+#pragma unroll
+    for (int k = 0; k < 4; ++k) p[k * 256 + threadIdx.x] = make_uint4(0u, 0u, 0u, 0u);
+  } else {
+    const long long end = base + kZeroSpan < a.nzero ? base + kZeroSpan : a.nzero;
+    for (long long i = base + threadIdx.x; i < end; i += 256) a.zero[i] = 0.f;
+  }
+}
+
+}
+
+namespace {
+bool gather_args(GatherArgs& a, const void* const* src, void* const* dst, const long long* row_bytes,
+                 const int* per_step, int nf, const long long* idx, int S, int B) {
+  if (nf < 1 || nf > kMaxGather) return false;
   for (int i = 0; i < nf; ++i) {
     const unsigned long long align = (unsigned long long)src[i] | (unsigned long long)dst[i];
     int unit = 1;
@@ -320,7 +372,44 @@
   a.idx = idx;
   a.S = S;
   a.B = B;
-  hipLaunchKernelGGL(replay_gather_kernel, dim3(256, nf), dim3(256), 0, st, a);
+  return true;
+}
+
+int weight_prep_blocks(int n16, int n32, int ns) {
+  int n = n16 > n32 ? n16 : n32;
+  if (ns > n) n = ns;
+  int blocks = (n + 255) / 256;
+  if (blocks > 2048) blocks = 2048;
+  if (blocks < 1) blocks = 1;
+  return blocks;
+}
+}
+
+extern "C" hipError_t dca_replay_gather(const void* const* src, void* const* dst, const long long* row_bytes,
+                                        const int* per_step, int nf, const long long* idx, int S, int B,
+                                        hipStream_t st) {
+  GatherArgs a{};
+  if (!gather_args(a, src, dst, row_bytes, per_step, nf, idx, S, B)) return hipErrorInvalidValue;
+  hipLaunchKernelGGL(replay_gather_kernel, dim3(kGatherBlocks, nf), dim3(256), 0, st, a);
+  DCA_CHECK_LAUNCH();
+  return hipSuccess;
+}
+
+extern "C" hipError_t dca_step_prologue(const void* const* src, void* const* dst, const long long* row_bytes,
+                                        const int* per_step, int nf, const long long* idx, int S, int B, float* zero,
+                                        long long nzero, const float* wsrc, const int* map16, short* dst16, int n16,
+                                        const int* map32, float* dst32, int n32, const int* maps, short* dsth,
+                                        short* dstl, int ns, hipStream_t st) {
+  PrologueArgs a{};
+  if (!gather_args(a.g, src, dst, row_bytes, per_step, nf, idx, S, B) || nzero < 0) return hipErrorInvalidValue;
+  a.w = WeightPrepArgs{wsrc, map16, dst16, n16, reinterpret_cast<const int2*>(map32), dst32, n32, maps, dsth, dstl, ns};
+  a.zero = zero;
+  a.nzero = nzero;
+  a.gblocks = kGatherBlocks * nf;
+  a.wblocks = weight_prep_blocks(n16, n32, ns);
+  a.zero_vec = (unsigned long long)zero % 16 == 0;
+  const int zblocks = (int)((nzero + kZeroSpan - 1) / kZeroSpan);
+  hipLaunchKernelGGL(step_prologue_kernel, dim3(a.gblocks + a.wblocks + zblocks), dim3(256), 0, st, a);
   DCA_CHECK_LAUNCH();
   return hipSuccess;
 }
@@ -342,9 +431,10 @@
 extern "C" int dca_loss_prep_blocks() { return kPrepBlocks; }
 
 extern "C" hipError_t dca_loss_prep(const unsigned char* act, int N, int A, int* partial, unsigned* counter,
-                                    float* norms, hipStream_t st) {
+                                    float* norms, hipStream_t st, const long long* idx, int S, int B) {
+  if (idx && (S < 1 || B < 1 || N != S * B)) return hipErrorInvalidValue;
   hipLaunchKernelGGL(loss_prep_kernel, dim3(kPrepBlocks), dim3(kPrepThreads), 0, st, act, N, A, partial, counter,
-                     norms);
+                     norms, idx, S, B);
   DCA_CHECK_LAUNCH();
   return hipSuccess;
 }
@@ -360,13 +450,9 @@
 extern "C" hipError_t dca_weight_prep(const float* src, const int* map16, short* dst16, int n16, const int* map32,
                                       float* dst32, int n32, const int* maps, short* dsth, short* dstl, int ns,
                                       hipStream_t st) {
-  int n = n16 > n32 ? n16 : n32;
-  if (ns > n) n = ns;
-  int blocks = (n + 255) / 256;
-  if (blocks > 2048) blocks = 2048;
-  if (blocks < 1) blocks = 1;
-  hipLaunchKernelGGL(weight_prep_kernel, dim3(blocks), dim3(256), 0, st, src, map16, dst16, n16,
-                     reinterpret_cast<const int2*>(map32), dst32, n32, maps, dsth, dstl, ns);
+  hipLaunchKernelGGL(weight_prep_kernel, dim3(weight_prep_blocks(n16, n32, ns)), dim3(256), 0, st,
+                     WeightPrepArgs{src, map16, dst16, n16, reinterpret_cast<const int2*>(map32), dst32, n32, maps, dsth,
+                                    dstl, ns});
   DCA_CHECK_LAUNCH();
   return hipSuccess;
 }
diff --git a/dotaclient_amd/ops/csrc/heads_loss.hip b/dotaclient_amd/ops/csrc/heads_loss.hip
--- a/dotaclient_amd/ops/csrc/heads_loss.hip
+++ b/dotaclient_amd/ops/csrc/heads_loss.hip
@@ -5,6 +5,7 @@
 constexpr int kRowsPerBlock = 4;
 constexpr int kQ = 128;
 constexpr int kNPart = 16;
+constexpr int kBlocksPerCU = 3;
 
 struct Params {
   const float* z; int ldz;
@@ -42,192 +43,218 @@
   p = (in && m) ? (PRECISE ? e / s : xexp<PRECISE>(logp)) : 0.f;
 }
 
-template <bool F32, bool PRECISE>
+template <int NIT>
+struct RowIn {
+  float q8[8];
+  float zl, adv, ret, lpo, nret;
+  unsigned char a0, a1, m0, m1;
+  float e8[NIT][8];
+};
+
+struct RowLds {
+  float tl[64];
+  float dtl[64];
+  float zl[32];
+  unsigned char act[128];
+  unsigned char msk[128];
+};
+
+template <bool F32, int NIT>
+__device__ __forceinline__ void row_load(const Params& P, int n, int lane, RowIn<NIT>& L) {
+  const int U = P.U;
+  const float* zr = P.z + (size_t)n * P.ldz;
+  const int ks = lane & 15, ug = lane >> 4;
+  {
+    const float4 a = *reinterpret_cast<const float4*>(zr + 8 * ks);
+    const float4 b = *reinterpret_cast<const float4*>(zr + 8 * ks + 4);
+    L.q8[0] = a.x; L.q8[1] = a.y; L.q8[2] = a.z; L.q8[3] = a.w;
+    L.q8[4] = b.x; L.q8[5] = b.y; L.q8[6] = b.z; L.q8[7] = b.w;
+  }
+  L.zl = zr[kQ + min(lane, 21)];
+  L.adv = P.adv[n]; L.ret = P.ret[n]; L.lpo = P.logp_old[n]; L.nret = P.nret[n];
+  const unsigned char* ar = P.act + (size_t)n * P.A;
+  const unsigned char* mr = P.msk + (size_t)n * P.A;
+  L.a0 = ar[min(lane, P.A - 1)]; L.a1 = ar[min(lane + 64, P.A - 1)];
+  L.m0 = mr[min(lane, P.A - 1)]; L.m1 = mr[min(lane + 64, P.A - 1)];
+  const int nit = (U + 3) >> 2;
+  const int lo = ug * kQ + 8 * ks, lo_last = min(ug, U - 1 - (nit - 1) * 4) * kQ + 8 * ks;
+#pragma unroll
+  for (int it = 0; it < NIT; ++it)
+    if (it < nit) {
+      const size_t o = ((size_t)n * U + it * 4) * kQ + (it == nit - 1 ? lo_last : lo);
+      if constexpr (F32) {
+        const float4 a = *reinterpret_cast<const float4*>(static_cast<const float*>(P.emb) + o);
+        const float4 b = *reinterpret_cast<const float4*>(static_cast<const float*>(P.emb) + o + 4);
+        L.e8[it][0] = a.x; L.e8[it][1] = a.y; L.e8[it][2] = a.z; L.e8[it][3] = a.w;
+        L.e8[it][4] = b.x; L.e8[it][5] = b.y; L.e8[it][6] = b.z; L.e8[it][7] = b.w;
+      } else {
+        const dca::bf16x8 h = *reinterpret_cast<const dca::bf16x8*>(static_cast<const short*>(P.emb) + o);
+#pragma unroll
+        for (int j = 0; j < 8; ++j) L.e8[it][j] = dca::bf2f(h[j]);
+      }
+    }
+}
+
+template <bool PRECISE, int NIT>
+__device__ __forceinline__ void row_compute(const Params& P, int n, int lane, const RowIn<NIT>& L,
+                                            const float (&nm)[8], RowLds& S, float (&acc)[kNPart]) {
+  const int U = P.U;
+  const int ks = lane & 15, ug = lane >> 4;
+  const int nit = (U + 3) >> 2;
+  if (lane < 32) S.zl[lane] = L.zl;
+  S.act[lane] = L.a0; S.act[lane + 64] = L.a1;
+  S.msk[lane] = L.m0; S.msk[lane + 64] = L.m1;
+#pragma unroll
+  for (int it = 0; it < NIT; ++it) {
+    if (it < nit) {
+      const int u = it * 4 + ug;
+      float d = 0.f;
+#pragma unroll
+      for (int j = 0; j < 8; ++j) d += L.q8[j] * L.e8[it][j];
+      d = dca::group_sum<16>(d);
+      if (ks == 0 && u < U) S.tl[u] = d;
+    }
+  }
+  __builtin_amdgcn_wave_barrier();
+  __builtin_amdgcn_fence(__ATOMIC_RELEASE, "wavefront");
+  const int hoff[4] = {0, 3, 12, 21};
+  const int hw[4] = {3, 9, 9, U};
+  float logp[4], pr[4], a[4];
+  bool mk[4];
+  float sel = 0.f;
+  int nsel = 0;
+#pragma unroll
+  for (int h = 0; h < 4; ++h) {
+    const bool in = lane < hw[h];
+    float lg = 0.f;
+    if (in) lg = (h == 3) ? S.tl[lane] : S.zl[hoff[h] + lane];
+    mk[h] = in && S.msk[hoff[h] + lane];
+    a[h] = (in && S.act[hoff[h] + lane]) ? 1.f : 0.f;
+    head_lsm<PRECISE>(lg, mk[h], lane, hw[h], logp[h], pr[h]);
+    if (!in) logp[h] = 0.f;
+    const float sh = dca::wave_sum(a[h] * logp[h]);
+    sel += sh;
+    const int ns = __popcll(__ballot(a[h] > 0.f));
+    nsel += ns;
+    acc[2 + h] += -dca::wave_sum(mk[h] ? pr[h] * logp[h] : 0.f);
+  }
+  const float valid = nsel > 0 ? 1.f : 0.f;
+  const float V = S.zl[21];
+  const float R = L.ret;
+  float g_sel = 0.f, dV = 0.f;
+  if (P.algo == 0) {
+    const float A = L.adv;
+    const float lr = sel - L.lpo;
+    const float r = xexp<PRECISE>(lr);
+    const float s1 = r * A;
+    const float rc = fminf(fmaxf(r, 1.f - P.clip_eps), 1.f + P.clip_eps);
+    const float s2 = rc * A;
+    acc[0] += valid * fminf(s1, s2);
+    const bool clipped = (A > 0.f && r > 1.f + P.clip_eps) || (A < 0.f && r < 1.f - P.clip_eps);
+    g_sel = clipped ? 0.f : -valid * A * r * nm[0];
+    acc[1] += valid * (V - R) * (V - R);
+    dV = P.vf_coef * 2.f * (V - R) * valid * nm[0];
+    acc[6] += valid * (-lr);
+    acc[7] += valid * (fabsf(r - 1.f) > P.clip_eps ? 1.f : 0.f);
+    acc[8] += valid * A;
+  } else if (P.algo == 2) {
+    const float A = L.adv;
+    const float lr = sel - L.lpo;
+    const float r = xexp<PRECISE>(lr);
+    const float w = fminf(r, 1.f);
+    acc[0] += valid * w * A;
+    g_sel = -valid * A * w * nm[0];
+    acc[1] += valid * (V - R) * (V - R);
+    dV = P.vf_coef * 2.f * (V - R) * valid * nm[0];
+    acc[6] += valid * (-lr);
+    acc[7] += valid * (r > 1.f ? 1.f : 0.f);
+    acc[8] += valid * A;
+  } else {
+    const float nr = L.nret;
+    acc[0] += -sel * nr;
+    g_sel = -nr * nm[1];
+    acc[1] += (V - R) * (V - R);
+    acc[9] += V;
+    acc[10] += V * V;
+    acc[8] += V - R;
+    if (P.vf_coef > 0.f) {
+      if (P.compat_value_bug) {
+        const float Sq = (float)P.S_bug, Bq = (float)P.B_bug;
+        dV = P.vf_coef * 2.f * (Sq * V - nm[6]) / (Bq * Sq * Sq);
+      } else {
+        dV = P.vf_coef * 2.f * (V - R) / ((float)P.S_bug * (float)P.B_bug);
+      }
+    }
+  }
+  acc[11] += valid;
+  if (P.logp_out) if (lane == 0) P.logp_out[n] = sel;
+#pragma unroll
+  for (int h = 0; h < 4; ++h) {
+    const bool in = lane < hw[h];
+    float dlp = g_sel * a[h];
+    if (P.ent_coef > 0.f) dlp += P.ent_coef * nm[2 + h] * (mk[h] ? pr[h] * (1.f + logp[h]) : 0.f);
+    if (!in) dlp = 0.f;
+    const float sd = dca::wave_sum(dlp);
+    const float dl = dlp - (mk[h] ? pr[h] : 0.f) * sd;
+    if (in) {
+      if (h == 3) {
+        S.dtl[lane] = dl;
+        P.dtl[(size_t)n * U + lane] = dl;
+      } else {
+        put_dz(P, (size_t)n * P.ldz + kQ + hoff[h] + lane, dl);
+      }
+    }
+  }
+  if (lane == 0) put_dz(P, (size_t)n * P.ldz + kQ + 21, dV);
+  for (int c = kQ + 22 + lane; c < P.ldz; c += 64) put_dz(P, (size_t)n * P.ldz + c, 0.f);
+  __builtin_amdgcn_wave_barrier();
+  __builtin_amdgcn_fence(__ATOMIC_RELEASE, "wavefront");
+  float dq[8] = {0.f, 0.f, 0.f, 0.f, 0.f, 0.f, 0.f, 0.f};
+#pragma unroll
+  for (int it = 0; it < NIT; ++it) {
+    if (it < nit) {
+      const int u = it * 4 + ug;
+      const float g = (u < U) ? S.dtl[u] : 0.f;
+#pragma unroll
+      for (int j = 0; j < 8; ++j) dq[j] += g * L.e8[it][j];
+    }
+  }
+#pragma unroll
+  for (int j = 0; j < 8; ++j) {
+    dq[j] += __shfl_xor(dq[j], 16, 64);
+    dq[j] += __shfl_xor(dq[j], 32, 64);
+  }
+  if (ug == 0) {
+    if (P.dz16) {
+      dca::bf16x8 h;
+#pragma unroll
+      for (int j = 0; j < 8; ++j) h[j] = dca::f2bf(dq[j]);
+      *reinterpret_cast<dca::bf16x8*>(P.dz16 + (size_t)n * P.ldz + 8 * ks) = h;
+    } else {
+      float4* o = reinterpret_cast<float4*>(P.dz + (size_t)n * P.ldz + 8 * ks);
+      o[0] = make_float4(dq[0], dq[1], dq[2], dq[3]);
+      o[1] = make_float4(dq[4], dq[5], dq[6], dq[7]);
+    }
+  }
+}
+
+template <bool F32, bool PRECISE, int NIT>
 __global__ __launch_bounds__(256) void heads_loss_kernel(Params P) {
-  const int tid = threadIdx.x, wv = tid >> 6, lane = tid & 63;
+  const int tid = threadIdx.x, wv = __builtin_amdgcn_readfirstlane(tid >> 6), lane = tid & 63;
   const int n = blockIdx.x * kRowsPerBlock + wv;
-  __shared__ float s_tl[kRowsPerBlock][64];
-  __shared__ float s_dtl[kRowsPerBlock][64];
+  __shared__ RowLds s_row[kRowsPerBlock];
   __shared__ float s_part[kRowsPerBlock][kNPart];
-  __shared__ float s_zl[kRowsPerBlock][32];
-  __shared__ unsigned char s_act[kRowsPerBlock][128];
-  __shared__ unsigned char s_msk[kRowsPerBlock][128];
   float acc[kNPart];
 #pragma unroll
   for (int i = 0; i < kNPart; ++i) acc[i] = 0.f;
 
   if (n < P.N) {
-    const int U = P.U;
-    const float* zr = P.z + (size_t)n * P.ldz;
-    const int ks = lane & 15, ug = lane >> 4;
-    float q8[8];
-    {
-      const float4 a = *reinterpret_cast<const float4*>(zr + 8 * ks);
-      const float4 b = *reinterpret_cast<const float4*>(zr + 8 * ks + 4);
-      q8[0] = a.x; q8[1] = a.y; q8[2] = a.z; q8[3] = a.w; q8[4] = b.x; q8[5] = b.y; q8[6] = b.z; q8[7] = b.w;
-    }
-    const float zl = zr[kQ + min(lane, 21)];
-    const float A_n = P.adv[n], R_n = P.ret[n], lpo_n = P.logp_old[n], nret_n = P.nret[n];
+    RowIn<NIT> L;
+    row_load<F32, NIT>(P, n, lane, L);
     float nm[8];
 #pragma unroll
     for (int i = 0; i < 8; ++i) nm[i] = P.norms[i];
-    const unsigned char* ar = P.act + (size_t)n * P.A;
-    const unsigned char* mr = P.msk + (size_t)n * P.A;
-    const unsigned char a0 = ar[min(lane, P.A - 1)], a1 = ar[min(lane + 64, P.A - 1)];
-    const unsigned char m0 = mr[min(lane, P.A - 1)], m1 = mr[min(lane + 64, P.A - 1)];
-    constexpr int kMaxIt = 16;
-    float e8[kMaxIt][8];
-    const int nit = (U + 3) >> 2;
-#pragma unroll
-    for (int it = 0; it < kMaxIt; ++it)
-      if (it < nit) {
-        const size_t o = ((size_t)n * U + min(it * 4 + ug, U - 1)) * kQ + 8 * ks;
-        if constexpr (F32) {
-          const float4 a = *reinterpret_cast<const float4*>(static_cast<const float*>(P.emb) + o);
-          const float4 b = *reinterpret_cast<const float4*>(static_cast<const float*>(P.emb) + o + 4);
-          e8[it][0] = a.x; e8[it][1] = a.y; e8[it][2] = a.z; e8[it][3] = a.w;
-          e8[it][4] = b.x; e8[it][5] = b.y; e8[it][6] = b.z; e8[it][7] = b.w;
-        } else {
-          const dca::bf16x8 h = *reinterpret_cast<const dca::bf16x8*>(static_cast<const short*>(P.emb) + o);
-#pragma unroll
-          for (int j = 0; j < 8; ++j) e8[it][j] = dca::bf2f(h[j]);
-        }
-      }
-    if (lane < 32) s_zl[wv][lane] = zl;
-    s_act[wv][lane] = a0; s_act[wv][lane + 64] = a1;
-    s_msk[wv][lane] = m0; s_msk[wv][lane + 64] = m1;
-#pragma unroll
-    for (int it = 0; it < kMaxIt; ++it) {
-      if (it < nit) {
-        const int u = it * 4 + ug;
-        float d = 0.f;
-#pragma unroll
-        for (int j = 0; j < 8; ++j) d += q8[j] * e8[it][j];
-        d = dca::group_sum<16>(d);
-        if (ks == 0 && u < U) s_tl[wv][u] = d;
-      }
-    }
-    __builtin_amdgcn_wave_barrier();
-    __builtin_amdgcn_fence(__ATOMIC_RELEASE, "wavefront");
-    const int hoff[4] = {0, 3, 12, 21};
-    const int hw[4] = {3, 9, 9, U};
-    float logp[4], pr[4], a[4];
-    bool mk[4];
-    float sel = 0.f;
-    int nsel = 0;
-#pragma unroll
-    for (int h = 0; h < 4; ++h) {
-      const bool in = lane < hw[h];
-      float lg = 0.f;
-      if (in) lg = (h == 3) ? s_tl[wv][lane] : s_zl[wv][hoff[h] + lane];
-      mk[h] = in && s_msk[wv][hoff[h] + lane];
-      a[h] = (in && s_act[wv][hoff[h] + lane]) ? 1.f : 0.f;
-      head_lsm<PRECISE>(lg, mk[h], lane, hw[h], logp[h], pr[h]);
-      if (!in) logp[h] = 0.f;
-      const float sh = dca::wave_sum(a[h] * logp[h]);
-      sel += sh;
-      const int ns = __popcll(__ballot(a[h] > 0.f));
-      nsel += ns;
-      acc[2 + h] += -dca::wave_sum(mk[h] ? pr[h] * logp[h] : 0.f);
-    }
-    const float valid = nsel > 0 ? 1.f : 0.f;
-    const float V = s_zl[wv][21];
-    const float R = R_n;
-    float g_sel = 0.f, dV = 0.f;
-    if (P.algo == 0) {
-      const float A = A_n;
-      const float lr = sel - lpo_n;
-      const float r = xexp<PRECISE>(lr);
-      const float s1 = r * A;
-      const float rc = fminf(fmaxf(r, 1.f - P.clip_eps), 1.f + P.clip_eps);
-      const float s2 = rc * A;
-      acc[0] += valid * fminf(s1, s2);
-      const bool clipped = (A > 0.f && r > 1.f + P.clip_eps) || (A < 0.f && r < 1.f - P.clip_eps);
-      g_sel = clipped ? 0.f : -valid * A * r * nm[0];
-      acc[1] += valid * (V - R) * (V - R);
-      dV = P.vf_coef * 2.f * (V - R) * valid * nm[0];
-      acc[6] += valid * (-lr);
-      acc[7] += valid * (fabsf(r - 1.f) > P.clip_eps ? 1.f : 0.f);
-      acc[8] += valid * A;
-    } else if (P.algo == 2) {
-      const float A = A_n;
-      const float lr = sel - lpo_n;
-      const float r = xexp<PRECISE>(lr);
-      const float w = fminf(r, 1.f);
-      acc[0] += valid * w * A;
-      g_sel = -valid * A * w * nm[0];
-      acc[1] += valid * (V - R) * (V - R);
-      dV = P.vf_coef * 2.f * (V - R) * valid * nm[0];
-      acc[6] += valid * (-lr);
-      acc[7] += valid * (r > 1.f ? 1.f : 0.f);
-      acc[8] += valid * A;
-    } else {
-      const float nr = nret_n;
-      acc[0] += -sel * nr;
-      g_sel = -nr * nm[1];
-      acc[1] += (V - R) * (V - R);
-      acc[9] += V;
-      acc[10] += V * V;
-      acc[8] += V - R;
-      if (P.vf_coef > 0.f) {
-        if (P.compat_value_bug) {
-          const float S = (float)P.S_bug, Bq = (float)P.B_bug;
-          dV = P.vf_coef * 2.f * (S * V - nm[6]) / (Bq * S * S);
-        } else {
-          dV = P.vf_coef * 2.f * (V - R) / ((float)P.S_bug * (float)P.B_bug);
-        }
-      }
-    }
-    acc[11] += valid;
-    if (P.logp_out) if (lane == 0) P.logp_out[n] = sel;
-#pragma unroll
-    for (int h = 0; h < 4; ++h) {
-      const bool in = lane < hw[h];
-      float dlp = g_sel * a[h];
-      if (P.ent_coef > 0.f) dlp += P.ent_coef * nm[2 + h] * (mk[h] ? pr[h] * (1.f + logp[h]) : 0.f);
-      if (!in) dlp = 0.f;
-      const float sd = dca::wave_sum(dlp);
-      const float dl = dlp - (mk[h] ? pr[h] : 0.f) * sd;
-      if (in) {
-        if (h == 3) {
-          s_dtl[wv][lane] = dl;
-          P.dtl[(size_t)n * U + lane] = dl;
-        } else {
-          put_dz(P, (size_t)n * P.ldz + kQ + hoff[h] + lane, dl);
-        }
-      }
-    }
-    if (lane == 0) put_dz(P, (size_t)n * P.ldz + kQ + 21, dV);
-    for (int c = kQ + 22 + lane; c < P.ldz; c += 64) put_dz(P, (size_t)n * P.ldz + c, 0.f);
-    __builtin_amdgcn_wave_barrier();
-    __builtin_amdgcn_fence(__ATOMIC_RELEASE, "wavefront");
-    float dq[8] = {0.f, 0.f, 0.f, 0.f, 0.f, 0.f, 0.f, 0.f};
-#pragma unroll
-    for (int it = 0; it < kMaxIt; ++it) {
-      if (it < nit) {
-        const int u = it * 4 + ug;
-        const float g = (u < U) ? s_dtl[wv][u] : 0.f;
-#pragma unroll
-        for (int j = 0; j < 8; ++j) dq[j] += g * e8[it][j];
-      }
-    }
-#pragma unroll
-    for (int j = 0; j < 8; ++j) {
-      dq[j] += __shfl_xor(dq[j], 16, 64);
-      dq[j] += __shfl_xor(dq[j], 32, 64);
-    }
-    if (ug == 0) {
-      if (P.dz16) {
-        dca::bf16x8 h;
-#pragma unroll
-        for (int j = 0; j < 8; ++j) h[j] = dca::f2bf(dq[j]);
-        *reinterpret_cast<dca::bf16x8*>(P.dz16 + (size_t)n * P.ldz + 8 * ks) = h;
-      } else {
-        float4* o = reinterpret_cast<float4*>(P.dz + (size_t)n * P.ldz + 8 * ks);
-        o[0] = make_float4(dq[0], dq[1], dq[2], dq[3]);
-        o[1] = make_float4(dq[4], dq[5], dq[6], dq[7]);
-      }
-    }
+    row_compute<PRECISE, NIT>(P, n, lane, L, nm, s_row[wv], acc);
   }
   if (lane == 0) {
 #pragma unroll
@@ -245,18 +272,39 @@
 }
 
 extern "C" int dca_heads_loss_nblocks(int N) { return (N + kRowsPerBlock - 1) / kRowsPerBlock; }
+
+extern "C" int dca_heads_loss_resident_blocks() {
+  static const int cap = [] {
+    int dev = 0, cus = 0;
+    if (hipGetDevice(&dev) != hipSuccess ||
+        hipDeviceGetAttribute(&cus, hipDeviceAttributeMultiprocessorCount, dev) != hipSuccess || cus < 1)
+      cus = 256;
+    return kBlocksPerCU * cus;
+  }();
+  return cap;
+}
 
 extern "C" hipError_t dca_heads_loss(const float* z, int ldz, const void* emb, const unsigned char* act,
                                      const unsigned char* msk, int A, const float* adv, const float* ret,
                                      const float* logp_old, const float* nret, const float* norms, float* dz,
                                      float* dtl, float* part, float* logp_out, int N, int U, int algo,
                                      int compat_value_bug, int S_bug, int B_bug, float clip_eps, float ent_coef,
-                                     float vf_coef, hipStream_t st, short* dz16, int emb_f32, int precise) {
+                                     float vf_coef, hipStream_t st, short* dz16, int emb_f32, int precise,
+                                     int wide) {
   if (U > 64 || U < 1 || ldz < kQ + 22 || A != 21 + U) return hipErrorInvalidValue;
   Params P{z, ldz, emb, act, msk, A, adv, ret, logp_old, nret, norms, dz, dtl, part, logp_out, dz16, N, U, algo,
            compat_value_bug, S_bug, B_bug, clip_eps, ent_coef, vf_coef};
-  if (emb_f32 && precise) heads_loss_kernel<true, true><<<dca_heads_loss_nblocks(N), 256, 0, st>>>(P);
-  else if (emb_f32) heads_loss_kernel<true, false><<<dca_heads_loss_nblocks(N), 256, 0, st>>>(P);
-  else heads_loss_kernel<false, false><<<dca_heads_loss_nblocks(N), 256, 0, st>>>(P);
+  const int nblk = dca_heads_loss_nblocks(N);
+  static const bool wide_env = [] { const char* e = getenv("DCA_HEADS_WIDE"); return e && e[0] == '1'; }();
+  const bool small = U <= 40 && !(wide < 0 ? wide_env : wide != 0);
+#define DCA_HL_LAUNCH(F, Pr) \
+  do { \
+    if (small) heads_loss_kernel<F, Pr, 10><<<nblk, 256, 0, st>>>(P); \
+    else heads_loss_kernel<F, Pr, 16><<<nblk, 256, 0, st>>>(P); \
+  } while (0)
+  if (emb_f32 && precise) DCA_HL_LAUNCH(true, true);
+  else if (emb_f32) DCA_HL_LAUNCH(true, false);
+  else DCA_HL_LAUNCH(false, false);
+#undef DCA_HL_LAUNCH
   return hipGetLastError();
 }
diff --git a/dotaclient_amd/ops/csrc/launchers.h b/dotaclient_amd/ops/csrc/launchers.h
--- a/dotaclient_amd/ops/csrc/launchers.h
+++ b/dotaclient_amd/ops/csrc/launchers.h
@@ -45,11 +45,13 @@
                           const float* scale, hipStream_t st);
 
 int dca_heads_loss_nblocks(int N);
+int dca_heads_loss_resident_blocks();
 hipError_t dca_heads_loss(const float* z, int ldz, const void* emb, const unsigned char* act, const unsigned char* msk,
                           int A, const float* adv, const float* ret, const float* logp_old, const float* nret,
                           const float* norms, float* dz, float* dtl, float* part, float* logp_out, int N, int U,
                           int algo, int compat_value_bug, int S_bug, int B_bug, float clip_eps, float ent_coef,
-                          float vf_coef, hipStream_t st, short* dz16, int emb_f32, int precise = 0);
+                          float vf_coef, hipStream_t st, short* dz16, int emb_f32, int precise = 0,
+                          int wide = -1);
 
 hipError_t dca_encoder_fwd(const float* units, const float* env, const float* w1, const float* b1, const void* wt,
                            const float* bt, const float* we, const float* be, void* x896, void* emb,
@@ -97,7 +99,7 @@
 
 int dca_loss_prep_blocks();
 hipError_t dca_loss_prep(const unsigned char* act, int N, int A, int* partial, unsigned* counter, float* norms,
-                         hipStream_t st);
+                         hipStream_t st, const long long* idx = nullptr, int S = 0, int B = 0);
 hipError_t dca_occupy_xcd(int xcd, int blocks, double seconds, int* seen, hipStream_t st);
 hipError_t dca_featurize_raw(const void* raw, const float* hero, void* units, void* handles, int rows, int U,
                              int half_out, hipStream_t st);
@@ -121,5 +123,9 @@
 
 hipError_t dca_replay_gather(const void* const* src, void* const* dst, const long long* row_bytes, const int* per_step,
                              int nf, const long long* idx, int S, int B, hipStream_t st);
+hipError_t dca_step_prologue(const void* const* src, void* const* dst, const long long* row_bytes, const int* per_step,
+                             int nf, const long long* idx, int S, int B, float* zero, long long nzero,
+                             const float* wsrc, const int* map16, short* dst16, int n16, const int* map32,
+                             float* dst32, int n32, const int* maps, short* dsth, short* dstl, int ns, hipStream_t st);
 
 }
```

Result: no change. 2.019 million (median of 6 runs) (+0.6%).
